# peaceminusones/Group-GAN-GCN-GAT

Hardware: AMD Instinct MI355X
Metric: scenes/sec (obs8/pred12, 20 peds) at 1/2/4/8 GPUs; ADE/FDE vs ref (higher is better)
Workload: dtype fp32; 1 GPU; train iteration = D-step + G-step (best_k=20, Adam), GAT generator; BASELINE configs[1] shape (batch 64); scenes_per_gpu=64, global_batch=64, obs_len=8, pred_len=12, generator=gat, hip_graph=True, parallelism=dp1

## Files before the change

### group-gan-gcn-gat_amd/csrc/fold.hip

```cpp
#include "sgg_common.h"

namespace sgg {

__global__ void __launch_bounds__(512) fold_fwd_kernel(const float* __restrict__ W, int ldw, int R, int E,
                                                       const float* __restrict__ We, const float* __restrict__ be,
                                                       const float* __restrict__ b1, const float* __restrict__ b2,
                                                       float* __restrict__ A, float* __restrict__ bias) {
  for (int r = threadIdx.x; r < R; r += blockDim.x) {
    float a0 = 0.f, a1 = 0.f, bb = 0.f;
    const float* w = W + (size_t)r * ldw;
#pragma unroll 8
    for (int e = 0; e < E; ++e) {
      const float we = w[e];
      a0 = fmaf(we, We[2 * e], a0);
      a1 = fmaf(we, We[2 * e + 1], a1);
      bb = fmaf(we, be[e], bb);
    }
    A[2 * r] = a0;
    A[2 * r + 1] = a1;
    bias[r] = bb + b1[r] + (b2 ? b2[r] : 0.f);
  }
}

struct FoldList {
  SggFold f[SGG_FOLD_MAX];
};

__global__ void __launch_bounds__(512) fold_fwd_multi_kernel(FoldList L) {
  const SggFold& d = L.f[blockIdx.x];
  for (int r = threadIdx.x; r < d.R; r += blockDim.x) {
    float a0 = 0.f, a1 = 0.f, bb = 0.f;
    const float* w = d.W + (size_t)r * d.ldw;
#pragma unroll 8
    for (int e = 0; e < d.E; ++e) {
      const float we = w[e];
      a0 = fmaf(we, d.We[2 * e], a0);
      a1 = fmaf(we, d.We[2 * e + 1], a1);
      bb = fmaf(we, d.be[e], bb);
    }
    d.A[2 * r] = a0;
    d.A[2 * r + 1] = a1;
    d.bias[r] = bb + d.b1[r] + (d.b2 ? d.b2[r] : 0.f);
  }
}

__device__ __forceinline__ void fold_bwd_body(const float* __restrict__ W, int ldw, int R, int E,
                                              const float* __restrict__ We, const float* __restrict__ be,
                                              const float* __restrict__ dA, const float* __restrict__ dbias,
                                              float* __restrict__ dW, int lddw, float* __restrict__ dWe,
                                              float* __restrict__ dbe, float* __restrict__ dbias_copy) {
  __shared__ float g3[3 * 512];
  __shared__ float part[3 * 512];
  for (int r = threadIdx.x; r < R; r += blockDim.x) {
    const float2 a = reinterpret_cast<const float2*>(dA)[r];
    const float b = dbias[r];
    g3[3 * r] = a.x;
    g3[3 * r + 1] = a.y;
    g3[3 * r + 2] = b;
    if (dbias_copy) dbias_copy[r] = b;
  }
  __syncthreads();
  const int ng = blockDim.x / E;
  const int t = threadIdx.x;
  if (t < ng * E) {
    const int e = t % E, g = t / E;
    const float we0 = We[2 * e], we1 = We[2 * e + 1], bee = be[e];
    float s0 = 0.f, s1 = 0.f, s2 = 0.f;
#pragma unroll 8
    for (int r = g; r < R; r += ng) {
      const float a0 = g3[3 * r], a1 = g3[3 * r + 1], b = g3[3 * r + 2];
      dW[(size_t)r * lddw + e] = fmaf(a0, we0, fmaf(a1, we1, b * bee));
      const float w = W[(size_t)r * ldw + e];
      s0 = fmaf(w, a0, s0);
      s1 = fmaf(w, a1, s1);
      s2 = fmaf(w, b, s2);
    }
    part[3 * t] = s0;
    part[3 * t + 1] = s1;
    part[3 * t + 2] = s2;
  }
  __syncthreads();
  if (t < 3 * E) {
    const int e = t / 3, j = t - 3 * e;
    float s = 0.f;
    for (int g = 0; g < ng; ++g) s += part[3 * (g * E + e) + j];
    if (j < 2) dWe[2 * e + j] = s;
    else dbe[e] = s;
  }
}

__global__ void __launch_bounds__(512) fold_bwd_kernel(const float* __restrict__ W, int ldw, int R, int E,
                                                       const float* __restrict__ We, const float* __restrict__ be,
                                                       const float* __restrict__ dA, const float* __restrict__ dbias,
                                                       float* __restrict__ dW, int lddw, float* __restrict__ dWe,
                                                       float* __restrict__ dbe, float* __restrict__ dbias_copy) {
  fold_bwd_body(W, ldw, R, E, We, be, dA, dbias, dW, lddw, dWe, dbe, dbias_copy);
// ... 53 lines not shown
```

### group-gan-gcn-gat_amd/csrc/lstm.hip

```cpp
#include <stdlib.h>
#include <string.h>

#include "sgg_common.h"

namespace sgg {

constexpr int kLstmPeds = 4;
constexpr int kLstmMaxT = 32;

__device__ __forceinline__ float sigm(float x) { return __builtin_amdgcn_rcpf(1.f + __expf(-x)); }
__device__ __forceinline__ float tanh_f(float x) {
  return fmaf(2.f, __builtin_amdgcn_rcpf(1.f + __builtin_amdgcn_exp2f(x * -2.8853900817779268f)), -1.f);
}

template <int H>
__global__ void __launch_bounds__(16 * H) lstm_fwd_kernel(
    const float* __restrict__ rel, const float* __restrict__ A, const float* __restrict__ Whh,
    const float* __restrict__ bias, const float* __restrict__ h0, const float* __restrict__ c0,
    const float* __restrict__ Wp, const float* __restrict__ bp, int T, int B, int decoder,
    float* __restrict__ h_all, float* __restrict__ c_all, float* __restrict__ act_all, float* __restrict__ rel_out) {
  const bool save_states = act_all != nullptr;
  constexpr int G4 = 4 * H;
  __shared__ __attribute__((aligned(16))) float hbuf[kLstmPeds][H];
  __shared__ float gbuf[kLstmPeds][G4];
// ... 236 lines not shown
    const bool x3 = H == 32 && !(x3e && strcmp(x3e, "0") == 0);
    snprintf(buf, sizeof buf, "sgg::lstm_fwd_mfma_kernel<%d, %s, %s>", H, tf[x3], tf[decoder != 0]);
  }
  else if (mw) snprintf(buf, sizeof buf, "sgg::lstm_mw_fwd_kernel<%d, %s, %s>", H, tf[decoder != 0], tf[save != 0]);
  else if (H <= 32) snprintf(buf, sizeof buf, "sgg::lstm_unit_fwd_kernel<%d>", H);
  else snprintf(buf, sizeof buf, "sgg::lstm_fwd_kernel<%d>", H);
  return buf;
}

static bool fwd_picks_mw(int H, int B, bool save) {
  const bool mw = lstm_mw_ok(H, B);
  if (save) return mw;
  return mw && !(lstm_fwd_mfma_ok(H, B) && !getenv("SGG_LSTM_NO_MFMA"));
}

extern "C" int sgg_lstm_u_ok(int T, int B, int H, int decoder, int save, int NU) {
  return !decoder && B > 0 && T >= 1 && NU >= 16 && NU % 16 == 0 && fwd_picks_mw(H, B, save != 0);
}

extern "C" int sgg_lstm_fwd_u(const float* rel, const float* A, const float* Whh, const float* bias, const float* h0,
                              const float* c0, int T, int B, int H, float* h_all, float* c_all, float* act_all,
                              const float* Wu, int ldwu, const float* cu, int NU, float* U, void* stream) {
  SGG_CHECK_ARG(rel && A && Whh && bias && h_all && c_all && Wu && cu && U, "sgg_lstm_fwd_u: null pointer");
  SGG_CHECK_ARG(sgg_lstm_u_ok(T, B, H, 0, act_all != nullptr, NU) && ldwu >= H,
                "sgg_lstm_fwd_u: no projection epilogue for T=%d B=%d H=%d NU=%d ldwu=%d (sgg_lstm_u_ok)", T, B, H, NU,
                ldwu);
  return lstm_mw_fwd(rel, A, Whh, bias, h0, c0, nullptr, nullptr, T, B, H, 0, h_all, c_all, act_all, nullptr,
                     (hipStream_t)stream, Wu, ldwu, cu, NU, U);
}

extern "C" int sgg_lstm_bwd_split(const float* A, const float* Whh, const float* Wp, const float* h_all,
                                  const float* c_all, const float* act_all, const float* rel, const float* rel_out,
                                  const float* dout, const float* dout2, int bsplit, int T, int B, int H, float* dh0,
                                  float* drel_in, float* drel_tot, float* wpart, void* stream) {
  SGG_CHECK_ARG(A && Whh && Wp && h_all && c_all && act_all && rel && rel_out && dout && dout2 && drel_in && drel_tot,
                "sgg_lstm_bwd_split: null pointer");
  SGG_CHECK_ARG(T >= 1 && B >= 1 && bsplit >= 0 && bsplit <= B && lstm_mw_ok(H, B),
                "sgg_lstm_bwd_split: bad sizes or no four-wave kernel (T=%d B=%d H=%d bsplit=%d)", T, B, H, bsplit);
  return lstm_mw_bwd(A, Whh, Wp, h_all, c_all, act_all, rel, rel_out, nullptr, dout, T, B, H, 1, dh0, drel_in,
                     drel_tot, wpart, (hipStream_t)stream, dout2, bsplit);
}

extern "C" int sgg_lstm_bwd_tail(const float* A, const float* Whh, const float* h_all, const float* c_all,
                                 const float* act_all, const float* rel, const float* dh_last, int T, int B, int H,
                                 int t_stop, float* drel_in, void* stream) {
  SGG_CHECK_ARG(A && Whh && h_all && c_all && act_all && rel && drel_in, "sgg_lstm_bwd_tail: null pointer");
  SGG_CHECK_ARG(T >= 1 && B >= 1 && t_stop >= 0 && t_stop < T && lstm_mw_ok(H, B),
                "sgg_lstm_bwd_tail: bad sizes or no four-wave kernel (T=%d B=%d H=%d t_stop=%d)", T, B, H, t_stop);
  return lstm_mw_bwd(A, Whh, nullptr, h_all, c_all, act_all, rel, nullptr, dh_last, nullptr, T, B, H, 0, nullptr,
                     drel_in, nullptr, nullptr, (hipStream_t)stream, nullptr, 0, t_stop);
}

static MwSeg to_mw(const SggLstmSeg& s) {
  return MwSeg{s.rel, s.A, s.Whh, s.bias, s.h0, s.c0, nullptr, nullptr, s.T, s.B, s.Bl, s.t0, s.Tl, s.Bsrc,
               s.h_all, s.c_all, s.act_all, nullptr, s.Wu, s.ldwu, s.cu, s.NU, s.U};
}

extern "C" int sgg_lstm_fwd_seg(const SggLstmSeg* seg, int H, void* stream) {
  SGG_CHECK_ARG(seg, "sgg_lstm_fwd_seg: null segment");
  SGG_CHECK_ARG(lstm_mw_ok(H, seg->B), "sgg_lstm_fwd_seg: no four-wave kernel for H=%d", H);
  return lstm_mw_fwd_seg(to_mw(*seg), H, (hipStream_t)stream);
}

static int device_cus() {
  static int ncu = 0;
  if (ncu == 0) {
    int d = 0, v = 0;
    const bool ok = hipGetDevice(&d) == hipSuccess &&
                    hipDeviceGetAttribute(&v, hipDeviceAttributeMultiprocessorCount, d) == hipSuccess;
    ncu = ok && v > 0 ? v : 256;
  }
  return ncu;
}

extern "C" int sgg_lstm_fwd_seg_glue(const SggLstmSeg* seg, int H, const SggGlueSeg* glue, void* stream) {
  SGG_CHECK_ARG(seg && glue, "sgg_lstm_fwd_seg_glue: null segment");
  SGG_CHECK_ARG(lstm_mw_ok(H, seg->B), "sgg_lstm_fwd_seg_glue: no four-wave kernel for H=%d", H);
  const SggGlueSeg& g = *glue;
  SGG_CHECK_ARG(g.kind == SGG_GLUE_NONE || g.kind == SGG_GLUE_SELECT || g.kind == SGG_GLUE_L2BWD,
                "sgg_lstm_fwd_seg_glue: glue kind %d", g.kind);
  if (g.kind == SGG_GLUE_SELECT) {
    SGG_CHECK_ARG(g.pred && g.gt && g.mask && g.scene_off && g.best, "sgg_lstm_fwd_seg_glue (select): null pointer");
    SGG_CHECK_ARG(g.S >= 0 && g.T >= 1 && g.B >= 0 && g.k >= 1 && g.k <= 256 && g.ldm >= g.T,
                  "sgg_lstm_fwd_seg_glue (select): bad sizes");
  } else if (g.kind == SGG_GLUE_L2BWD) {
    SGG_CHECK_ARG(g.pred && g.gt && g.mask && g.scene_off && g.gout && g.dpred,
                  "sgg_lstm_fwd_seg_glue (l2 backward): null pointer");
    SGG_CHECK_ARG(g.S >= 0 && g.T >= 1 && g.B >= 0 && g.ldm >= g.T && g.ldp >= 2 * g.B && g.ldd >= 2 * g.B,
                  "sgg_lstm_fwd_seg_glue (l2 backward): bad sizes");
  }
  if (g.kind != SGG_GLUE_NONE && g.S > 0) {
    const int cus = device_cus(), nblk = (seg->B + 15) / 16, last = nblk % cus;
    if ((nblk >= cus && last == 0) || last + g.S > cus) {
      const int rc = g.kind == SGG_GLUE_SELECT
                         ? sgg_l2_select(g.pred, g.gt, g.mask, g.ldm, g.scene_off, g.S, g.T, g.B, g.k, g.best, stream)
                         : sgg_l2_loss_bwd_scenes(g.pred, g.ldp, g.gt, g.mask, g.ldm, g.scene_off, g.S, g.T, g.B, g.w,
                                                  g.gout, g.dpred, g.ldd, g.term, stream);
      if (rc) return rc;
      return lstm_mw_fwd_seg(to_mw(*seg), H, (hipStream_t)stream);
    }
  }
  return lstm_mw_fwd_seg(to_mw(*seg), H, (hipStream_t)stream, glue);
}

extern "C" int sgg_lstm_fwd_seg2(const SggLstmSeg* a, int Ha, const SggLstmSeg* b, int Hb, void* stream) {
  SGG_CHECK_ARG(a && b, "sgg_lstm_fwd_seg2: null segment");
  SGG_CHECK_ARG(lstm_mw_ok(Ha, a->B) && lstm_mw_ok(Hb, b->B), "sgg_lstm_fwd_seg2: no four-wave kernel (Ha=%d Hb=%d)",
                Ha, Hb);
  return lstm_mw_fwd_seg2(to_mw(*a), Ha, to_mw(*b), Hb, (hipStream_t)stream);
}

extern "C" int sgg_lstm_fwd_seg3(const SggLstmSeg* a, int Ha, const SggLstmSeg* b, int Hb, const SggLstmSeg* c, int Hc,
                                 void* stream) {
  SGG_CHECK_ARG(a && b && c, "sgg_lstm_fwd_seg3: null segment");
  SGG_CHECK_ARG(lstm_mw_ok(Ha, a->B) && lstm_mw_ok(Hb, b->B) && lstm_mw_ok(Hc, c->B),
                "sgg_lstm_fwd_seg3: no four-wave kernel (Ha=%d Hb=%d Hc=%d)", Ha, Hb, Hc);
  return lstm_mw_fwd_seg3(to_mw(*a), Ha, to_mw(*b), Hb, to_mw(*c), Hc, (hipStream_t)stream);
}

extern "C" int sgg_lstm_bwd_shared(const float* A, const float* Whh, const float* h_all, const float* c_all,
                                   const float* act_all, const float* rel, const float* dh_last, int T, int B, int H,
                                   int t_sh, int Bsrc, float* drel_in, float* wpart, void* stream) {
  SGG_CHECK_ARG(A && Whh && h_all && c_all && act_all && rel, "sgg_lstm_bwd_shared: null pointer");
  SGG_CHECK_ARG(T >= 1 && B >= 1 && t_sh >= 1 && lstm_mw_ok(H, B),
                "sgg_lstm_bwd_shared: bad sizes or no four-wave kernel (T=%d B=%d H=%d t_sh=%d)", T, B, H, t_sh);
  SGG_CHECK_ARG(drel_in || (wpart && lstm_mw_bwd_nodx_ok(H)),
                "sgg_lstm_bwd_shared: drel_in may be NULL only with weight gradients (wpart) and H = 16 / 32 / 48 "
                "(wpart=%d H=%d)", wpart != nullptr, H);
  return lstm_mw_bwd(A, Whh, nullptr, h_all, c_all, act_all, rel, nullptr, dh_last, nullptr, T, B, H, 0, nullptr,
                     drel_in, nullptr, wpart, (hipStream_t)stream, nullptr, 0, 0, t_sh, Bsrc);
}

extern "C" int sgg_lstm_wpart_rows(int H, int B) {
  if (B < 0) return -1;
  return lstm_mw_ok(H, B) ? lstm_mw_wpart_rows(H, B) : 0;
}

extern "C" int sgg_lstm_fwd(const float* rel, const float* A, const float* Whh, const float* bias, const float* h0,
                            const float* c0, const float* Wp, const float* bp, int T, int B, int H, int decoder, float* h_all,
                            float* c_all, float* act_all, float* rel_out, void* stream) {
  SGG_CHECK_ARG(rel && A && Whh && bias && h_all && c_all, "sgg_lstm_fwd: null pointer");
  SGG_CHECK_ARG(!decoder || (Wp && bp && rel_out), "sgg_lstm_fwd: decoder needs Wp, bp, rel_out");
  SGG_CHECK_ARG(T >= 1 && B >= 0, "sgg_lstm_fwd: bad sizes T=%d B=%d", T, B);
  if (B == 0) return 0;
  hipStream_t st = (hipStream_t)stream;
  const bool mw = lstm_mw_ok(H, B);
  if (act_all && mw)
    return lstm_mw_fwd(rel, A, Whh, bias, h0, c0, Wp, bp, T, B, H, decoder, h_all, c_all, act_all, rel_out, st);
  if (!act_all && lstm_fwd_mfma_ok(H, B) && !getenv("SGG_LSTM_NO_MFMA"))
    return lstm_fwd_mfma(rel, A, Whh, bias, h0, c0, Wp, bp, T, B, H, decoder, h_all, c_all, nullptr, rel_out, st);
  if (mw)
    return lstm_mw_fwd(rel, A, Whh, bias, h0, c0, Wp, bp, T, B, H, decoder, h_all, c_all, act_all, rel_out, st);
  if (lstm_unit_ok(H, decoder) && !getenv("SGG_LSTM_ROWS"))
    return lstm_unit_fwd(rel, A, Whh, bias, h0, c0, Wp, bp, T, B, H, decoder, h_all, c_all, act_all, rel_out, st);
  switch (H) {
    case 16: return launch_lstm_fwd<16>(rel, A, Whh, bias, h0, c0, Wp, bp, T, B, decoder, h_all, c_all, act_all, rel_out, st);
    case 32: return launch_lstm_fwd<32>(rel, A, Whh, bias, h0, c0, Wp, bp, T, B, decoder, h_all, c_all, act_all, rel_out, st);
    case 48: return launch_lstm_fwd<48>(rel, A, Whh, bias, h0, c0, Wp, bp, T, B, decoder, h_all, c_all, act_all, rel_out, st);
    case 64: return launch_lstm_fwd<64>(rel, A, Whh, bias, h0, c0, Wp, bp, T, B, decoder, h_all, c_all, act_all, rel_out, st);
    default: SGG_CHECK_ARG(false, "sgg_lstm_fwd: hidden size %d not built (16/32/48/64)", H);
  }
}

static int dec_check(const SggDecInit* di, const float* A, const float* Whh, const float* bias, const float* Wp,
                     const float* bp, int T, int B, int H, float* h_all, float* c_all, float* act_all, float* rel_out,
                     const SggTrajOut* to) {
  SGG_CHECK_ARG(di && di->ctx && di->ped_scene && di->last_rel && (di->nz == 0 || di->z) && A && Whh && bias &&
                    ((h_all && c_all) || (!h_all && !c_all && !act_all)) && Wp && bp && rel_out,
                "sgg_lstm_fwd_dec: null pointer");
  SGG_CHECK_ARG(T >= 1 && B >= 0 && di->Bper >= 1 && B % di->Bper == 0 && di->Dc >= 1 && di->nz >= 0 &&
                    di->Dc + di->nz == H && di->ldc >= di->Dc && di->S >= 1,
                "sgg_lstm_fwd_dec: bad sizes (T=%d B=%d Bper=%d Dc=%d nz=%d H=%d)", T, B, di->Bper, di->Dc, di->nz, H);
  if (to) {
    SGG_CHECK_ARG(to->out && to->head && (!to->start || to->pos0), "sgg_lstm_fwd_dec: null pointer in SggTrajOut");
    SGG_CHECK_ARG(to->T0 >= 0 && to->ncol >= 1 && to->col0 >= 0 && to->col0 + to->ncol <= B &&
                      to->NB == (to->b ? 2 : 1) * to->ncol && to->ldh >= 2 * to->ncol &&
                      (!to->b || to->ldb >= 2 * to->ncol),
                  "sgg_lstm_fwd_dec: bad SggTrajOut sizes (NB=%d T0=%d col0=%d ncol=%d B=%d)", to->NB, to->T0,
                  to->col0, to->ncol, B);
  }
  return 0;
}

extern "C" int sgg_lstm_fwd_dec_seg(const SggDecInit* di, const float* A, const float* Whh, const float* bias,
                                    const float* Wp, const float* bp, int T, int B, int H, float* h_all, float* c_all,
                                    float* act_all, float* rel_out, float* rel0_out, const SggTrajOut* to,
                                    const SggLstmSeg* pre, int Hp, void* stream) {
  if (int rc = dec_check(di, A, Whh, bias, Wp, bp, T, B, H, h_all, c_all, act_all, rel_out, to)) return rc;
  SGG_CHECK_ARG(pre && B >= 1 && act_all && lstm_mw_ok(H, B) && lstm_mw_ok(Hp, pre->B),
                "sgg_lstm_fwd_dec_seg: needs a saving four-wave decoder and a prefix segment (H=%d B=%d Hp=%d)", H, B,
                Hp);
  return lstm_mw_fwd_dec_seg(A, Whh, bias, Wp, bp, T, B, H, h_all, c_all, act_all, rel_out, di, rel0_out, to,
                             to_mw(*pre), Hp, (hipStream_t)stream);
}

extern "C" int sgg_lstm_fwd_dec2(const SggDecInit* di, const SggDecInit* di2, const float* A, const float* Whh,
                                 const float* bias, const float* Wp, const float* bp, int T, int B, int B2, int H,
                                 float* rel_out, float* rel_out2, const SggTrajOut* to2, void* stream) {
  if (int rc = dec_check(di, A, Whh, bias, Wp, bp, T, B, H, nullptr, nullptr, nullptr, rel_out, nullptr)) return rc;
  if (int rc = dec_check(di2, A, Whh, bias, Wp, bp, T, B2, H, nullptr, nullptr, nullptr, rel_out2, to2)) return rc;
  SGG_CHECK_ARG(B >= 1 && B2 >= 1 && lstm_fwd_mfma_ok(H, B) && !getenv("SGG_LSTM_NO_MFMA"),
                "sgg_lstm_fwd_dec2: the batch-MFMA rollout family only (H=%d B=%d)", H, B);
  return lstm_fwd_mfma_dec2(di, di2, A, Whh, bias, Wp, bp, T, B, B2, H, rel_out, rel_out2, to2, (hipStream_t)stream);
}

extern "C" int sgg_lstm_fwd_dec(const SggDecInit* di, const float* A, const float* Whh, const float* bias,
                                const float* Wp, const float* bp, int T, int B, int H, float* h_all, float* c_all,
                                float* act_all, float* rel_out, float* rel0_out, const SggTrajOut* to,
                                void* stream) {
  if (int rc = dec_check(di, A, Whh, bias, Wp, bp, T, B, H, h_all, c_all, act_all, rel_out, to)) return rc;
  if (B == 0) return 0;
  hipStream_t st = (hipStream_t)stream;
  const bool mw = lstm_mw_ok(H, B);
  if (act_all && mw)
    return lstm_mw_fwd(nullptr, A, Whh, bias, nullptr, nullptr, Wp, bp, T, B, H, 1, h_all, c_all, act_all, rel_out,
                       st, nullptr, 0, nullptr, 0, nullptr, di, rel0_out, to);
  if (!act_all && lstm_fwd_mfma_ok(H, B) && !getenv("SGG_LSTM_NO_MFMA")) {
    if (to) {
      SGG_CHECK_ARG(!h_all, "sgg_lstm_fwd_dec: the batch-MFMA family writes the discriminator input without a "
                            "final state (h_all NULL)");
      return lstm_fwd_mfma_dec2(di, di, A, Whh, bias, Wp, bp, T, 0, B, H, nullptr, rel_out, to, st);
    }
    return lstm_fwd_mfma(nullptr, A, Whh, bias, nullptr, nullptr, Wp, bp, T, B, H, 1, h_all, c_all, nullptr, rel_out,
                         st, di);
  }
  SGG_CHECK_ARG(!to || mw, "sgg_lstm_fwd_dec: no family writes the discriminator input for H=%d B=%d", H, B);
  if (!act_all && mw)
    return lstm_mw_fwd(nullptr, A, Whh, bias, nullptr, nullptr, Wp, bp, T, B, H, 1, h_all, c_all, nullptr, rel_out, st,
                       nullptr, 0, nullptr, 0, nullptr, di, nullptr, to);
  SGG_CHECK_ARG(false, "sgg_lstm_fwd_dec: no fused decoder start for H=%d B=%d (use sgg_decoder_init)", H, B);
}

extern "C" int sgg_lstm_bwd(const float* A, const float* Whh, const float* Wp, const float* h_all, const float* c_all,
                            const float* act_all, const float* rel, const float* rel_out, const float* dh_last,
                            const float* dout, int T, int B, int H, int decoder, float* dG, float* dh0,
                            float* drel_in, float* drel_tot, float* wpart, void* stream) {
  SGG_CHECK_ARG(A && Whh && c_all && act_all, "sgg_lstm_bwd: null pointer");
  SGG_CHECK_ARG(drel_in || (!decoder && wpart && lstm_mw_ok(H, B) && lstm_mw_bwd_nodx_ok(H)),
                "sgg_lstm_bwd: drel_in may be NULL only for an encoder of the four-wave family with weight gradients "
                "(wpart) and H = 16 / 32 / 48 (decoder=%d wpart=%d H=%d)", decoder, wpart != nullptr, H);
  SGG_CHECK_ARG(!decoder || (Wp && dout && drel_tot), "sgg_lstm_bwd: decoder needs Wp, dout, drel_tot");
// ... 22 lines not shown
```

### group-gan-gcn-gat_amd/csrc/lstm_mw.hip

```cpp
#include <stdlib.h>
#include <string.h>

#include <type_traits>

#include "sgg_common.h"
#include "l2_body.h"

namespace sgg {

namespace {

constexpr int kMwThreads = 256;
constexpr int kMwPeds = 16;
constexpr int kMwMaxT = 64;
constexpr int kDgPitch = 68;

constexpr float kNegLog2e = -1.4426950408889634f;
__device__ __forceinline__ float gate_act(float x, float s, float nsl) {
  return fmaf(s, __builtin_amdgcn_rcpf(1.f + __builtin_amdgcn_exp2f(x * nsl)), 1.f - s);
}
__device__ __forceinline__ float tanh_m(float x) {
  return fmaf(2.f, __builtin_amdgcn_rcpf(1.f + __builtin_amdgcn_exp2f(x * (2.f * kNegLog2e))), -1.f);
}

template <int MU>
__device__ __forceinline__ void store_vec(float* p, const float (&v)[MU]) {
  if constexpr (MU == 4) {
    *reinterpret_cast<float4*>(p) = make_float4(v[0], v[1], v[2], v[3]);
  } else if constexpr (MU == 2) {
    *reinterpret_cast<float2*>(p) = make_float2(v[0], v[1]);
  } else if constexpr (MU == 3) {
    typedef float f3 __attribute__((ext_vector_type(3)));
    f3 x = {v[0], v[1], v[2]};
    __builtin_memcpy(p, &x, 12);
  } else {
#pragma unroll
    for (int i = 0; i < MU; ++i) p[i] = v[i];
  }
}
template <int MU>
__device__ __forceinline__ void load_vec(const float* p, float (&v)[MU]) {
  if constexpr (MU == 4) {
    const float4 x = *reinterpret_cast<const float4*>(p);
    v[0] = x.x; v[1] = x.y; v[2] = x.z; v[3] = x.w;
  } else if constexpr (MU == 2) {
    const float2 x = *reinterpret_cast<const float2*>(p);
    v[0] = x.x; v[1] = x.y;
  } else if constexpr (MU == 3) {
    typedef float f3 __attribute__((ext_vector_type(3)));
    f3 x;
    __builtin_memcpy(&x, p, 12);
    v[0] = x.x; v[1] = x.y; v[2] = x.z;
  } else {
#pragma unroll
    for (int i = 0; i < MU; ++i) v[i] = p[i];
  }
}

__device__ __forceinline__ int slot_unit(int j, int q) { return 16 * (j >> 2) + 4 * q + (j & 3); }

__device__ __forceinline__ floatx4 mfma_x3x2(const bf16x8 (&a)[2][3], const bf16x8 (&b)[2][3], floatx4 c) {
  constexpr int pa[6] = {2, 1, 0, 1, 0, 0}, pb[6] = {0, 1, 2, 0, 1, 0};
#pragma unroll
  for (int k = 0; k < 6; ++k) {
    c = __builtin_amdgcn_mfma_f32_16x16x32_bf16(a[0][pa[k]], b[0][pb[k]], c, 0, 0, 0);
    c = __builtin_amdgcn_mfma_f32_16x16x32_bf16(a[1][pa[k]], b[1][pb[k]], c, 0, 0, 0);
  }
  return c;
}

template <int H>
struct MwCfg {
  static constexpr int MU = H / 16, KS = H / 4, G4 = 4 * H;
  static constexpr int HP = H <= 16 ? 16 : 80;
  static constexpr int NHS = (kMwPeds * H + kMwThreads - 1) / kMwThreads;
  static constexpr int P = G4 * H + G4 + 2 * G4;
};

}


#ifdef SGG_LSTM_PROF
__device__ long long g_lstm_prof[256];
#define LMARK(i) \
  if (threadIdx.x == 0 && blk == 0) g_lstm_prof[i] = wall_clock64();
#define LSUB(k) \
  if ((threadIdx.x & 63) == 0 && blk == 0 && t == 4) g_lstm_prof[64 + 8 * (threadIdx.x >> 6) + (k)] = wall_clock64();
#define LUSE(x) __asm__ volatile("" ::"v"(x));
#define LSUBB(k) \
  if ((threadIdx.x & 63) == 0 && blk == 0 && t == T - 5) g_lstm_prof[96 + 8 * (threadIdx.x >> 6) + (k)] = wall_clock64();
#else
#define LSUBB(k)
#define LMARK(i)
#define LSUB(k)
#define LUSE(x)
#endif

#ifndef SGG_MW_UPRE
#define SGG_MW_UPRE 1
#endif
#ifndef SGG_MW_FWD_X3
#define SGG_MW_FWD_X3 1
#endif

namespace {

template <int H, bool DEC, bool SAVE>
__device__ __forceinline__ void mw_fwd_body(const MwSeg& sg, int blk, const SggGlueSeg* glue = nullptr) {
  constexpr int MU = MwCfg<H>::MU, KS = MwCfg<H>::KS;
  constexpr bool decoder = DEC, save = SAVE;
  const float* __restrict__ rel = sg.rel;
  const float* __restrict__ A = sg.A;
  const float* __restrict__ Whh = sg.Whh;
  const float* __restrict__ bias = sg.bias;
  const float* __restrict__ Wp = sg.Wp;
  const float* __restrict__ bp = sg.bp;
  float* __restrict__ h_all = sg.h_all;
  float* __restrict__ c_tile = sg.c_tile;
  float* __restrict__ act_tile = sg.act_tile;
  float* __restrict__ rel_out = sg.rel_out;
  const int T = sg.T, B = sg.B, Bl = sg.Bl, t0 = sg.t0, Tl = sg.Tl;
  constexpr bool X3 = !DEC && SGG_MW_FWD_X3 && H == 48;
  __shared__ float hb[X3 ? 1 : 2][KS][64];
  __shared__ sgg_uint4v hx[X3 ? 2 : 1][3][2][64];
  constexpr int kHsP = H + 4;
  __shared__ float hst[X3 && SAVE ? 2 : 1][kMwPeds][X3 && SAVE ? kHsP : 1];
  __shared__ float2 rpart[2][4][kMwPeds];
  __shared__ float relseq[kMwMaxT][kMwPeds][2];
  if constexpr (!DEC) {
    if (glue) {
      static_assert(sizeof(relseq) >= kL2MaxElems * sizeof(float) && sizeof(hx) >= kL2MaxK * sizeof(float),
                    "the glue bodies' LDS is lent by relseq / hx");
      float* msk = &relseq[0][0][0];
      if (glue->kind == SGG_GLUE_SELECT) {
        l2_select_body<kMwThreads / 64>(glue->pred, glue->gt, glue->mask, glue->ldm, glue->scene_off, glue->T,
                                        glue->B, glue->k, glue->best, blk, reinterpret_cast<float*>(&hx[0][0][0][0]),
                                        msk);
      } else if (threadIdx.x < 64) {
        l2_bwd_scene_body(glue->pred, glue->ldp, glue->gt, glue->mask, glue->ldm, glue->scene_off, glue->T, glue->B,
                          glue->w, glue->gout, glue->dpred, glue->ldd, glue->term, blk, threadIdx.x, msk);
      }
      return;
    }
  }
  const int g = __builtin_amdgcn_readfirstlane(threadIdx.x >> 6);
  const int lane = threadIdx.x & 63;
  const int q = lane >> 4, c16 = lane & 15;
  const int ped = blk * kMwPeds + c16;
  const int pc = ped < B ? ped : B - 1;
  LMARK(0);

  float w[MU][KS + 1], ak0[MU], ak1[MU];
  bf16x8 wx[X3 ? MU : 1][2][3];
  if constexpr (X3) {
#pragma unroll
    for (int mu = 0; mu < MU; ++mu) {
      const int row = (c16 & 3) * H + slot_unit(g * MU + mu, c16 >> 2);
      const float a0 = A[2 * row], a1 = A[2 * row + 1], bi = bias[row];
#pragma unroll
      for (int c = 0; c < 2; ++c) {
        float v[8];
#pragma unroll
        for (int i = 0; i < 8; ++i) {
          const int w2 = (8 * c + i) >> 2, m2 = (8 * c + i) & 3;
          if (m2 < MU)
            v[i] = Whh[row * H + slot_unit(w2 * MU + m2, q)];
          else if (m2 == 3)
            v[i] = q != 0 ? 0.f : w2 == 0 ? a0 : w2 == 1 ? a1 : w2 == 2 ? bi : 0.f;
          else
            v[i] = 0.f;
        }
        split8(v, wx[mu][c]);
      }
    }
  }
#pragma unroll
  for (int mu = 0; mu < (X3 ? 0 : MU); ++mu) {
    const int row = (c16 & 3) * H + slot_unit(g * MU + mu, c16 >> 2);
#pragma unroll
    for (int m = 0; m < KS / 4; ++m) {
      const float4 v = *reinterpret_cast<const float4*>(Whh + row * H + 16 * m + 4 * q);
      w[mu][4 * m] = v.x;
      w[mu][4 * m + 1] = v.y;
      w[mu][4 * m + 2] = v.z;
      w[mu][4 * m + 3] = v.w;
    }
    ak0[mu] = A[2 * row];
    ak1[mu] = A[2 * row + 1];
    w[mu][KS] = q == 0 ? ak0[mu] : q == 1 ? ak1[mu] : q == 2 ? bias[row] : 0.f;
  }
  float c[MU], wp0[MU], wp1[MU], hv0[MU];
  const int nsrc = (sg.Bsrc + kMwPeds - 1) / kMwPeds;
  const int sblk = t0 > 0 ? blk % nsrc : blk;
  const int spc = t0 > 0 ? pc % sg.Bsrc : pc;
#pragma unroll
  for (int i = 0; i < MU; ++i) {
    const int j = g * MU + i, u = slot_unit(j, q);
    float hv, cv;
    if (t0 > 0) {
      hv = h_all[((size_t)t0 * Bl + spc) * H + u];
      cv = c_tile[((((size_t)sblk * (Tl + 1) + t0) * 4 + g) * 64 + lane) * MU + i];
    } else {
      hv = sg.di.ctx ? dec_h0(sg.di, pc, u) : sg.h0 ? sg.h0[(size_t)pc * H + u] : 0.f;
      cv = sg.c0 ? sg.c0[(size_t)pc * H + u] : 0.f;
      if (save) {
        h_all[(size_t)pc * H + u] = hv;
        c_tile[(((size_t)blk * (Tl + 1) * 4 + g) * 64 + lane) * MU + i] = cv;
      }
    }
    c[i] = cv;
    hv0[i] = hv;
    if constexpr (!X3) hb[0][j][lane] = hv;
    wp0[i] = decoder ? Wp[u] : 0.f;
    wp1[i] = decoder ? Wp[H + u] : 0.f;
  }
  const float bp0 = decoder ? bp[0] : 0.f, bp1 = decoder ? bp[1] : 0.f;
  constexpr int kTo = 4;
  float2 tov[kTo];
  float2* tod[kTo];
  int nto = 0;
  if (DEC && sg.to.out != nullptr) {
    const SggTrajOut& to = sg.to;
    const int dup = to.b ? 2 : 1;
    const int nh = to.T0 * dup, nb = to.b ? T : 0, ns = to.start ? dup : 0;
    nto = kMwPeds * (nh + nb + ns);
    auto entry = [&](int e, float2*& d) -> float2 {
      const int i = e % kMwPeds, w = e / kMwPeds;
      const int col = min(blk * kMwPeds + i, B - 1) - to.col0;
      d = nullptr;
      if (col < 0 || col >= to.ncol) return make_float2(0.f, 0.f);
      float2* o2 = reinterpret_cast<float2*>(to.out);
      if (w < nh) {
        const int t = w / dup, half = w - t * dup;
        d = o2 + (size_t)t * to.NB + col + half * to.ncol;
        return reinterpret_cast<const float2*>(to.head + (size_t)t * to.ldh)[col];
      }
      if (w < nh + nb) {
        const int t = w - nh;
        d = o2 + (size_t)(to.T0 + t) * to.NB + to.ncol + col;
        return reinterpret_cast<const float2*>(to.b + (size_t)t * to.ldb)[col];
      }
      d = reinterpret_cast<float2*>(to.start) + col + (w - nh - nb) * to.ncol;
      return reinterpret_cast<const float2*>(to.pos0)[col];
    };
#pragma unroll
    for (int m = 0; m < kTo; ++m) {
      const int e = threadIdx.x + m * kMwThreads;
      tod[m] = nullptr;
      if (e < nto) tov[m] = entry(e, tod[m]);
    }
    for (int e = threadIdx.x + kTo * kMwThreads; e < nto; e += kMwThreads) {
      float2* d;
      const float2 v = entry(e, d);
      if (d) *d = v;
    }
  }

  constexpr int kRelPer = 2 * kMwPeds * kMwMaxT / kMwThreads;
  float rv[kRelPer];
  if (!decoder) {
#pragma unroll
    for (int m = 0; m < kRelPer; ++m) {
      const int e = threadIdx.x + m * kMwThreads;
      if (e < 2 * kMwPeds * T) {
        const int t = e / (2 * kMwPeds), p = (e >> 1) & (kMwPeds - 1), k = e & 1;
        const int pp = min(blk * kMwPeds + p, B - 1);
        rv[m] = rel[((size_t)(t0 + t) * B + pp) * 2 + k];
      }
    }
  }

  constexpr bool kUPre = SGG_MW_UPRE && !DEC && H <= 48;
  constexpr int kUT = 8;
  const float* __restrict__ Wu = sg.Wu;
  const int ldwu = sg.ldwu, NU = sg.NU;
  const bool upre = kUPre && sg.U && NU <= 16 * 4 * kUT &&
                    ((reinterpret_cast<uintptr_t>(Wu) | ((uintptr_t)ldwu * 4)) & 15) == 0;
  float wu[kUPre ? kUT : 1][KS];
  float cuv[kUPre ? kUT : 1][4];
  auto load_wu = [&](int i) {
    const int ntile = NU >> 4;
    const float4 v = *reinterpret_cast<const float4*>(sg.cu + 16 * min(g + 4 * i, ntile - 1) + 4 * q);
    cuv[i][0] = v.x;
    cuv[i][1] = v.y;
    cuv[i][2] = v.z;
    cuv[i][3] = v.w;
    const float* wr = Wu + (size_t)(min(g + 4 * i, ntile - 1) * 16 + c16) * ldwu;
#pragma unroll
    for (int m = 0; m < KS / 4; ++m) {
      const float4 w4 = *reinterpret_cast<const float4*>(wr + 16 * m + 4 * q);
      wu[i][4 * m] = w4.x;
      wu[i][4 * m + 1] = w4.y;
      wu[i][4 * m + 2] = w4.z;
      wu[i][4 * m + 3] = w4.w;
    }
  };

  if (!decoder) {
#pragma unroll
    for (int m = 0; m < kRelPer; ++m) {
      const int e = threadIdx.x + m * kMwThreads;
      if (e < 2 * kMwPeds * T) relseq[e / (2 * kMwPeds)][(e >> 1) & (kMwPeds - 1)][e & 1] = rv[m];
    }
  }
  if (DEC && nto > 0) {
#pragma unroll
    for (int m = 0; m < kTo; ++m)
      if (tod[m]) *tod[m] = tov[m];
  }
  auto put_x3 = [&](int buf, const float (&hv)[MU], float inv) {
    float v[4] = {0.f, 0.f, 0.f, inv};
#pragma unroll
    for (int i = 0; i < MU; ++i) v[i] = hv[i];
    unsigned wd[3][2];
#pragma unroll
    for (int k = 0; k < 2; ++k) {
      float h0, m0, l0, h1, m1, l1;
      split3(v[2 * k], h0, m0, l0);
      split3(v[2 * k + 1], h1, m1, l1);
      wd[0][k] = bf16_pack_top(h0, h1);
      wd[1][k] = bf16_pack_top(m0, m1);
      wd[2][k] = bf16_pack_top(l0, l1);
    }
#pragma unroll
    for (int p = 0; p < 3; ++p)
      reinterpret_cast<uint2*>(&hx[buf][p][g >> 1][lane])[g & 1] = make_uint2(wd[p][0], wd[p][1]);
  };
  auto in_x3 = [&](int t) -> float {
    return g < 2 ? rel[((size_t)(t0 + t) * B + pc) * 2 + g] : (g == 2 ? 1.f : 0.f);
  };
  if constexpr (X3) put_x3(0, hv0, in_x3(0));
  lds_barrier();
  LMARK(1);

  auto input = [&](int t) -> float {
// ... 178 lines not shown
    for (int ks = 0; ks < KS; ++ks) hk[ks] = hb[X3 ? 0 : T & 1][ks][lane];
    const int ntile = NU >> 4;
    floatx4 acc[kUT];
#pragma unroll
    for (int i = 0; i < kUT; ++i) acc[i] = floatx4{0.f, 0.f, 0.f, 0.f};
#pragma unroll
    for (int ks = 0; ks < KS; ++ks)
#pragma unroll
      for (int i = 0; i < kUT; ++i) acc[i] = __builtin_amdgcn_mfma_f32_16x16x4f32(wu[i][ks], hk[ks], acc[i], 0, 0, 0);
#pragma unroll
    for (int i = 0; i < kUT; ++i) {
      const int nt = g + 4 * i;
      if (nt < ntile)
        *reinterpret_cast<float4*>(U + (size_t)pc * NU + 16 * nt + 4 * q) =
            make_float4(acc[i][0] + cuv[i][0], acc[i][1] + cuv[i][1], acc[i][2] + cuv[i][2], acc[i][3] + cuv[i][3]);
    }
  } else if (!decoder && U) {
    float hk[KS];
#pragma unroll
    for (int ks = 0; ks < KS; ++ks) hk[ks] = hb[X3 ? 0 : T & 1][ks][lane];
    const int ntile = NU >> 4;
    float wa[2][KS], wn[2][KS];
    const bool vec = ((reinterpret_cast<uintptr_t>(Wu) | ((uintptr_t)ldwu * 4)) & 15) == 0;
    auto load_w = [&](int nt, float (&w)[KS]) {
      const float* wr = Wu + (size_t)(min(nt, ntile - 1) * 16 + c16) * ldwu;
      if (vec) {
#pragma unroll
        for (int m = 0; m < KS / 4; ++m) {
          const float4 v = *reinterpret_cast<const float4*>(wr + 16 * m + 4 * q);
          w[4 * m] = v.x;
          w[4 * m + 1] = v.y;
          w[4 * m + 2] = v.z;
          w[4 * m + 3] = v.w;
        }
      } else {
#pragma unroll
        for (int ks = 0; ks < KS; ++ks) w[ks] = wr[slot_unit(ks, q)];
      }
    };
    load_w(g, wa[0]);
    load_w(g + 4, wa[1]);
    for (int nt = g; nt < ntile; nt += 8) {
      const bool more = nt + 8 < ntile;
      if (more) {
        load_w(nt + 8, wn[0]);
        load_w(nt + 12, wn[1]);
      }
      floatx4 acc0 = floatx4{0.f, 0.f, 0.f, 0.f}, acc1 = acc0;
#pragma unroll
      for (int ks = 0; ks < KS; ++ks) {
        acc0 = __builtin_amdgcn_mfma_f32_16x16x4f32(wa[0][ks], hk[ks], acc0, 0, 0, 0);
        acc1 = __builtin_amdgcn_mfma_f32_16x16x4f32(wa[1][ks], hk[ks], acc1, 0, 0, 0);
      }
      const float4 cb0 = *reinterpret_cast<const float4*>(cu + 16 * nt + 4 * q);
      *reinterpret_cast<float4*>(U + (size_t)pc * NU + 16 * nt + 4 * q) =
          make_float4(acc0[0] + cb0.x, acc0[1] + cb0.y, acc0[2] + cb0.z, acc0[3] + cb0.w);
      if (nt + 4 < ntile) {
        const float4 cb1 = *reinterpret_cast<const float4*>(cu + 16 * (nt + 4) + 4 * q);
        *reinterpret_cast<float4*>(U + (size_t)pc * NU + 16 * (nt + 4) + 4 * q) =
            make_float4(acc1[0] + cb1.x, acc1[1] + cb1.y, acc1[2] + cb1.z, acc1[3] + cb1.w);
      }
      if (more) {
#pragma unroll
        for (int ks = 0; ks < KS; ++ks) {
          wa[0][ks] = wn[0][ks];
          wa[1][ks] = wn[1][ks];
        }
      }
    }
  }
  LMARK(63);
}

template <int H, bool DEC, bool SAVE>
__global__ void __launch_bounds__(kMwThreads) lstm_mw_fwd_kernel(MwSeg sg, SggGlueSeg gl, int nblk) {
  if constexpr (!DEC) {
    if ((int)blockIdx.x >= nblk) {
      mw_fwd_body<H, DEC, SAVE>(sg, blockIdx.x - nblk, &gl);
      return;
    }
  }
  mw_fwd_body<H, DEC, SAVE>(sg, blockIdx.x);
}

template <int HA, bool SA, int HB, bool SB>
__global__ void __launch_bounds__(kMwThreads) lstm_mw_fwd2_kernel(MwSeg a, MwSeg b, int nblk_a) {
  if ((int)blockIdx.x < nblk_a)
    mw_fwd_body<HA, false, SA>(a, blockIdx.x);
  else
    mw_fwd_body<HB, false, SB>(b, blockIdx.x - nblk_a);
}

template <int HA, bool SA, int HB, bool SB>
__global__ void __launch_bounds__(kMwThreads) lstm_mw_fwd2d_kernel(MwSeg a, MwSeg b, int nblk_a) {
  if ((int)blockIdx.x < nblk_a)
    mw_fwd_body<HA, true, SA>(a, blockIdx.x);
  else
    mw_fwd_body<HB, false, SB>(b, blockIdx.x - nblk_a);
}

template <int HA, bool SA, int HB, bool SB, int HC, bool SC>
__global__ void __launch_bounds__(kMwThreads) lstm_mw_fwd3_kernel(MwSeg a, MwSeg b, MwSeg c, int nblk_a, int nblk_b) {
  const int blk = blockIdx.x;
  if (blk < nblk_a)
    mw_fwd_body<HA, false, SA>(a, blk);
  else if (blk < nblk_a + nblk_b)
    mw_fwd_body<HB, false, SB>(b, blk - nblk_a);
  else
    mw_fwd_body<HC, false, SC>(c, blk - nblk_a - nblk_b);
}

#ifndef SGG_MW_BWD_DB
#define SGG_MW_BWD_DB 1
#endif
#ifndef SGG_MW_BWD_X3
#define SGG_MW_BWD_X3 1
#endif
#ifndef SGG_MW_BWD_DB_NODX
#define SGG_MW_BWD_DB_NODX 1
#endif

template <int H, bool DEC, bool WGRAD, bool NODX>
__device__ __forceinline__ void mw_bwd_body(
    const float* __restrict__ A, const float* __restrict__ Whh, const float* __restrict__ Wp,
    const float* __restrict__ h_all, const float* __restrict__ c_tile, const float* __restrict__ act_tile,
    const float* __restrict__ rel, const float* __restrict__ rel_out, const float* __restrict__ dh_last,
    const float* __restrict__ dout, int T, int B, float* __restrict__ dh0, float* __restrict__ drel_in,
    float* __restrict__ drel_tot, float* __restrict__ wpart, const float* __restrict__ dout2, int bsplit,
    int t_stop, int t_sh, int Bsrc) {
  static_assert(!NODX || (WGRAD && !DEC), "NODX: the encoder's weight-gradient form only");
  constexpr int MU = MwCfg<H>::MU, KS = MwCfg<H>::KS, G4 = MwCfg<H>::G4, HP = MwCfg<H>::HP;
  constexpr bool decoder = DEC, wgrad = WGRAD;
  constexpr bool BX3 = SGG_MW_BWD_X3 != 0;
  constexpr bool hacc = wgrad && !decoder && !NODX;
  constexpr bool oacc = !(wgrad && !decoder);
  constexpr bool hdb = wgrad;
  constexpr int NHS = MwCfg<H>::NHS, P0 = MwCfg<H>::P, P = P0 + (DEC ? 2 * H + 2 : 0);
  __shared__ float dgb[2][4][KS][kDgPitch];
  __shared__ float part[2][4][KS][64];
  __shared__ float2 fbp[NODX ? 1 : 2][4][kMwPeds];
  __shared__ float hs[2][kMwPeds][HP];
  const int g = __builtin_amdgcn_readfirstlane(threadIdx.x >> 6);
  const int lane = threadIdx.x & 63;
  const int q = lane >> 4, c16 = lane & 15;
  const int blk = blockIdx.x;
  LMARK(0);
  const int ped = blk * kMwPeds + c16;
  const bool valid = ped < B;
  const int pc = valid ? ped : B - 1;
  const int nsrc = t_sh > 0 ? Bsrc / kMwPeds : 1;
  auto sblk = [&](bool shared_at) { return (shared_at && t_sh > 0) ? blk % nsrc : blk; };

  float hv[NHS];
  const int ht = threadIdx.x & (kMwThreads - 1);
  auto stage_load = [&](int t) {
#pragma unroll
    for (int m = 0; m < NHS; ++m) {
      const int e = ht + m * kMwThreads;
      int r = min(blk * kMwPeds + e / H, B - 1);
      if (t <= t_sh && t_sh > 0) r %= Bsrc;
      hv[m] = h_all[((size_t)t * B + r) * H + e % H];
    }
// ... 428 lines not shown
          x += __shfl_xor(x, o);
          y += __shfl_xor(y, o);
        }
        const int u = slot_unit(g * MU + i, q);
        if (c16 == 0) {
          row[P0 + u] = x;
          row[P0 + H + u] = y;
        }
      }
      if (g == 0 && q == 0) {
        float x = dbp0, y = dbp1;
#pragma unroll
        for (int o = 1; o < 16; o <<= 1) {
          x += __shfl_xor(x, o);
          y += __shfl_xor(y, o);
        }
        if (c16 == 0) {
          row[P0 + 2 * H] = x;
          row[P0 + 2 * H + 1] = y;
        }
      }
    }
  }
  LMARK(62);
}

#define SGG_MW_BWD_PARAMS                                                                                         \
  const float *__restrict__ A, const float *__restrict__ Whh, const float *__restrict__ Wp,                      \
      const float *__restrict__ h_all, const float *__restrict__ c_tile, const float *__restrict__ act_tile,     \
      const float *__restrict__ rel, const float *__restrict__ rel_out, const float *__restrict__ dh_last,       \
      const float *__restrict__ dout, int T, int B, float *__restrict__ dh0, float *__restrict__ drel_in,        \
      float *__restrict__ drel_tot, float *__restrict__ wpart, const float *__restrict__ dout2, int bsplit,      \
      int t_stop, int t_sh, int Bsrc
#define SGG_MW_BWD_ARGS                                                                                           \
  A, Whh, Wp, h_all, c_tile, act_tile, rel, rel_out, dh_last, dout, T, B, dh0, drel_in, drel_tot, wpart, dout2,  \
      bsplit, t_stop, t_sh, Bsrc

template <int H, bool DEC, bool WGRAD>
__global__ void __launch_bounds__(WGRAD ? 2 * kMwThreads : kMwThreads) lstm_mw_bwd_kernel(SGG_MW_BWD_PARAMS) {
  mw_bwd_body<H, DEC, WGRAD, false>(SGG_MW_BWD_ARGS);
}

template <int H>
__global__ void __launch_bounds__(2 * kMwThreads) lstm_mw_bwd_nodx_kernel(SGG_MW_BWD_PARAMS) {
  mw_bwd_body<H, false, true, true>(SGG_MW_BWD_ARGS);
}
constexpr bool mw_bwd_nodx_built(int H) { return H == 16 || H == 32 || H == 48; }

template <int H>
int launch_seg(const MwSeg& sg, bool decoder, hipStream_t st, const SggGlueSeg* glue = nullptr) {
  const int nblk = (sg.B + kMwPeds - 1) / kMwPeds;
  auto k = decoder ? (sg.act_tile ? lstm_mw_fwd_kernel<H, true, true> : lstm_mw_fwd_kernel<H, true, false>)
                   : (sg.act_tile ? lstm_mw_fwd_kernel<H, false, true> : lstm_mw_fwd_kernel<H, false, false>);
  const bool ride = glue && !decoder && glue->kind != SGG_GLUE_NONE && glue->S > 0;
  SggGlueSeg gl{};
  if (ride) gl = *glue;
  hipLaunchKernelGGL(k, dim3(nblk + (ride ? gl.S : 0)), dim3(kMwThreads), 0, st, sg, gl, nblk);
  SGG_RETURN_LAUNCH("sgg_lstm_fwd");
}

int launch_seg_h(const MwSeg& sg, int H, bool decoder, hipStream_t st, const SggGlueSeg* glue = nullptr) {
  switch (H) {
    case 16: return launch_seg<16>(sg, decoder, st, glue);
    case 32: return launch_seg<32>(sg, decoder, st, glue);
    case 48: return launch_seg<48>(sg, decoder, st, glue);
    default: return launch_seg<64>(sg, decoder, st, glue);
  }
}

template <int H>
int launch_bwd(const float* A, const float* Whh, const float* Wp, const float* h_all, const float* c_all,
               const float* act_all, const float* rel, const float* rel_out, const float* dh_last, const float* dout,
               int T, int B, int decoder, float* dh0, float* drel_in, float* drel_tot, float* wpart, hipStream_t st,
               const float* dout2, int bsplit, int t_stop, int t_sh, int Bsrc) {
  const int grid = (B + kMwPeds - 1) / kMwPeds;
  auto k = decoder ? (wpart ? lstm_mw_bwd_kernel<H, true, true> : lstm_mw_bwd_kernel<H, true, false>)
                   : (wpart ? lstm_mw_bwd_kernel<H, false, true> : lstm_mw_bwd_kernel<H, false, false>);
  if constexpr (mw_bwd_nodx_built(H)) {
    if (!drel_in) k = lstm_mw_bwd_nodx_kernel<H>;
  }
  hipLaunchKernelGGL(k, dim3(grid), dim3(wpart ? 2 * kMwThreads : kMwThreads), 0, st, A, Whh, Wp, h_all, c_all, act_all, rel, rel_out,
                     dh_last, dout, T, B, dh0, drel_in, drel_tot, wpart, dout2, bsplit, t_stop, t_sh, Bsrc);
  SGG_RETURN_LAUNCH("sgg_lstm_bwd");
}

}

bool lstm_mw_ok(int H, int B) {
  (void)B;
  const char* e = getenv("SGG_LSTM_MW");
  if (e && strcmp(e, "0") == 0) return false;
  if (e && strcmp(e, "big") == 0) return H == 48 || H == 64;
  return H == 16 || H == 32 || H == 48 || H == 64;
}

bool lstm_mw_bwd_nodx_ok(int H) { return mw_bwd_nodx_built(H); }

long long lstm_mw_state_floats(int T, int B, int H, int which) {
  const long long padded = (long long)(B + kMwPeds - 1) / kMwPeds * kMwPeds;
  return which == 0 ? (long long)T * padded * 4 * H : (long long)(T + 1) * padded * H;
}

int lstm_mw_wpart_rows(int H, int B) {
  (void)H;
  return (B + kMwPeds - 1) / kMwPeds;
}

int lstm_mw_fwd(const float* rel, const float* A, const float* Whh, const float* bias, const float* h0,
                const float* c0, const float* Wp, const float* bp, int T, int B, int H, int decoder, float* h_all,
                float* c_all, float* act_all, float* rel_out, hipStream_t st, const float* Wu, int ldwu,
                const float* cu, int NU, float* U, const SggDecInit* di, float* rel0_out, const SggTrajOut* to) {
  SGG_CHECK_ARG(decoder || T <= kMwMaxT, "sgg_lstm_fwd: encoder sequences of the H=%d kernels hold <= %d steps (T=%d)",
                H, kMwMaxT, T);
  MwSeg sg{rel, A, Whh, bias, h0, c0, Wp, bp, T, B, B, 0, T, B, h_all, c_all, act_all, rel_out, Wu, ldwu, cu, NU, U};
  if (di) {
    sg.di = *di;
    sg.rel0_out = rel0_out;
  }
  if (to) sg.to = *to;
  return launch_seg_h(sg, H, decoder != 0, st);
}

static int seg_check(const MwSeg& s, int H, const char* fn) {
  SGG_CHECK_ARG(s.rel && s.A && s.Whh && s.bias && s.h_all && (s.c_tile || !s.act_tile), "%s: null pointer", fn);
  SGG_CHECK_ARG(H == 16 || H == 32 || H == 48 || H == 64, "%s: hidden size %d (16/32/48/64)", fn, H);
  SGG_CHECK_ARG(s.T >= 1 && s.T <= kMwMaxT && s.B >= 1 && s.Bl >= s.B && s.t0 >= 0 && s.t0 + s.T <= s.Tl,
                "%s: bad sizes T=%d B=%d Bl=%d t0=%d Tl=%d", fn, s.T, s.B, s.Bl, s.t0, s.Tl);
  SGG_CHECK_ARG(s.t0 == 0 || (s.c_tile && s.Bsrc >= 1 && s.Bsrc <= s.Bl &&
                              (s.Bsrc == s.B || (s.Bsrc % kMwPeds == 0 && s.B % s.Bsrc == 0))),
                "%s: a segment from step t0=%d needs the saved cells and Bsrc = B or a multiple of 16 dividing B "
                "(B=%d Bsrc=%d)", fn, s.t0, s.B, s.Bsrc);
  SGG_CHECK_ARG(s.t0 == 0 || (!s.h0 && !s.c0), "%s: t0 > 0 takes its state from h_all / c_all, not h0 / c0", fn);
  SGG_CHECK_ARG(!s.U || (s.Wu && s.cu && s.NU >= 16 && s.NU % 16 == 0 && s.ldwu >= H), "%s: bad projection", fn);
  return 0;
}

int lstm_mw_fwd_seg(const MwSeg& s, int H, hipStream_t st, const SggGlueSeg* glue) {
  if (int rc = seg_check(s, H, glue ? "sgg_lstm_fwd_seg_glue" : "sgg_lstm_fwd_seg")) return rc;
  return launch_seg_h(s, H, false, st, glue);
}

int lstm_mw_fwd_seg2(const MwSeg& a, int Ha, const MwSeg& b, int Hb, hipStream_t st) {
  if (int rc = seg_check(a, Ha, "sgg_lstm_fwd_seg2 (a)")) return rc;
  if (int rc = seg_check(b, Hb, "sgg_lstm_fwd_seg2 (b)")) return rc;
  const int na = (a.B + kMwPeds - 1) / kMwPeds, nb = (b.B + kMwPeds - 1) / kMwPeds;
  if (Ha == 32 && Hb == 48 && b.act_tile) {
    auto k = a.act_tile ? lstm_mw_fwd2_kernel<32, true, 48, true> : lstm_mw_fwd2_kernel<32, false, 48, true>;
    hipLaunchKernelGGL(k, dim3(na + nb), dim3(kMwThreads), 0, st, a, b, na);
    SGG_RETURN_LAUNCH("sgg_lstm_fwd_seg2");
  }
  if (int rc = launch_seg_h(a, Ha, false, st)) return rc;
  return launch_seg_h(b, Hb, false, st);
}

int lstm_mw_fwd_dec_seg(const float* A, const float* Whh, const float* bias, const float* Wp, const float* bp, int T,
                        int B, int H, float* h_all, float* c_all, float* act_all, float* rel_out, const SggDecInit* di,
                        float* rel0_out, const SggTrajOut* to, const MwSeg& b, int Hb, hipStream_t st) {
  if (int rc = seg_check(b, Hb, "sgg_lstm_fwd_dec_seg (prefix)")) return rc;
  MwSeg a{nullptr, A, Whh, bias, nullptr, nullptr, Wp, bp, T, B, B, 0, T, B, h_all, c_all, act_all, rel_out};
  a.di = *di;
  a.rel0_out = rel0_out;
  if (to) a.to = *to;
  const int na = (B + kMwPeds - 1) / kMwPeds, nb = (b.B + kMwPeds - 1) / kMwPeds;
  if (H == 32 && Hb == 48 && act_all && b.act_tile) {
    hipLaunchKernelGGL((lstm_mw_fwd2d_kernel<32, true, 48, true>), dim3(na + nb), dim3(kMwThreads), 0, st, a, b, na);
    SGG_RETURN_LAUNCH("sgg_lstm_fwd_dec_seg");
  }
  if (int rc = launch_seg_h(a, H, true, st)) return rc;
  return launch_seg_h(b, Hb, false, st);
}

int lstm_mw_fwd_seg3(const MwSeg& a, int Ha, const MwSeg& b, int Hb, const MwSeg& c, int Hc, hipStream_t st) {
  if (int rc = seg_check(a, Ha, "sgg_lstm_fwd_seg3 (a)")) return rc;
  if (int rc = seg_check(b, Hb, "sgg_lstm_fwd_seg3 (b)")) return rc;
  if (int rc = seg_check(c, Hc, "sgg_lstm_fwd_seg3 (c)")) return rc;
  const int na = (a.B + kMwPeds - 1) / kMwPeds, nb = (b.B + kMwPeds - 1) / kMwPeds, nc = (c.B + kMwPeds - 1) / kMwPeds;
  if (Ha == 32 && Hb == 48 && Hc == 32 && !a.act_tile && b.act_tile && c.act_tile) {
    hipLaunchKernelGGL((lstm_mw_fwd3_kernel<32, false, 48, true, 32, true>), dim3(na + nb + nc), dim3(kMwThreads), 0, st,
                       a, b, c, na, nb);
    SGG_RETURN_LAUNCH("sgg_lstm_fwd_seg3");
  }
  if (int rc = lstm_mw_fwd_seg2(a, Ha, b, Hb, st)) return rc;
  return launch_seg_h(c, Hc, false, st);
}

int lstm_mw_bwd(const float* A, const float* Whh, const float* Wp, const float* h_all, const float* c_all,
                const float* act_all, const float* rel, const float* rel_out, const float* dh_last, const float* dout,
// ... 19 lines not shown
```

### group-gan-gcn-gat_amd/csrc/sgg_common.h

```cpp
#pragma once
#include <hip/hip_runtime.h>
#include <stdint.h>
#include <stdio.h>
#include <stdarg.h>
#include "../../include/sgg.h"

typedef float floatx4 __attribute__((ext_vector_type(4)));

namespace sgg {

constexpr int kWave = 64;
constexpr int kGatEncMaxHeads = SGG_GATENC_MAX_HEADS;
using GatEncArgs = SggGatEncArgs;
constexpr int kHidden = 512;

void set_error(const char* fmt, ...);

#define SGG_CHECK_ARG(cond, ...)            \
  do {                                      \
    if (!(cond)) {                          \
      ::sgg::set_error(__VA_ARGS__);        \
      return SGG_E_ARG;                     \
    }                                       \
  } while (0)
// ... 29 lines not shown
                                                        const float* Wp, const float* bp, int T, int B, int H,
                                                        int decoder, float* h_all, float* c_all, float* act_all,
                                                        float* rel_out, hipStream_t st,
                                                        const SggDecInit* di = nullptr);

__attribute__((visibility("hidden"))) int lstm_fwd_mfma_dec2(const SggDecInit* di, const SggDecInit* di2,
                                                             const float* A, const float* Whh, const float* bias,
                                                             const float* Wp, const float* bp, int T, int B, int B2,
                                                             int H, float* rel_out, float* rel_out2,
                                                             const SggTrajOut* to2, hipStream_t st);

__attribute__((visibility("hidden"))) bool lstm_unit_ok(int H, int decoder);
__attribute__((visibility("hidden"))) int lstm_unit_fwd(const float* rel, const float* A, const float* Whh,
                                                        const float* bias, const float* h0, const float* c0,
                                                        const float* Wp, const float* bp, int T, int B, int H,
                                                        int decoder, float* h_all, float* c_all, float* act_all,
                                                        float* rel_out, hipStream_t st);
__attribute__((visibility("hidden"))) int lstm_unit_bwd(const float* A, const float* Whh, const float* Wp,
                                                        const float* c_all, const float* act_all, const float* dh_last,
                                                        const float* dout, int T, int B, int H, int decoder, float* dG,
                                                        float* dh0, float* drel_in, float* drel_tot, hipStream_t st);

__attribute__((visibility("hidden"))) bool lstm_mw_ok(int H, int B);
__attribute__((visibility("hidden"))) long long lstm_mw_state_floats(int T, int B, int H, int which);
__attribute__((visibility("hidden"))) int lstm_mw_wpart_rows(int H, int B);
__attribute__((visibility("hidden"))) int lstm_mw_fwd(const float* rel, const float* A, const float* Whh,
                                                      const float* bias, const float* h0, const float* c0,
                                                      const float* Wp, const float* bp, int T, int B, int H,
                                                      int decoder, float* h_all, float* c_all, float* act_all,
                                                      float* rel_out, hipStream_t st, const float* Wu = nullptr,
                                                      int ldwu = 0, const float* cu = nullptr, int NU = 0,
                                                      float* U = nullptr, const SggDecInit* di = nullptr,
                                                      float* rel0_out = nullptr, const SggTrajOut* to = nullptr);
__attribute__((visibility("hidden"))) int lstm_mw_bwd(const float* A, const float* Whh, const float* Wp,
                                                      const float* h_all, const float* c_all, const float* act_all,
                                                      const float* rel, const float* rel_out, const float* dh_last,
                                                      const float* dout, int T, int B, int H, int decoder,
                                                      float* dh0, float* drel_in, float* drel_tot, float* wpart,
                                                      hipStream_t st, const float* dout2 = nullptr,
                                                      int bsplit = 0, int t_stop = 0, int t_sh = 0, int Bsrc = 0);
__attribute__((visibility("hidden"))) bool lstm_mw_bwd_nodx_ok(int H);
struct MwSeg {
  const float *rel, *A, *Whh, *bias, *h0, *c0, *Wp, *bp;
  int T, B, Bl, t0, Tl, Bsrc;
  float *h_all, *c_tile, *act_tile, *rel_out;
  const float* Wu;
  int ldwu;
  const float* cu;
  int NU;
  float* U;
  SggDecInit di;
  float* rel0_out;
  SggTrajOut to;
};
__device__ __forceinline__ float dec_h0(const SggDecInit& d, int p, int u) {
  const int r = p / d.Bper, i = p - r * d.Bper;
  if (u < d.Dc) return d.ctx[(size_t)i * d.ldc + u];
  const int s = d.ped_scene[i];
  const int k = (d.best && r == 0) ? (int)d.best[s] : d.first_k + r - (d.best ? 1 : 0);
  return d.z[((size_t)k * d.S + s) * d.nz + (u - d.Dc)];
}
__device__ __forceinline__ float dec_rel0(const SggDecInit& d, int p, int k) {
  return d.last_rel[(size_t)(p % d.Bper) * 2 + k];
}
__attribute__((visibility("hidden"))) int lstm_mw_fwd_seg(const MwSeg& s, int H, hipStream_t st,
                                                          const SggGlueSeg* glue = nullptr);
__attribute__((visibility("hidden"))) int lstm_mw_fwd_seg2(const MwSeg& a, int Ha, const MwSeg& b, int Hb,
                                                           hipStream_t st);
__attribute__((visibility("hidden"))) int lstm_mw_fwd_dec_seg(const float* A, const float* Whh, const float* bias,
                                                              const float* Wp, const float* bp, int T, int B, int H,
                                                              float* h_all, float* c_all, float* act_all,
                                                              float* rel_out, const SggDecInit* di, float* rel0_out,
                                                              const SggTrajOut* to, const MwSeg& b, int Hb,
                                                              hipStream_t st);
__attribute__((visibility("hidden"))) int lstm_mw_fwd_seg3(const MwSeg& a, int Ha, const MwSeg& b, int Hb,
                                                           const MwSeg& c, int Hc, hipStream_t st);

__attribute__((visibility("hidden"))) void fold_bwd_multi(const SggFoldBwd* folds, int n, hipStream_t st);

__device__ __forceinline__ float keep_if(float v, bool keep) {
  return __int_as_float(__float_as_int(v) & (keep ? -1 : 0));
}

typedef __bf16 bf16x8 __attribute__((ext_vector_type(8)));
typedef unsigned sgg_uint4v __attribute__((ext_vector_type(4)));

__device__ __forceinline__ float bf16_trunc(float x) { return __uint_as_float(__float_as_uint(x) & 0xffff0000u); }
__device__ __forceinline__ unsigned bf16_pack_top(float a, float b) {
  return __builtin_amdgcn_perm(__float_as_uint(b), __float_as_uint(a), 0x07060302u);
}
__device__ __forceinline__ void split3(float x, float& h, float& m, float& l) {
#pragma clang fp contract(off)
  h = bf16_trunc(x);
  const float r = x - h;
  m = bf16_trunc(r);
  l = r - m;
}
__device__ __forceinline__ void split8(const float (&v)[8], bf16x8 (&o)[3]) {
  sgg_uint4v u[3];
#pragma unroll
  for (int i = 0; i < 4; ++i) {
    float h0, m0, l0, h1, m1, l1;
    split3(v[2 * i], h0, m0, l0);
    split3(v[2 * i + 1], h1, m1, l1);
    u[0][i] = bf16_pack_top(h0, h1);
    u[1][i] = bf16_pack_top(m0, m1);
    u[2][i] = bf16_pack_top(l0, l1);
  }
#pragma unroll
  for (int p = 0; p < 3; ++p) o[p] = __builtin_bit_cast(bf16x8, u[p]);
}
__device__ __forceinline__ floatx4 mfma_x3(const bf16x8 (&a)[3], const bf16x8 (&b)[3], floatx4 c) {
  c = __builtin_amdgcn_mfma_f32_16x16x32_bf16(a[2], b[0], c, 0, 0, 0);
  c = __builtin_amdgcn_mfma_f32_16x16x32_bf16(a[1], b[1], c, 0, 0, 0);
  c = __builtin_amdgcn_mfma_f32_16x16x32_bf16(a[0], b[2], c, 0, 0, 0);
  c = __builtin_amdgcn_mfma_f32_16x16x32_bf16(a[1], b[0], c, 0, 0, 0);
  c = __builtin_amdgcn_mfma_f32_16x16x32_bf16(a[0], b[1], c, 0, 0, 0);
  return __builtin_amdgcn_mfma_f32_16x16x32_bf16(a[0], b[0], c, 0, 0, 0);
}

__device__ __forceinline__ float elu(float x) { return x > 0.f ? x : expm1f(x); }
__device__ __forceinline__ float elu_grad(float x) { return x > 0.f ? 1.f : expf(x); }

}
```

### group-gan-gcn-gat_amd/sgan/_native.py

```python
import ctypes
import os

import torch

from ._srchash import source_hash

_LIB_EXPLICIT = bool(os.environ.get("SGG_LIB"))
_LIB_PATH = os.environ.get("SGG_LIB") or os.path.join(os.path.dirname(os.path.abspath(__file__)), "_lib", "libsgg.so")

_i = ctypes.c_int
_f = ctypes.c_float
_p = ctypes.c_void_p
_sz = ctypes.c_size_t

MAX_HEADS = 4


class GatEncWeights(ctypes.Structure):
    _fields_ = [("Wi", _p * MAX_HEADS), ("ai", _p * MAX_HEADS), ("Wio", _p), ("aio", _p),
                ("Wg", _p * MAX_HEADS), ("ag", _p * MAX_HEADS), ("Wgo", _p), ("ago", _p), ("Woe", _p), ("boe", _p)]


class GatEncArgs(ctypes.Structure):
    _fields_ = [("X", _p), ("ldx", _i), ("labels", _p), ("scene_off", _p), ("S", _i), ("np", _i), ("nh", _i),
                ("alpha", _f), ("w", GatEncWeights), ("y", _p), ("ldy", _i), ("dy", _p), ("lddy", _i), ("dX", _p),
                ("lddx", _i), ("slab", _p), ("saved", _p), ("X2", _p), ("ldx2", _i), ("kx1", _i),
                ("dX2", _p), ("lddx2", _i), ("dy_copies", _i), ("dy_cstride", _i)]


_pargs = ctypes.POINTER(GatEncArgs)


class GcnModArgs(ctypes.Structure):
    _fields_ = [("X", _p), ("ldx", _i), ("X2", _p), ("ldx2", _i), ("kx1", _i), ("labels", _p), ("scene_off", _p),
                ("S", _i), ("np", _i), ("fin", _i), ("fe", _i), ("bf16", _i), ("W0i", _p), ("W1i", _p), ("W0g", _p),
                ("W1g", _p), ("Woe", _p), ("boe", _p), ("y", _p), ("ldy", _i), ("dy", _p), ("lddy", _i),
                ("dy_copies", _i), ("dy_cstride", _i), ("dX", _p), ("lddx", _i), ("dX2", _p), ("lddx2", _i),
                ("slab", _p)]


_gargs = ctypes.POINTER(GcnModArgs)


class LstmSeg(ctypes.Structure):
    _fields_ = [("rel", _p), ("A", _p), ("Whh", _p), ("bias", _p), ("h0", _p), ("c0", _p), ("T", _i), ("B", _i),
                ("Bl", _i), ("t0", _i), ("Tl", _i), ("Bsrc", _i), ("h_all", _p), ("c_all", _p), ("act_all", _p),
                ("Wu", _p), ("ldwu", _i), ("cu", _p), ("NU", _i), ("U", _p)]


_sargs = ctypes.POINTER(LstmSeg)


GLUE_NONE, GLUE_SELECT, GLUE_L2BWD = 0, 1, 2


class GlueSeg(ctypes.Structure):
    _fields_ = [("kind", _i), ("pred", _p), ("ldp", _i), ("gt", _p), ("mask", _p), ("ldm", _i), ("scene_off", _p),
                ("S", _i), ("T", _i), ("B", _i), ("k", _i), ("best", _p), ("w", _f), ("gout", _p), ("dpred", _p),
                ("ldd", _i), ("term", _p)]

FOLD_MAX = 8


class Fold(ctypes.Structure):
    _fields_ = [("W", _p), ("ldw", _i), ("R", _i), ("E", _i), ("We", _p), ("be", _p), ("b1", _p), ("b2", _p),
                ("A", _p), ("bias", _p)]

RED_MAX = 24
FOLDB_MAX = 6


class Red(ctypes.Structure):
    _fields_ = [("src", _p), ("rows", _i), ("ld", _i), ("col0", _i), ("cols", _i), ("out", _p), ("map", _i),
                ("N", _i), ("ldo", _i), ("trans", _i)]


class FoldBwd(ctypes.Structure):
    _fields_ = [("W", _p), ("ldw", _i), ("R", _i), ("E", _i), ("We", _p), ("be", _p),
                ("dA_src", _p), ("dA_rows", _i), ("dA_ld", _i), ("dA_col0", _i),
                ("db_src", _p), ("db_rows", _i), ("db_ld", _i), ("db_col0", _i),
                ("dW", _p), ("lddw", _i), ("dWe", _p), ("dbe", _p), ("dbias_copy", _p)]


class DecInit(ctypes.Structure):
    _fields_ = [("ctx", _p), ("ldc", _i), ("Dc", _i), ("z", _p), ("nz", _i), ("best", _p), ("first_k", _i),
                ("ped_scene", _p), ("S", _i), ("Bper", _i), ("last_rel", _p)]


LOSSJOB_MAX = 2


class TrajOut(ctypes.Structure):
    _fields_ = [("out", _p), ("NB", _i), ("T0", _i), ("col0", _i), ("ncol", _i), ("head", _p), ("ldh", _i),
                ("b", _p), ("ldb", _i), ("pos0", _p), ("start", _p)]


class PoolBatch(ctypes.Structure):
    _fields_ = [("U", _p), ("pos", _p), ("scene_off", _p), ("chunks", _p), ("nchunks", _i), ("max_rows", _i),
                ("gpw", _i), ("B", _i), ("max_n", _i), ("out", _p), ("argmax", _p), ("nchunks_dev", _p)]


class GatLayerSet(ctypes.Structure):
    _fields_ = [("x1", _p), ("ld1", _i), ("K1", _i), ("x2", _p), ("ld2", _i), ("K2", _i), ("seg_off", _p),
                ("nseg", _i), ("n", _i), ("max_seg", _i), ("xn", _p), ("rstd", _p), ("wh", _p), ("hp", _p), ("y", _p),
                ("ldy", _i)]


class L2Job(ctypes.Structure):
    _fields_ = [("term", _p), ("S", _i), ("loss", _p)]


class BceJob(ctypes.Structure):
    _fields_ = [("x", _p), ("n", _i), ("split", _i), ("ya", _p), ("yb", _p), ("w", _f), ("loss", _p),
                ("addend", _p), ("total", _p), ("nvalid", _p)]


SIGNATURES = {
    "sgg_version": (_i, []),
    "sgg_last_error": (ctypes.c_char_p, []),
    "sgg_source_hash": (ctypes.c_char_p, []),
    "sgg_xw": (_i, [_p, _i, _p, _i, _p, _i, _i, _p, _p, _i, _i, _i, _i, _i, _p]),
    "sgg_xw_bf16": (_i, [_p, _i, _p, _i, _p, _i, _i, _p, _p, _i, _i, _i, _i, _i, _p]),
    "sgg_pool_plan": (_i, [_p, _i, _i, _i, _i, _p, _i, _p, _p]),
    "sgg_pool_fwd": (_i, [_p, _p, _p, _p, _p, _p, _p, _i, _i, _i, _i, _i, _i, _p, _p, _p, _p]),
    "sgg_pool_plan_bf16": (_i, [_p, _i, _i, _i, _p, _i, _p, _p]),
    "sgg_pool_fwd_bf16": (_i, [_p, _p, _p, _p, _p, _p, _p, _i, _i, _i, _i, _i, _i, _p, _p, _p, _p]),
    "sgg_pool_fwd2": (_i, [ctypes.POINTER(PoolBatch), ctypes.POINTER(PoolBatch), _p, _p, _p, _i, _i, _p]),
    "sgg_pool_bwd_grid": (_i, [_i]),
    "sgg_pool_dh_dw": (_i, [_p, _i, _p, _i, _p, _i, _i, _p, _i, _i, _i, _p, _sz, _p]),
    "sgg_pool_bwd": (_i, [_p, _p, _p, _p, _p, _p, _p, _p, _i, _i, _i, _i, _p, _p, _p]),
    "sgg_gat_fwd": (_i, [_p, _i, _p, _p, _p, _p, _i, _i, _i, _f, _i, _i, _i, _p, _p, _i, _p]),
    "sgg_gat_bwd": (_i, [_p, _i, _p, _p, _p, _i, _i, _i, _f, _i, _i, _i, _p, _p, _p, _i, _p, _p, _p, _p]),
    "sgg_gat_fwd_ex": (_i, [_p, _i, _p, _p, _p, _p, _p, _i, _i, _i, _f, _i, _i, _i, _p, _p, _i, _p]),
    "sgg_gat_bwd_ex": (_i, [_p, _i, _p, _p, _p, _p, _i, _i, _i, _f, _i, _i, _i, _p, _p, _p, _i, _p, _p, _p, _p, _p,
                            _p]),
    "sgg_gat_bwd_ex_work_bytes": (_sz, [_i, _i, _i]),
    "sgg_gat_layer_lds_bytes": (_sz, [_i, _i, _i]),
    "sgg_gat_layer_fwd": (_i, [_p, _i, _i, _p, _i, _i, _p, _p, _p, _p, _p, _i, _i, _i, _i, _f, _f, _i, _i, _i, _p, _p,
                               _p, _p, _p, _i, _p]),
    "sgg_gat_layer_fwd2": (_i, [ctypes.POINTER(GatLayerSet), ctypes.POINTER(GatLayerSet), _p, _p, _p, _p, _i, _i, _f,
                                _f, _i, _i, _p]),
    "sgg_seg_norm_fwd": (_i, [_p, _i, _i, _p, _i, _f, _p, _i, _p, _p]),
    "sgg_seg_norm_bwd": (_i, [_p, _i, _p, _i, _i, _p, _i, _p, _p, _i, _p]),
    "sgg_group_index_ws": (_sz, [_i, _i]),
    "sgg_group_index": (_i, [_p, _p, _i, _i, _i, _p, _p, _p, _p, _p, _p, _p]),
    "sgg_seg_reduce": (_i, [_p, _i, _i, _p, _p, _p, _p, _p, _i, _i, _p, _i, _p]),
    "sgg_seg_gather": (_i, [_p, _i, _i, _p, _p, _p, _i, _p, _i, _p]),
    "sgg_xtw_splits": (_i, [_i, _i, _i]),
    "sgg_lstm_bwd_split": (_i, [_p, _p, _p, _p, _p, _p, _p, _p, _p, _p, _i, _i, _i, _i, _p, _p, _p, _p, _p]),
    "sgg_lstm_bwd_tail": (_i, [_p, _p, _p, _p, _p, _p, _p, _i, _i, _i, _i, _p, _p]),
    "sgg_lstm_fwd_seg": (_i, [_sargs, _i, _p]),
    "sgg_lstm_fwd_seg_glue": (_i, [_sargs, _i, ctypes.POINTER(GlueSeg), _p]),
    "sgg_lstm_fwd_seg2": (_i, [_sargs, _i, _sargs, _i, _p]),
    "sgg_lstm_fwd_seg3": (_i, [_sargs, _i, _sargs, _i, _sargs, _i, _p]),
    "sgg_lstm_bwd_shared": (_i, [_p, _p, _p, _p, _p, _p, _p, _i, _i, _i, _i, _i, _p, _p, _p]),
    "sgg_lstm_u_ok": (_i, [_i, _i, _i, _i, _i, _i]),
    "sgg_lstm_fwd_u": (_i, [_p, _p, _p, _p, _p, _p, _i, _i, _i, _p, _p, _p, _p, _i, _p, _i, _p, _p]),
    "sgg_head_ok": (_i, [_i, _i]),
    "sgg_head_slab_cols": (_i, [_i, _i]),
    "sgg_head_fwd": (_i, [_p, _i, _i, _i, _i, _p, _p, _p, _p, _i, _p, _p, _p]),
    "sgg_head_bwd": (_i, [_p, _i, _i, _i, _i, _p, _p, _p, _p, _p, _i, _p, _i, _p, _p, _p, _p, _i, _f, _p, _p]),
    "sgg_head_fwdbwd": (_i, [_p, _i, _i, _i, _i, _p, _p, _p, _p, _i, _p, _p, _i, _p, _p, _p, _p, _i, _f, _p, _p]),
    "sgg_xtw_partial": (_i, [_p, _i, _p, _i, _p, _i, _i, _i, _i, _i, _p, _sz, _p]),
    "sgg_grad_finish": (_i, [ctypes.POINTER(Red), _i, ctypes.POINTER(FoldBwd), _i, _p, _sz, _p]),
    "sgg_lstm_fwd_dec": (_i, [ctypes.POINTER(DecInit), _p, _p, _p, _p, _p, _i, _i, _i, _p, _p, _p, _p, _p,
                              ctypes.POINTER(TrajOut), _p]),
    "sgg_lstm_fwd_dec2": (_i, [ctypes.POINTER(DecInit), ctypes.POINTER(DecInit), _p, _p, _p, _p, _p, _i, _i, _i, _i,
                               _p, _p, ctypes.POINTER(TrajOut), _p]),
    "sgg_lstm_fwd_dec_seg": (_i, [ctypes.POINTER(DecInit), _p, _p, _p, _p, _p, _i, _i, _i, _p, _p, _p, _p, _p,
                                  ctypes.POINTER(TrajOut), _sargs, _i, _p]),
    "sgg_grad_finish_losses": (_i, [ctypes.POINTER(Red), _i, ctypes.POINTER(FoldBwd), _i, _p, _sz,
                                    ctypes.POINTER(L2Job), _i, ctypes.POINTER(BceJob), _i, _p]),
    "sgg_adam_parts": (_i, [ctypes.c_longlong]),
    "sgg_adam_step": (_i, [_p, _p, _p, _p, _p, _i, ctypes.c_double, ctypes.c_double, ctypes.c_double, _f, _f, _p, _p,
                          _sz, _p]),
    "sgg_xtw": (_i, [_p, _i, _p, _i, _p, _i, _i, _i, _i, _p, _i, _i, _p, _p, _sz, _p]),
    "sgg_fold_fwd": (_i, [_p, _i, _i, _i, _p, _p, _p, _p, _p, _p, _p]),
    "sgg_fold_fwd_multi": (_i, [ctypes.POINTER(Fold), _i, _p]),
    "sgg_fold_bwd": (_i, [_p, _i, _i, _i, _p, _p, _p, _p, _p, _i, _p, _p, _p, _p]),
    "sgg_lstm_fwd": (_i, [_p, _p, _p, _p, _p, _p, _p, _p, _i, _i, _i, _i, _p, _p, _p, _p, _p]),
    "sgg_lstm_state_floats": (ctypes.c_longlong, [_i, _i, _i, _i]),
    "sgg_lstm_wpart_rows": (_i, [_i, _i]),
    "sgg_lstm_kernel_name": (ctypes.c_char_p, [_i, _i, _i, _i, _i]),
    "sgg_lstm_bwd": (_i, [_p, _p, _p, _p, _p, _p, _p, _p, _p, _p, _i, _i, _i, _i, _p, _p, _p, _p, _p, _p]),
    "sgg_bce_fwd": (_i, [_p, _i, _i, _p, _p, _f, _p, _p, _p, _p, _p]),
    "sgg_bce_bwd": (_i, [_p, _i, _i, _p, _p, _f, _p, _p, _p, _p]),
    "sgg_gatenc_param_size": (_i, [_i]),
    "sgg_gatenc_lds_bytes": (ctypes.c_longlong, [_i, _i, _i]),
    "sgg_gatenc_saved_floats": (ctypes.c_longlong, [_i, _i, _i]),
    "sgg_gatenc_fwd": (_i, [_pargs, _p]),
    "sgg_gatenc_fwd2": (_i, [_pargs, _pargs, _p]),
    "sgg_gatenc_bwd": (_i, [_pargs, _p]),
    "sgg_gcnmod_param_size": (_i, [_i, _i]),
    "sgg_gcnmod_slab_rows": (_i, [_i]),
    "sgg_gcnmod_lds_bytes": (ctypes.c_longlong, [_i, _i, _i, _i]),
    "sgg_gcnmod_fwd": (_i, [_gargs, _p]),
    "sgg_gcnmod_fwd2": (_i, [_gargs, _gargs, _p]),
    "sgg_gcnmod_bwd": (_i, [_gargs, _p]),
    "sgg_slab_reduce": (_i, [_p, _i, _i, _p, _p]),
    "sgg_gather_batch_floats": (ctypes.c_longlong, [_i, _i, _i]),
    "sgg_gather_batch": (_i, [_p, _i, _p, _i, _i, _i, _p, _p]),
    "sgg_traj_cat": (_i, [_p, _i, _i, _p, _i, _p, _i, _i, _i, _p, _p, _p, _p]),
    "sgg_decoder_init": (_i, [_p, _i, _i, _p, _i, _p, _i, _i, _p, _i, _i, _p, _p, _p, _p]),
    "sgg_l2_select": (_i, [_p, _p, _p, _i, _p, _i, _i, _i, _i, _p, _p]),
    "sgg_l2_loss_fwd": (_i, [_p, _i, _p, _p, _i, _p, _i, _i, _i, _f, _p, _p, _p, _p]),
    "sgg_l2_loss_bwd": (_i, [_p, _i, _p, _p, _i, _p, _p, _i, _i, _f, _p, _p, _i, _p]),
    "sgg_l2_loss_bwd_scenes": (_i, [_p, _i, _p, _p, _i, _p, _i, _i, _i, _f, _p, _p, _i, _p, _p]),
}

_lib = None


class NativeError(RuntimeError):
    pass


def lib_path():
    return _LIB_PATH


def built_hash():
    return load(require_gpu=False).sgg_source_hash().decode()

# ... 39 lines not shown
```

### group-gan-gcn-gat_amd/sgan/kernels.py

```python
import contextlib
import functools
import os
import weakref

import torch

from . import _native as N

GATENC_FUSED = os.environ.get("SGG_GATENC_FUSED", "1") != "0"
GATENC_SAVE = os.environ.get("SGG_GATENC_SAVE", "1") != "0"
DUAL_POOL_BWD = os.environ.get("SGG_DUAL_POOL_BWD", "1") != "0"
SIDE_STREAM = os.environ.get("SGG_SIDE_STREAM", "0") == "1"


DEBUG = os.environ.get("SGG_DEBUG", "0") == "1"


def _lib():
    return N.load()


def _req(t, name, dtype=torch.float32):
    if not t.is_cuda:
        raise N.NativeError("%s must be a device tensor (no CPU path)" % name)
# ... 103 lines not shown

    bf16 = (prec or _PRECISION) == "bf16"
    fn = _lib().sgg_xw_bf16 if bf16 else _lib().sgg_xw

    def launch():
        N.check(fn(N.ptr(x), x.stride(0), N.ptr(mask), mask.stride(0) if mask is not None else 0,
                   N.ptr(w), w.stride(0), int(bool(trans_w)), N.ptr(bias), N.ptr(y), y.stride(0), M, K, Nn,
                   int(act), N.stream_ptr()), "sgg_xw")
    launch()
    if timer.active and M > 0:
        tw = "true" if trans_w else "false"
        name = ("sgg::xw_bf16_kernel<%s>" % tw if bf16 else
                "sgg::xw_splitk_kernel<%s>" % tw if K >= 256 else
                "sgg::xw_kernel<true, true>" if trans_w and K <= 256 else
                "sgg::xw_kernel<%s, false>" % tw)
        timer.add(name, (M, K, Nn, mask is not None), 2.0 * M * K * Nn,
                  4.0 * (M * K * (2 if mask is not None else 1) + K * Nn + M * Nn), launch)
    return y


def xtw(X, Y, colsum=False, trans_c=False, out=None, mask=None):
    lib = _lib()
    X = _rows(X, "X")
    Y = _rows(Y, "Y")
    if mask is not None:
        mask = _rows(mask, "mask")
        assert mask.shape == Y.shape
    R, M = X.shape
    Nn = Y.shape[1]
    assert Y.shape[0] == R
    shape = (Nn, M) if trans_c else (M, Nn)
    if out is None:
        C = torch.empty(shape, device=X.device, dtype=torch.float32)
    else:
        assert tuple(out.shape) == shape and out.stride(1) == 1, (out.shape, shape)
        C = out
    if R == 0:
        C.zero_()
        return (C, torch.zeros(Nn, device=X.device)) if colsum else C
    splits = lib.sgg_xtw_splits(R, M, Nn)
    ws = torch.empty(splits * (M * Nn + Nn), device=X.device, dtype=torch.float32)
    cs = torch.empty(Nn, device=X.device, dtype=torch.float32) if colsum else None
    def launch():
        N.check(lib.sgg_xtw(N.ptr(X), X.stride(0), N.ptr(Y), Y.stride(0), N.ptr(mask),
                            mask.stride(0) if mask is not None else 0, R, M, Nn, N.ptr(C), C.stride(0), int(trans_c),
                            N.ptr(cs), N.ptr(ws), ws.numel() * 4, N.stream_ptr()), "sgg_xtw")
    launch()
    if timer.active:
        timer.add("sgg::xtw_partial_kernel+xtw_reduce_kernel", (R, M, Nn, mask is not None), 2.0 * R * M * Nn,
                  4.0 * (R * M + R * Nn * (2 if mask is not None else 1) + M * Nn) + 8.0 * ws.numel(), launch)
    return (C, cs) if colsum else C


def fold_fwd(W, We, be, b1, b2=None):
    key, ver = _fold_key(W, We, be, b1, b2)
    ent = _FOLD_CACHE.get(key)
    if _fold_hit(ent, ver, (W, We, be, b1, b2)):
        return ent[1], ent[2]
    prefold([(W, We, be, b1, b2)])
    ent = _FOLD_CACHE[key]
    return ent[1], ent[2]


_EPOCH = {}
_FOLD_CACHE = {}


def _fold_key(W, We, be, b1, b2):
    ts = (W, We, be, b1, b2)
    key = tuple((t.data_ptr(), tuple(t.shape), t.stride(0)) if t is not None else None for t in ts)
    ver = tuple((t._version, _EPOCH.get(t.data_ptr(), 0)) if t is not None else None for t in ts)
    return key, ver


def _owner(t):
    return t._base if t._base is not None else t


def _fold_hit(ent, ver, ts):
    return (ent is not None and ent[0] == ver
            and all((r is None) if t is None else (r is not None and r() is _owner(t)) for r, t in zip(ent[4], ts)))


def _fold_purge():
    dead = [k for k, e in _FOLD_CACHE.items() if any(r is not None and r() is None for r in e[4])]
    for k in dead:
        del _FOLD_CACHE[k]


def clear_fold_cache():
    _FOLD_CACHE.clear()


def prefold(specs):
    todo = []
    for W, We, be, b1, b2 in specs:
        key, ver = _fold_key(W, We, be, b1, b2)
        if not _fold_hit(_FOLD_CACHE.get(key), ver, (W, We, be, b1, b2)):
            todo.append((key, ver, (W, We, be, b1, b2)))
    if not todo:
        return
    _fold_purge()
    arr = (N.Fold * len(todo))()
    outs = []
    for k, (key, ver, (W, We, be, b1, b2)) in enumerate(todo):
        W = _rows(W, "W")
        R, E = W.shape
        A = torch.empty(R, 2, device=W.device, dtype=torch.float32)
        bias = torch.empty(R, device=W.device, dtype=torch.float32)
        parts = (W, We.contiguous(), be.contiguous(), b1.contiguous(), b2.contiguous() if b2 is not None else None)
        arr[k] = N.Fold(N.ptr(parts[0]), W.stride(0), R, E, N.ptr(parts[1]), N.ptr(parts[2]), N.ptr(parts[3]),
                        N.ptr(parts[4]), N.ptr(A), N.ptr(bias))
        outs.append((key, ver, A, bias, parts))
    for i in range(0, len(todo), N.FOLD_MAX):
        chunk = (N.Fold * min(N.FOLD_MAX, len(todo) - i))(*arr[i:i + N.FOLD_MAX])
        N.check(_lib().sgg_fold_fwd_multi(chunk, len(chunk), N.stream_ptr()), "sgg_fold_fwd_multi")
    for (key, ver, A, bias, parts), (_, _, ts) in zip(outs, todo):
        refs = tuple(weakref.ref(_owner(t)) if t is not None else None for t in ts)
        copies = tuple(p for p, t in zip(parts, ts) if p is not None and p.data_ptr() != t.data_ptr())
        _FOLD_CACHE[key] = (ver, A, bias, copies, refs)


def lstm_fold_spec(lstm, emb):
    return (lstm.weight_ih_l0, emb.weight, emb.bias, lstm.bias_ih_l0, lstm.bias_hh_l0)


def pool_fold_spec(pool):
    l1, E = pool.mlp_pre_pool[0], pool.embedding_dim
    return (l1.weight[:, :E], pool.spatial_embedding.weight, pool.spatial_embedding.bias, l1.bias, None)


def fold_bwd(W, We, be, dA, dbias, dW=None, dbias_copy=None):
    W = _rows(W, "W")
    R, E = W.shape
    dW = dW if dW is not None else torch.empty(R, E, device=W.device, dtype=torch.float32)
    dWe = torch.empty(E, 2, device=W.device, dtype=torch.float32)
    dbe = torch.empty(E, device=W.device, dtype=torch.float32)
    N.check(_lib().sgg_fold_bwd(N.ptr(W), W.stride(0), R, E, N.ptr(We.contiguous()), N.ptr(be.contiguous()),
                                N.ptr(dA.contiguous()), N.ptr(dbias.contiguous()), N.ptr(dW), dW.stride(0), N.ptr(dWe),
                                N.ptr(dbe), N.ptr(dbias_copy), N.stream_ptr()), "sgg_fold_bwd")
    return dW, dWe, dbe


def xtw_partial(X, Y, colsum=False):
    lib = _lib()
    X = _rows(X, "X")
    Y = _rows(Y, "Y")
    R, M = X.shape
    Nn = Y.shape[1]
    assert Y.shape[0] == R and R > 0
    splits = lib.sgg_xtw_splits(R, M, Nn)
    ws = torch.empty(splits * (M * Nn + (Nn if colsum else 0)), device=X.device, dtype=torch.float32)

    def launch():
        N.check(lib.sgg_xtw_partial(N.ptr(X), X.stride(0), N.ptr(Y), Y.stride(0), None, 0, R, M, Nn, int(colsum),
                                    N.ptr(ws), ws.numel() * 4, N.stream_ptr()), "sgg_xtw_partial")
    launch()
    if timer.active:
        mt = 4 if M >= 64 else (M + 15) // 16
        timer.add("sgg::xtw_partial_kernel<%d>" % mt, (R, M, Nn), 2.0 * R * M * Nn,
                  4.0 * (R * M + R * Nn) + 4.0 * ws.numel(), launch)
    return ws, splits


class GradFinish:

    def __init__(self):
        self.reds, self.folds, self.keep = [], [], []

    def _hold(self, *ts):
        self.keep += [t.untyped_storage() for t in ts if t is not None]

    def rowsum(self, src, rows, ld, col0, cols, out):
# ... 825 lines not shown
            _, dWe, dbe = gf.fold(W1[:, :E], We, be, part, rows, P, bn * 512, ws[splits * H * 512:], splits, 512, 0,
                                  dW=dW1[:, :E])
            gf.run()
        return dh, None, dW1, dWe, dbe, dc, dW2, db2, None, None, None


class Handoff:

    def __init__(self):
        self.pending = None

    def put(self, *args):
        self.pending = args

    def take(self):
        p, self.pending = self.pending, None
        return p


class CopiesLink:

    def __init__(self):
        self.pending = None

    def put(self, base, copies, cstride, ld):
        self.pending = (base, copies, cstride, ld)

    def take(self):
        p, self.pending = self.pending, None
        return p


class GradLink:

    def __init__(self):
        self.grad = None

    def put(self, g):
        assert self.grad is None, "GradLink: gradient already pending"
        self.grad = g.contiguous()

    def take(self):
        g, self.grad = self.grad, None
        return g


def social_pool(h, pos, W1, We, be, b1, W2, b2, scenes, link=None, U=None):
    out, _ = _Pool.apply(h, pos, W1, We, be, b1, W2, b2, scenes, link, U)
    return out


def pool_u_spec(pool):
    l1, E = pool.mlp_pre_pool[0], pool.embedding_dim
    _, c = fold_fwd(l1.weight[:, :E], pool.spatial_embedding.weight, pool.spatial_embedding.bias, l1.bias)
    return l1.weight[:, E:], c


class _GatAttn(torch.autograd.Function):
    @staticmethod
    def forward(ctx, wh, a, bias, labels, seg_off, nseg, max_seg, alpha, mode, epi, heads):
        lib = _lib()
        wh = _req(wh, "wh").contiguous()
        n, HF = wh.shape
        F = HF // heads
        ctx.a_shape = a.shape
        a = a.contiguous().view(-1)
        if bias is not None:
            bias = bias.contiguous()
        y = torch.empty(n, HF, device=wh.device, dtype=torch.float32)
        hp = torch.empty(n, HF, device=wh.device, dtype=torch.float32) if epi else None
        N.check(lib.sgg_gat_fwd(N.ptr(wh), heads, N.ptr(a), N.ptr(bias), N.ptr(labels), N.ptr(seg_off), nseg, n, F,
                                float(alpha), mode, epi, max_seg, N.ptr(hp), N.ptr(y), HF, N.stream_ptr()),
                "sgg_gat_fwd")
        ctx.meta = (labels, seg_off, nseg, max_seg, float(alpha), mode, epi, heads, bias is not None)
        ctx.save_for_backward(wh, a, hp, y)
        return y

    @staticmethod
    def backward(ctx, dy):
        lib = _lib()
        wh, a, hp, y = ctx.saved_tensors
        labels, seg_off, nseg, max_seg, alpha, mode, epi, heads, has_bias = ctx.meta
        n, HF = wh.shape
        F = HF // heads
        dy = dy.contiguous()
        dWh = torch.empty(n, HF, device=wh.device, dtype=torch.float32)
        ds = torch.empty(n, heads, device=wh.device, dtype=torch.float32)
        dt = torch.empty(n, heads, device=wh.device, dtype=torch.float32)
        N.check(lib.sgg_gat_bwd(N.ptr(wh), heads, N.ptr(a), N.ptr(labels), N.ptr(seg_off), nseg, n, F, alpha, mode,
                                epi, max_seg, N.ptr(hp), N.ptr(y), N.ptr(dy), HF, N.ptr(dWh), N.ptr(ds), N.ptr(dt),
                                N.stream_ptr()), "sgg_gat_bwd")
        if not ctx.needs_input_grad[1] and not has_bias:
            return dWh, None, None, None, None, None, None, None, None, None, None
        dsdt = torch.cat([ds, dt], 1)
        if heads == 1:
            da = xtw(wh, dsdt).t().reshape(ctx.a_shape)
        else:
            C = xtw(wh, dsdt).view(heads, F, 2, heads)
            hh = torch.arange(heads, device=wh.device)
            da = C[hh, :, :, hh].permute(0, 2, 1).reshape(heads, 2 * F)
        dbias = None
        if has_bias:
            dpre = dy if epi == 0 else dy * torch.where(hp > 0, torch.ones_like(hp), torch.exp(hp))
            dbias = dpre.view(n, heads, F).double().sum((0, 1)).float()
        return dWh, da, dbias, None, None, None, None, None, None, None, None


# ... 653 lines not shown
    sc = groups.scenes
    rs = groups.ped_inv_size if scale else None
    return _SegGather.apply(gx, groups.ped_gid, rs, None, sc.B, sc.scene_off, groups.group_scene,
                            groups.n_groups_dev)


def scene_mean_over_groups(gx, groups):
    sc = groups.scenes
    if not hasattr(groups, "_group_inv_ng"):
        ng = (groups.group_off[1:] - groups.group_off[:-1]).float().clamp(min=1)
        groups._group_inv_ng = ng.index_select(0, groups.group_scene.long()).reciprocal()
    sm = _SegReduce.apply(gx, groups.group_scene, None, groups.group_off, None, None, sc.S, True,
                          groups._group_inv_ng, groups.n_groups_dev)
    return _SegGather.apply(sm, groups.group_scene, None, groups.n_groups_dev, groups.cap, groups.group_off, None,
                            None)


def _tkey(t):
    return (t.data_ptr(), tuple(t.shape), tuple(t.stride()))


class SharedPrefix:

    def __init__(self, lstm, emb, obs_rel, T, copies, fold_specs=None):
        self.lstm, self.emb, self.fold_specs = lstm, emb, fold_specs
        self.obs_rel = obs_rel
        self.key = _tkey(obs_rel)
        self.T_pre, self.Bsrc = int(obs_rel.shape[0]), int(obs_rel.shape[1])
        self.T, self.B = int(T), copies * self.Bsrc
        self.H = int(lstm.weight_hh_l0.shape[1])
        self.ran = self.used = False
        lib = _lib()
        self.ok = (lstm.num_layers == 1 and 0 < self.T_pre < self.T and self.Bsrc > 0
                   and (copies == 1 or self.Bsrc % 16 == 0)
                   and bool(lib.sgg_lstm_u_ok(self.T, self.B, self.H, 0, 1, 16))
                   and bool(lib.sgg_lstm_u_ok(self.T_pre, self.Bsrc, self.H, 0, 1, 16)))

    def arm(self, rel, H_g):
        return self.ok and not self.ran and H_g == 32 and self.H == 48 and _tkey(rel) == self.key

    def arm_dec(self, H_dec):
        return self.ok and not self.ran and H_dec == 32 and self.H == 48

    def segment(self, rel):
        lib = _lib()
        dev = rel.device
        T, B, H = self.T, self.B, self.H
        self.h_all = torch.empty(T + 1, B, H, device=dev, dtype=torch.float32)
        self.c_all = torch.empty(int(lib.sgg_lstm_state_floats(T, B, H, 1)), device=dev, dtype=torch.float32)
        self.act = torch.empty(int(lib.sgg_lstm_state_floats(T, B, H, 0)), device=dev, dtype=torch.float32)
        l = self.lstm
        if self.fold_specs is not None:
            prefold(self.fold_specs())
        self.A, self.bias = fold_fwd(l.weight_ih_l0, self.emb.weight, self.emb.bias, l.bias_ih_l0, l.bias_hh_l0)
        self.Whh = l.weight_hh_l0.contiguous()
        self.fold_ver = _fold_key(*lstm_fold_spec(l, self.emb))[1]
        self.whh_ver = (l.weight_hh_l0._version, _EPOCH.get(l.weight_hh_l0.data_ptr(), 0))
        s = N.LstmSeg(N.ptr(rel), N.ptr(self.A), N.ptr(self.Whh), N.ptr(self.bias), None, None, self.T_pre,
                      self.Bsrc, B, 0, T, self.Bsrc, N.ptr(self.h_all), N.ptr(self.c_all), N.ptr(self.act),
                      None, 0, None, 0, None)
        s._keep = (rel, self.A, self.Whh, self.bias, self.h_all, self.c_all, self.act)
        return s

    def matches(self, rel, W_hh, T, save):
        if not (self.ran and not self.used and save and T == self.T and W_hh is self.lstm.weight_hh_l0):
            return False
        if tuple(rel.shape) != (self.T, self.B, 2) or getattr(rel, "_sgg_head_key", None) != self.key:
            return False
        l = self.lstm
        return (_fold_key(*lstm_fold_spec(l, self.emb))[1] == self.fold_ver
                and (l.weight_hh_l0._version, _EPOCH.get(l.weight_hh_l0.data_ptr(), 0)) == self.whh_ver)


_PREFIX = [None]


@contextlib.contextmanager
def shared_prefix(D, obs_rel, T, copies):
    prev = _PREFIX[0]
    enc = D.encoder
    _PREFIX[0] = SharedPrefix(enc.encoder, enc.spatial_embedding, obs_rel, T, copies,
                              getattr(D, "fold_specs", None))
    try:
        yield _PREFIX[0]
    finally:
        _PREFIX[0] = prev


class EncoderRider:

    def __init__(self):
        self.held = None
        self.timing = None
        self.done = False

    def hold(self, segs, launch, timing):
        self.held = (segs, launch)
        self.timing = timing

    def carry(self, own, H):
        (a, Ha), (b, Hb) = self.held[0]
        self.held = None
        self.done = True
        lib = _lib()
        return lambda: N.check(lib.sgg_lstm_fwd_seg3(N.ctypes.byref(a), Ha, N.ctypes.byref(b), Hb,
                                                     N.ctypes.byref(own), H, N.stream_ptr()), "sgg_lstm_fwd_seg3")

    def flush(self):
        if self.held is not None:
            segs, launch = self.held
            self.held = None
            launch()
            if timer.active:
                name, key, fl, nb = self.timing
                timer.add(name, key, fl, nb, launch)
        self.done = True


_RIDER = [None]


class DecoderRider:

    def __init__(self):
        self.held = None
        self.timing = None
        self.done = False

    def hold(self, di, rel_out, to, B, H, T, weights, keep, launch):
        self.held = (di, rel_out, to, B, H, T, weights, keep, launch)

    def fits(self, H, T, *weights):
        if self.held is None:
            return False
        _, _, _, _, Hh, Th, wh, _, _ = self.held
        return Hh == H and Th == T and all(a is b for a, b in zip(wh, weights))

    def carry(self, di, A, Whh, bias, Wp, bp, T, B, H, rel_out, keep):
        di2, rel2, to2, B2, _, _, _, keep2, _ = self.held
        self.held = None
        self.done = True
        lib = _lib()
        return lambda k=(keep, keep2): lib.sgg_lstm_fwd_dec2(
            N.ctypes.byref(di), N.ctypes.byref(di2), N.ptr(A), N.ptr(Whh), N.ptr(bias), N.ptr(Wp), N.ptr(bp), T, B,
            B2, H, N.ptr(rel_out), N.ptr(rel2), N.ctypes.byref(to2) if to2 is not None else None, N.stream_ptr())

    def flush(self):
        if self.held is not None:
            launch = self.held[-1]
            self.held = None
            launch()
            if timer.active:
                timer.add(*self.timing, launch)
        self.done = True


_DRIDER = [None]


@contextlib.contextmanager
def decoder_pair():
    prev = _DRIDER[0]
    r = _DRIDER[0] = DecoderRider()
    try:
        yield r
    finally:
        _DRIDER[0] = prev
        r.flush()


@contextlib.contextmanager
def encoder_pair():
# ... 15 lines not shown
        self.held = None

    def hold(self, seg, alone, outs, nbytes):
        self.flush()
        self.held = (seg, alone, outs, nbytes)

    def take(self):
        seg, _, _, nb = self.held
        self.held = None
        return seg, nb

    def writes(self, t):
        return self.held is not None and t is not None and any(o.data_ptr() == t.data_ptr() for o in self.held[2])

    def flush(self):
        if self.held is not None:
            alone = self.held[1]
            self.held = None
            alone()


_GRIDE = [None]


@contextlib.contextmanager
def glue_ride():
    prev = _GRIDE[0]
    r = _GRIDE[0] = GlueRider()
    try:
        yield r
    finally:
        _GRIDE[0] = prev
        r.flush()


def glue_flush(reader=None):
    r = _GRIDE[0]
    if r is not None and (reader is None or r.writes(reader)):
        r.flush()


class _LSTMSeq(torch.autograd.Function):

    @staticmethod
    def forward(ctx, rel, W_ih, W_hh, b_ih, b_hh, We, be, h0, c0, Wp, bp, decoder, T, save, u=None, slink=None):
        lib = _lib()
        ctx.t_stop = int(getattr(rel, "_sgg_grad_from", 0))
        pfx = _PREFIX[0]
        rel_in = rel
        rel = _req(rel, "rel").contiguous()
        H = W_hh.shape[1]
        B = rel.shape[-2]
        dev = rel.device
        A, bias = fold_fwd(W_ih, We, be, b_ih, b_hh)
        carry = pfx is not None and not decoder and h0 is None and c0 is None and pfx.arm(rel_in, H)
        cont = (pfx is not None and not decoder and h0 is None and c0 is None and not carry
                and pfx.matches(rel_in, W_hh, T, save))
        ctx.t_sh, ctx.bsrc = (pfx.T_pre, pfx.Bsrc) if cont and pfx.Bsrc < B else (0, 0)
        glue, glue_nb = None, 0.0
        if _GRIDE[0] is not None and _GRIDE[0].held is not None:
            if cont or (not decoder and not carry and save and T <= 64
                        and bool(lib.sgg_lstm_u_ok(T, B, H, 0, 1, u[0].shape[0] if u is not None else 16))
                        and (u is None or _RIDER[0] is None or _RIDER[0].held is None)):
                glue, glue_nb = _GRIDE[0].take()
            else:
                glue_flush()
        if cont:
            h_all, c_all, act = pfx.h_all, pfx.c_all, pfx.act
            pfx.used = True
        else:
            h_all = torch.empty(T + 1, B, H, device=dev, dtype=torch.float32)
            c_all = torch.empty(int(lib.sgg_lstm_state_floats(T, B, H, 1)), device=dev, dtype=torch.float32)
            act = torch.empty(int(lib.sgg_lstm_state_floats(T, B, H, 0)), device=dev, dtype=torch.float32) \
                if save else None
        rel_out = torch.empty(T, B, 2, device=dev, dtype=torch.float32) if decoder else None
        no_final = (_NO_FINAL[0] and decoder and not save and not cont and h0 is not None and c0 is None
                    and getattr(h0, "_sgg_dinit", None) is not None)
        if no_final:
            h_all = c_all = None
        Whh = W_hh.contiguous()
        h0c = h0.contiguous() if h0 is not None else None
        c0c = c0.contiguous() if c0 is not None else None
        Wpc = Wp.contiguous() if Wp is not None else None
        U = None
        Wu = cu = None
        if u is not None:
            Wu, cu = u
            Wu = _rows(Wu, "Wu")
            cu = cu.contiguous()
            U = torch.empty(B, Wu.shape[0], device=dev, dtype=torch.float32)

        def seg(t0, Tn, Bsrc):
            s = N.LstmSeg(N.ptr(rel), N.ptr(A), N.ptr(Whh), N.ptr(bias), N.ptr(h0c), N.ptr(c0c), Tn, B, B, t0, T,
                          Bsrc, N.ptr(h_all), N.ptr(c_all), N.ptr(act), N.ptr(Wu),
                          Wu.stride(0) if Wu is not None else 0, N.ptr(cu), Wu.shape[0] if Wu is not None else 0,
                          N.ptr(U))
            s._keep = (rel, A, Whh, bias, h0c, c0c, h_all, c_all, act, Wu, cu, U)
            return s
        pfx_seg = pfx.segment(rel) if carry else None
        if carry:
            pfx.ran = True
        kname = None
        launch_done = False
        dheld = dcarried = False
        if carry:
            ga, gb = seg(0, T, B), pfx_seg
            kname = "sgg::lstm_mw_fwd2_kernel<32, %s, 48, true>" % ("true" if save else "false")

            def launch():
                N.check(lib.sgg_lstm_fwd_seg2(N.ctypes.byref(ga), H, N.ctypes.byref(gb), pfx.H, N.stream_ptr()),
                        "sgg_lstm_fwd_seg2")
        elif cont:
            gs = seg(pfx.T_pre, T - pfx.T_pre, pfx.Bsrc)

            if glue is not None:
                def launch():
                    N.check(lib.sgg_lstm_fwd_seg_glue(N.ctypes.byref(gs), H, N.ctypes.byref(glue), N.stream_ptr()),
                            "sgg_lstm_fwd_seg_glue")
            else:
                def launch():
                    N.check(lib.sgg_lstm_fwd_seg(N.ctypes.byref(gs), H, N.stream_ptr()), "sgg_lstm_fwd_seg")
        elif u is not None and glue is not None:
            gs = seg(0, T, B)

            def launch():
                N.check(lib.sgg_lstm_fwd_seg_glue(N.ctypes.byref(gs), H, N.ctypes.byref(glue), N.stream_ptr()),
                        "sgg_lstm_fwd_seg_glue")
        elif u is not None:
            def launch():
                N.check(lib.sgg_lstm_fwd_u(N.ptr(rel), N.ptr(A), N.ptr(Whh), N.ptr(bias), N.ptr(h0c), N.ptr(c0c), T,
                                           B, H, N.ptr(h_all), N.ptr(c_all), N.ptr(act), N.ptr(Wu), Wu.stride(0),
                                           N.ptr(cu), Wu.shape[0], N.ptr(U), N.stream_ptr()), "sgg_lstm_fwd_u")
        else:
            def launch():
                N.check(lib.sgg_lstm_fwd(N.ptr(rel), N.ptr(A), N.ptr(Whh), N.ptr(bias), N.ptr(h0c), N.ptr(c0c),
                                         N.ptr(Wpc), N.ptr(bp), T, B, H, int(decoder), N.ptr(h_all), N.ptr(c_all),
                                         N.ptr(act), N.ptr(rel_out), N.stream_ptr()), "sgg_lstm_fwd")
            if glue is not None:
                gs = seg(0, T, B)

                def launch():
                    N.check(lib.sgg_lstm_fwd_seg_glue(N.ctypes.byref(gs), H, N.ctypes.byref(glue), N.stream_ptr()),
                            "sgg_lstm_fwd_seg_glue")
            dinit =getattr(h0, "_sgg_dinit", None) if (decoder and h0 is not None and c0 is None) else None
            if dinit is not None:
                di, dkeep, materialize = dinit
                ta = _TRAJ[0]
                to = ta.desc(T, B) if ta is not None else None
                fkeep = (dkeep, A, Whh, bias, Wpc, bp, h_all, c_all, act, rel_out, rel,
                         (ta.out, ta.start, ta.head, ta.b, ta.pos0) if to is not None else None)
                dcarry = pfx is not None and save and pfx.arm_dec(H)
                if dcarry:
                    pseg = pfx.segment(pfx.obs_rel)
                    pfx.ran = True
                    kname = "sgg::lstm_mw_fwd2d_kernel<32, true, 48, true>"
                    fused = lambda k=fkeep, to=to, pseg=pseg, Hp=pfx.H: lib.sgg_lstm_fwd_dec_seg(
                        N.ctypes.byref(di), N.ptr(A), N.ptr(Whh), N.ptr(bias), N.ptr(Wpc), N.ptr(bp), T, B, H,
                        N.ptr(h_all), N.ptr(c_all), N.ptr(act), N.ptr(rel_out), N.ptr(rel),
                        N.ctypes.byref(to) if to is not None else None, N.ctypes.byref(pseg), Hp, N.stream_ptr())
                else:
                    fused = lambda k=fkeep, to=to: lib.sgg_lstm_fwd_dec(
                        N.ctypes.byref(di), N.ptr(A), N.ptr(Whh), N.ptr(bias), N.ptr(Wpc), N.ptr(bp), T, B, H,
                        N.ptr(h_all), N.ptr(c_all), N.ptr(act), N.ptr(rel_out), N.ptr(rel) if save else None,
                        N.ctypes.byref(to) if to is not None else None, N.stream_ptr())
                drider = _DRIDER[0]
                if drider is not None and not save and not dcarry and h_all is None and Wpc is not None:
                    mfma = "mfma" in lib.sgg_lstm_kernel_name(H, B, 1, 0, 0).decode()
                    if to is not None and drider.held is None and not drider.done:
                        dheld = True
                    elif mfma and drider.fits(H, T, A, Whh, bias, Wpc, bp):
                        fused = drider.carry(di, A, Whh, bias, Wpc, bp, T, B, H, rel_out, fkeep)
                        dcarried = True
                if dheld:
                    rc = 0
                else:
                    rc = fused()
                if rc != 0 and (dcarry or dcarried):
                    N.check(rc, "sgg_lstm_fwd_dec_seg" if dcarry else "sgg_lstm_fwd_dec2")
                if rc != 0 and to is not None:
                    to = None
                    fused = functools.partial(fused, to=None)
                    rc = fused()
                if rc == 0:
                    if to is not None:
                        ta.filled = (rel_out.data_ptr() + 8 * ta.col0, rel_out.stride(0))
                    launch = lambda: N.check(fused(), "sgg_lstm_fwd_dec")
                    if dheld:
                        drider.hold(di, rel_out, to, B, H, T, (A, Whh, bias, Wpc, bp), fkeep, launch)
                else:
                    if h_all is None:
                        h_all = torch.empty(T + 1, B, H, device=dev, dtype=torch.float32)
                        c_all = torch.empty(int(lib.sgg_lstm_state_floats(T, B, H, 1)), device=dev,
                                            dtype=torch.float32)
                    h0d, r0d = h0.detach(), rel
                    materialize(h0d, r0d)
                    plain = launch
                    launch = lambda: (materialize(h0d, r0d), plain())
                    plain()
                launch_done = True
            else:
                launch_done = False
        rider = _RIDER[0]
        held = carried = False
        if rider is not None and not launch_done and not decoder:
            if carry and rider.held is None and not rider.done:
                held = True
            elif (u is not None and save and not carry and not cont and rider.held is not None
                  and len(rider.held[0]) == 2):
                own = seg(0, T, B)
                launch = rider.carry(own, H)
                carried = True
        if not launch_done and not held:
            launch()
        if timer.active or held or dheld:
            Ts = T - pfx.T_pre if cont else T
            fl = Ts * B * (8.0 * H * (H + 3) + 12.0 * H) + (2.0 * B * H * U.shape[1] if U is not None else 0.0)
            nb = 4.0 * (Ts * B * 2 + ((act.numel() + c_all.numel()) * Ts / T + (Ts + 1) * B * H if save else
                                      (0 if no_final else 2 * B * H))
                        + 4 * H * (H + 3) + (T * B * 2 if decoder else 0) + (U.numel() if U is not None else 0))
            nb += glue_nb
            if carry or (decoder and kname is not None):
                Hp, Tp, Bp = pfx.H, pfx.T_pre, pfx.Bsrc
                fl += Tp * Bp * (8.0 * Hp * (Hp + 3) + 12.0 * Hp)
                nb += 4.0 * (Tp * Bp * 2 + Tp * Bp * 5 * Hp + (Tp + 1) * Bp * Hp + 4 * Hp * (Hp + 3))
            name = kname or lib.sgg_lstm_kernel_name(H, B, int(decoder), int(save), 0).decode()
            key = (Ts, B, int(decoder), int(save)) + ((pfx.T_pre,) if (carry or cont) else ())
            if dheld:
                drider.timing = (name, key, fl, nb)
            elif dcarried:
                hname, hkey, hfl, hnb = drider.timing
                timer.add(name, key + hkey, fl + hfl, nb + hnb, launch)
            elif held:
                rider.hold([(ga, H), (gb, pfx.H)], launch, (name, key, fl, nb))
            elif carried:
                hname, hkey, hfl, hnb = rider.timing
                timer.add("sgg::lstm_mw_fwd3_kernel<32, false, 48, true, 32, true>", hkey + key, hfl + fl, hnb + nb,
                          launch)
            else:
                timer.add(name, key, fl, nb, launch)
        ctx.meta = (decoder, T, B, H, h0 is not None)
        ctx.slink = slink
        ctx.set_materialize_grads(False)
        if save:
            ctx.save_for_backward(rel, W_ih, We, be, A, Whh, Wpc, h_all, c_all, act, rel_out)
        h_last = h_all[T] if h_all is not None else rel.new_empty(0, H)
        if U is not None:
            ctx.mark_non_differentiable(U)
            return h_last, U
        if decoder:
            return h_last, rel_out
        return h_last, h_last.new_empty(0)

    @staticmethod
    def backward(ctx, dh_last, drel_out):
        lib = _lib()
        decoder, T, B, H, has_h0 = ctx.meta
        rel, W_ih, We, be, A, Whh, Wp, h_all, c_all, act, rel_out = ctx.saved_tensors
        dev = rel.device
        need = ctx.needs_input_grad
        wgrad = any(need[1:7])
        rows = int(lib.sgg_lstm_wpart_rows(H, B))
        G4 = 4 * H
        P = G4 * H + G4 + 2 * G4
        PW = P + (2 * H + 2 if decoder else 0)
        wpart = torch.empty(rows, PW, device=dev, dtype=torch.float32) if (wgrad and rows > 0) else None
        dG = torch.empty(T, B, G4, device=dev, dtype=torch.float32) if rows == 0 else None
        nodx_name = (lib.sgg_lstm_kernel_name(H, B, 0, 1, 2).decode()
                     if (not decoder and not need[0] and wpart is not None) else "")
        nodx = nodx_name != ""
        drel_in = None if nodx else torch.empty(T, B, 2, device=dev, dtype=torch.float32)
        dh0 = torch.empty(B, H, device=dev, dtype=torch.float32) if has_h0 else None
        drel_tot = torch.empty(T, B, 2, device=dev, dtype=torch.float32) if decoder else None
        split = None
        if decoder and ctx.slink is not None:
            pend = ctx.slink.take()
            if pend is not None:
                ga, gb, bsplit, ph = pend
                if drel_out is None or drel_out.data_ptr() != ph.data_ptr():
                    raise N.NativeError("decoder backward: the split rollout output has another consumer")
                if rows > 0 and wgrad:
                    split = (ga, gb, bsplit)
                else:
                    drel_out = torch.cat([ga, gb], 1)
        if decoder:
            if split is not None:
                dout = split[0]
            else:
                dout = drel_out.contiguous() if drel_out is not None else torch.zeros(T, B, 2, device=dev)
            dhl = None
        else:
# ... 517 lines not shown
```

### group-gan-gcn-gat_amd/sgan/train_step.py

```python
import contextlib
import collections
import functools
import os
import random
import time

import numpy as np
import torch
import torch.distributed as dist

from . import kernels as K
from .models import get_noise
from .scene import SceneIndex


PAIR = os.environ.get("SGG_PAIR", "1") != "0"
DEC_PAIR = os.environ.get("SGG_DEC_PAIR", "1") != "0"


class TrainArgs:

    def __init__(self, **kw):
        self.obs_len = 8
        self.pred_len = 12
# ... 50 lines not shown
    def collective(self):
        return self.on and (self.world > 1 or self.exercise)

    @property
    def segmented(self):
        return self.collective and not self.capture

    def shard(self, S_global):
        if S_global < self.world:
            raise ValueError("scene-sharded DP needs >= %d scenes (one per rank), got %d: the reference loader "
                             "keeps a short last batch (loader.py:22-27); drop it or run it on fewer ranks"
                             % (self.world, S_global))
        per, rem = divmod(S_global, self.world)
        s0 = self.rank * per + min(self.rank, rem)
        return s0, s0 + per + (1 if self.rank < rem else 0)

    def allreduce_(self, tensors):
        if not self.collective or not tensors:
            return
        if self.cut is not None:
            self.cut(tensors)
            return
        flat = torch.cat([t.reshape(-1) for t in tensors])
        if self.transport == "rccl":
            self.rccl.allreduce_sum_(flat)
        else:
            dist.all_reduce(flat, op=dist.ReduceOp.SUM, group=self.group)
        views = flat.split([t.numel() for t in tensors])
        torch._foreach_copy_(tensors, [v.view_as(t) for v, t in zip(views, tensors)])


class StepInputs:

    def __init__(self, z_d, z_g, y):
        self.z_d, self.z_g, self.y = z_d, z_g, y


class KernelOps:
    traj_cat = staticmethod(K.traj_cat)
    l2_select = staticmethod(K.l2_select)
    l2_loss = staticmethod(K.l2_loss)
    bce_pair = staticmethod(K.bce_pair)
    bce_pair_total = staticmethod(K.bce_pair_total)
    split2 = staticmethod(K.split2)
    prefold = staticmethod(K.prefold)
    one = staticmethod(lambda device: K.const(1.0, device))
    optimizer = staticmethod(lambda params, lr: K.ClipAdam(params, lr=lr))
    handoff = staticmethod(K.bce_handoff)
    defer_finish = staticmethod(K.defer_grad_finish)
    shared_prefix = staticmethod(K.shared_prefix)
    traj_ahead = staticmethod(K.traj_ahead)
    decoder_pair = staticmethod(K.decoder_pair)
    glue_ride = staticmethod(K.glue_ride)
    eager_losses = staticmethod(K.eager_losses)


class GanTrainer:
    def __init__(self, G, D, args=None, dp=None, selective_backward=True, capturable=False, bce_pair=None, ops=None):
        self.G, self.D = G, D
        self.ops = ops or KernelOps()
        self._bce_override = bce_pair
        self.bce_pair = bce_pair or self.ops.bce_pair
        self.args = args or TrainArgs()
        self.dp = dp or DataParallel()
        self.selective_backward = selective_backward
        bn = [n for n, m in list(G.named_modules()) + list(D.named_modules()) if isinstance(m, torch.nn.BatchNorm1d)]
        if bn:
            raise NotImplementedError("GanTrainer: BatchNorm layers (%s) are not supported (train.py's batch_norm=0 "
                                      "default); drive the modules with the reference's own step functions" % bn[:3])
        self.g_params = list(G.parameters())
        self.d_params = list(D.parameters())
        self.opt_g = self.ops.optimizer(self.g_params, self.args.g_learning_rate)
        self.opt_d = self.ops.optimizer(self.d_params, self.args.d_learning_rate)

    def _noise(self, S_global, s0, s1):
        G = self.G
        if not G.noise_dim:
            return None
        if G.noise_mix_type != "global":
            raise NotImplementedError("GanTrainer shards scenes; per-ped noise ('ped' mix) is not sharded yet")
        z = get_noise((S_global,) + tuple(G.noise_dim), G.noise_type)
        return z[s0:s1]

    def _finish(self, params, opt, loss_terms, clip):
        K.side_join()
        K.grad_flush()
        grads = [p.grad for p in params if p.grad is not None]
        if self.dp.collective:
            vals = torch.stack([t.detach().reshape(()) for t in loss_terms])
            self.dp.allreduce_(grads + [vals])
        else:
            vals = [t.detach().reshape(()) for t in loss_terms]
        opt.step(max_norm=clip)
        return vals

    def _prefix(self, obs_rel, copies):
        sp = getattr(self.ops, "shared_prefix", None)
        if sp is None or getattr(self.D, "encoder", None) is None or os.environ.get("SGG_NO_SHARED_PREFIX"):
            return contextlib.nullcontext()
        return sp(self.D, obs_rel, self.args.obs_len + self.args.pred_len, copies)

    def _traj_ahead(self, head, T1, ncol, col0=0, b=None, pos0=None):
        ta = getattr(self.ops, "traj_ahead", None)
        if ta is None:
            return contextlib.nullcontext()
        return ta(head, T1, ncol, col0, b, pos0)

    def _scope(self):
        st = contextlib.ExitStack()
        st.enter_context(getattr(self.ops, "handoff", contextlib.nullcontext)())
        if not self._grad_observed():
            st.enter_context(getattr(self.ops, "defer_finish", contextlib.nullcontext)())
        st.enter_context(getattr(self.ops, "glue_ride", contextlib.nullcontext)())
        return st

    def _grad_observed(self):
        for p in self.g_params + self.d_params:
            if getattr(p, "_backward_hooks", None) or getattr(p, "_post_accumulate_grad_hooks", None) \
                    or p.retains_grad:
                return True
        return False

    def d_step(self, batch, sc, S_global=None, B_global=None, shard=(0, None), inputs=None, pair=None):
        with self._scope():
            return self._d_step(batch, sc, S_global, B_global, shard, inputs, pair)

    def _pairs(self, sc, sc_g):
        G = self.G
        return (PAIR and self.selective_backward and self.args.best_k > 1 and self.args.l2_loss_weight > 0
                and hasattr(G, "context_pair") and G.pair_ok(sc, sc_g))

    def _d_step(self, batch, sc, S_global, B_global, shard, inputs, pair=None):
        a = self.args
        G = self.G
        (obs, pred_gt, obs_rel, pred_gt_rel, _ov, _pv, obs_g, _pg, _nl, _lm, sse) = batch
        g_kw = (S_global, B_global)
        S_global = S_global or sc.S
        B_global = B_global or sc.B
        s0 = shard[0]
        z = inputs.z_d if inputs is not None else self._noise(S_global, s0, s0 + sc.S)
        prefold = getattr(self.ops, "prefold", None)
        if prefold is not None and hasattr(G, "fold_specs") and hasattr(self.D, "fold_specs") \
                and G.num_layers == 1 and self.D.encoder.num_layers == 1:
            prefold(G.fold_specs() + self.D.fold_specs())
        pre = None
        dpair = getattr(self.ops, "decoder_pair", None)
        dpair = dpair() if (pair is not None and DEC_PAIR and dpair is not None) else contextlib.nullcontext()
        with self._prefix(obs_rel, 2):
            with dpair:
                with self._traj_ahead(obs_rel, pred_gt_rel.shape[0], sc.B, 0, pred_gt_rel, obs[0]):
                    if pair is not None:
                        bg, scg = pair
                        ctx_d, ctx_g = G.context_pair((obs, obs_rel, sse, obs_g, sc),
                                                      (bg[0], bg[2], bg[10], bg[6], scg))
                        with torch.no_grad():
                            fake_rel = G.decode(ctx_d, obs, obs_rel, sse, user_noise=z, scenes=sc)
                    else:
                        with torch.no_grad():
                            fake_rel = G(obs, obs_rel, sse, obs_g, user_noise=z, scenes=sc)
                    traj_rel, start = self.ops.traj_cat(obs_rel, fake_rel, pred_gt_rel, obs[0])
                if pair is not None:
                    self._no_shared = True
                    try:
                        pre = self._g_prefix(bg, scg, g_kw[0], g_kw[1], shard, inputs, ctx=ctx_g)
                    finally:
                        self._no_shared = False
# ... 597 lines not shown
```

### include/sgg.h

```cpp
#ifndef SGG_H
#define SGG_H

#include <stdint.h>
#include <stddef.h>

#ifdef __cplusplus
extern "C" {
#endif

#define SGG_E_ARG (-1)

int sgg_version(void);
const char* sgg_last_error(void);
const char* sgg_source_hash(void);

#define SGG_POOL_MAX_PEDS 64
#define SGG_GAT_MAX_NODES 128

int sgg_xw(const float* X, int ldx, const float* Xmask, int ldm, const float* W, int ldw, int trans_w,
           const float* bias, float* Y, int ldy, int M, int K, int N, int act, void* stream);

int sgg_xw_bf16(const float* X, int ldx, const float* Xmask, int ldm, const float* W, int ldw, int trans_w,
                const float* bias, float* Y, int ldy, int M, int K, int N, int act, void* stream);

// ... 217 lines not shown
  int NB;
  int T0;
  int col0;
  int ncol;
  const float* head;
  int ldh;
  const float* b;
  int ldb;
  const float* pos0;
  float* start;
} SggTrajOut;
int sgg_lstm_fwd_dec(const SggDecInit* di, const float* A, const float* Whh, const float* bias, const float* Wp,
                     const float* bp, int T, int B, int H, float* h_all, float* c_all, float* act_all,
                     float* rel_out, float* rel0_out, const SggTrajOut* to, void* stream);
int sgg_lstm_fwd_dec2(const SggDecInit* di, const SggDecInit* di2, const float* A, const float* Whh,
                      const float* bias, const float* Wp, const float* bp, int T, int B, int B2, int H,
                      float* rel_out, float* rel_out2, const SggTrajOut* to2, void* stream);

int sgg_lstm_u_ok(int T, int B, int H, int decoder, int save, int NU);
int sgg_lstm_fwd_u(const float* rel, const float* A, const float* Whh, const float* bias, const float* h0,
                   const float* c0, int T, int B, int H, float* h_all, float* c_all, float* act_all,
                   const float* Wu, int ldwu, const float* cu, int NU, float* U, void* stream);

int sgg_lstm_wpart_rows(int H, int B);
const char* sgg_lstm_kernel_name(int H, int B, int decoder, int save, int bwd);
int sgg_lstm_bwd_split(const float* A, const float* Whh, const float* Wp, const float* h_all, const float* c_all,
                       const float* act_all, const float* rel, const float* rel_out, const float* dout,
                       const float* dout2, int bsplit, int T, int B, int H, float* dh0, float* drel_in,
                       float* drel_tot, float* wpart, void* stream);
int sgg_lstm_bwd_tail(const float* A, const float* Whh, const float* h_all, const float* c_all,
                      const float* act_all, const float* rel, const float* dh_last, int T, int B, int H,
                      int t_stop, float* drel_in, void* stream);
int sgg_lstm_bwd(const float* A, const float* Whh, const float* Wp, const float* h_all, const float* c_all,
                 const float* act_all, const float* rel, const float* rel_out, const float* dh_last,
                 const float* dout, int T, int B, int H, int decoder, float* dG, float* dh0,
                 float* drel_in, float* drel_tot, float* wpart, void* stream);

typedef struct {
  const float* rel;
  const float* A;
  const float* Whh;
  const float* bias;
  const float* h0;
  const float* c0;
  int T, B, Bl, t0, Tl, Bsrc;
  float* h_all;
  float* c_all;
  float* act_all;
  const float* Wu;
  int ldwu;
  const float* cu;
  int NU;
  float* U;
} SggLstmSeg;
int sgg_lstm_fwd_seg(const SggLstmSeg* seg, int H, void* stream);
int sgg_lstm_fwd_seg2(const SggLstmSeg* a, int Ha, const SggLstmSeg* b, int Hb, void* stream);
int sgg_lstm_fwd_seg3(const SggLstmSeg* a, int Ha, const SggLstmSeg* b, int Hb, const SggLstmSeg* c, int Hc,
                      void* stream);
int sgg_lstm_fwd_dec_seg(const SggDecInit* di, const float* A, const float* Whh, const float* bias, const float* Wp,
                         const float* bp, int T, int B, int H, float* h_all, float* c_all, float* act_all,
                         float* rel_out, float* rel0_out, const SggTrajOut* to, const SggLstmSeg* pre, int Hp,
                         void* stream);
int sgg_lstm_bwd_shared(const float* A, const float* Whh, const float* h_all, const float* c_all,
                        const float* act_all, const float* rel, const float* dh_last, int T, int B, int H,
                        int t_sh, int Bsrc, float* drel_in, float* wpart, void* stream);

int sgg_bce_fwd(const float* x, int n, int split, const float* ya, const float* yb, float w, float* loss,
                const float* addend, float* total, const int32_t* nvalid, void* stream);

int sgg_bce_bwd(const float* x, int n, int split, const float* ya, const float* yb, float w,
                const float* gout, float* dx, const int32_t* nvalid, void* stream);

int sgg_adam_parts(long long total);
int sgg_adam_step(float* const* params, float* const* grads, float* const* exp_avg, float* const* exp_avg_sq,
                  const long long* numel, int n, double lr, double beta1, double beta2, float eps, float max_norm,
                  float* const* step, float* ws, size_t ws_bytes, void* stream);

#define SGG_GATENC_MAX_HEADS 4
typedef struct {
  const float* Wi[SGG_GATENC_MAX_HEADS];
  const float* ai[SGG_GATENC_MAX_HEADS];
  const float* Wio;
  const float* aio;
  const float* Wg[SGG_GATENC_MAX_HEADS];
  const float* ag[SGG_GATENC_MAX_HEADS];
  const float* Wgo;
  const float* ago;
  const float* Woe;
  const float* boe;
} SggGatEncWeights;

typedef struct {
  const float* X;
  int ldx;
  const float* labels;
  const int32_t* scene_off;
  int S;
  int np;
  int nh;
  float alpha;
  SggGatEncWeights w;
  float* y;
  int ldy;
  const float* dy;
  int lddy;
  float* dX;
  int lddx;
  float* slab;
  float* saved;
  const float* X2;
  int ldx2;
  int kx1;
  float* dX2;
  int lddx2;
  int dy_copies;
// ... 99 lines not shown
```

Before: 142,900 scenes/s.

## Fold input-embedding weights inside fused LSTM kernels via rider fold jobs

Fold jobs (W_ih·W_emb products and combined biases) are deferred and run as extra blocks in the fused multi-segment LSTM forward kernels, so they no longer need a separate fold launch. Encoder segments that carry raw fold weights compute their own folded input weights in-kernel. The goal is to drop standalone fold_fwd_multi launches from the graph. The cost is more complex kernels, with a fallback to separate launches when the riders do not fit the CU count or a dependency is detected.

```diff
diff --git a/group-gan-gcn-gat_amd/csrc/fold.hip b/group-gan-gcn-gat_amd/csrc/fold.hip
--- a/group-gan-gcn-gat_amd/csrc/fold.hip
+++ b/group-gan-gcn-gat_amd/csrc/fold.hip
@@ -1,4 +1,5 @@
 #include "sgg_common.h"
+#include "fold_body.h"
 
 namespace sgg {
 
@@ -6,20 +7,7 @@
                                                        const float* __restrict__ We, const float* __restrict__ be,
                                                        const float* __restrict__ b1, const float* __restrict__ b2,
                                                        float* __restrict__ A, float* __restrict__ bias) {
-  for (int r = threadIdx.x; r < R; r += blockDim.x) {
-    float a0 = 0.f, a1 = 0.f, bb = 0.f;
-    const float* w = W + (size_t)r * ldw;
-#pragma unroll 8
-    for (int e = 0; e < E; ++e) {
-      const float we = w[e];
-      a0 = fmaf(we, We[2 * e], a0);
-      a1 = fmaf(we, We[2 * e + 1], a1);
-      bb = fmaf(we, be[e], bb);
-    }
-    A[2 * r] = a0;
-    A[2 * r + 1] = a1;
-    bias[r] = bb + b1[r] + (b2 ? b2[r] : 0.f);
-  }
+  fold_fwd_body(W, ldw, R, E, We, be, b1, b2, A, bias);
 }
 
 struct FoldList {
@@ -28,20 +16,7 @@
 
 __global__ void __launch_bounds__(512) fold_fwd_multi_kernel(FoldList L) {
   const SggFold& d = L.f[blockIdx.x];
-  for (int r = threadIdx.x; r < d.R; r += blockDim.x) {
-    float a0 = 0.f, a1 = 0.f, bb = 0.f;
-    const float* w = d.W + (size_t)r * d.ldw;
-#pragma unroll 8
-    for (int e = 0; e < d.E; ++e) {
-      const float we = w[e];
-      a0 = fmaf(we, d.We[2 * e], a0);
-      a1 = fmaf(we, d.We[2 * e + 1], a1);
-      bb = fmaf(we, d.be[e], bb);
-    }
-    d.A[2 * r] = a0;
-    d.A[2 * r + 1] = a1;
-    d.bias[r] = bb + d.b1[r] + (d.b2 ? d.b2[r] : 0.f);
-  }
+  fold_fwd_body(d.W, d.ldw, d.R, d.E, d.We, d.be, d.b1, d.b2, d.A, d.bias);
 }
 
 __device__ __forceinline__ void fold_bwd_body(const float* __restrict__ W, int ldw, int R, int E,
diff --git a/group-gan-gcn-gat_amd/csrc/fold_body.h b/group-gan-gcn-gat_amd/csrc/fold_body.h
--- /dev/null
+++ b/group-gan-gcn-gat_amd/csrc/fold_body.h
@@ -0,0 +1,87 @@
+#pragma once
+#include "sgg_common.h"
+
+namespace sgg {
+
+__device__ __forceinline__ void fold_step(float we, float we0, float we1, float bee, float& a0, float& a1,
+                                          float& bb) {
+  a0 = fmaf(we, we0, a0);
+  a1 = fmaf(we, we1, a1);
+  bb = fmaf(we, bee, bb);
+}
+
+__device__ __forceinline__ float fold_bias(float bb, float b1v, float b2v) { return bb + b1v + b2v; }
+
+__device__ __forceinline__ void fold_fwd_body(const float* __restrict__ W, int ldw, int R, int E,
+                                              const float* __restrict__ We, const float* __restrict__ be,
+                                              const float* __restrict__ b1, const float* __restrict__ b2,
+                                              float* __restrict__ A, float* __restrict__ bias) {
+  for (int r = threadIdx.x; r < R; r += blockDim.x) {
+    float a0 = 0.f, a1 = 0.f, bb = 0.f;
+    const float* w = W + (size_t)r * ldw;
+#pragma unroll 8
+    for (int e = 0; e < E; ++e) fold_step(w[e], We[2 * e], We[2 * e + 1], be[e], a0, a1, bb);
+    A[2 * r] = a0;
+    A[2 * r + 1] = a1;
+    bias[r] = fold_bias(bb, b1[r], b2 ? b2[r] : 0.f);
+  }
+}
+
+constexpr int kFoldChunk = 16;
+constexpr int kFoldMaxE = 64;
+
+template <int NR>
+struct FoldChunk {
+  float4 w[NR][kFoldChunk / 4];
+  float emb;
+};
+
+template <int NR>
+__device__ __forceinline__ void fold_load(const float* __restrict__ W, int ldw, int E, const int (&row)[NR], int e0,
+                                          const float* __restrict__ We, const float* __restrict__ be, int lane,
+                                          FoldChunk<NR>& ch) {
+#pragma unroll
+  for (int i = 0; i < NR; ++i)
+#pragma unroll
+    for (int k = 0; k < kFoldChunk / 4; ++k)
+      ch.w[i][k] = *reinterpret_cast<const float4*>(W + (size_t)row[i] * ldw + min(e0 + 4 * k, E - 4));
+  const float* p = lane < 2 * kFoldChunk ? We + min(2 * e0 + lane, 2 * E - 1)
+                                         : be + min(e0 + ((lane - 2 * kFoldChunk) & (kFoldChunk - 1)), E - 1);
+  ch.emb = *p;
+}
+
+template <int NR>
+__device__ __forceinline__ void fold_acc(const FoldChunk<NR>& ch, int E, int e0, float (&a0)[NR], float (&a1)[NR],
+                                         float (&bb)[NR]) {
+  auto emb = [&](int l) -> float {
+    return __int_as_float(__builtin_amdgcn_readlane(__float_as_int(ch.emb), l));
+  };
+#pragma unroll
+  for (int k = 0; k < kFoldChunk / 4; ++k) {
+    if (e0 + 4 * k < E) {
+#pragma unroll
+      for (int u = 0; u < 4; ++u) {
+        const int j = 4 * k + u;
+        const float we0 = emb(2 * j), we1 = emb(2 * j + 1), bee = emb(2 * kFoldChunk + j);
+#pragma unroll
+        for (int i = 0; i < NR; ++i) {
+          const float w = u == 0 ? ch.w[i][k].x : u == 1 ? ch.w[i][k].y : u == 2 ? ch.w[i][k].z : ch.w[i][k].w;
+          fold_step(w, we0, we1, bee, a0[i], a1[i], bb[i]);
+        }
+      }
+    }
+  }
+}
+
+template <int NR>
+__device__ __forceinline__ void fold_rest(const float* __restrict__ W, int ldw, int E, const int (&row)[NR],
+                                          const float* __restrict__ We, const float* __restrict__ be, int lane,
+                                          float (&a0)[NR], float (&a1)[NR], float (&bb)[NR]) {
+  for (int e0 = kFoldChunk; e0 < E; e0 += kFoldChunk) {
+    FoldChunk<NR> ch;
+    fold_load<NR>(W, ldw, E, row, e0, We, be, lane, ch);
+    fold_acc<NR>(ch, E, e0, a0, a1, bb);
+  }
+}
+
+}
diff --git a/group-gan-gcn-gat_amd/csrc/lstm.hip b/group-gan-gcn-gat_amd/csrc/lstm.hip
--- a/group-gan-gcn-gat_amd/csrc/lstm.hip
+++ b/group-gan-gcn-gat_amd/csrc/lstm.hip
@@ -312,9 +312,13 @@
 }
 
 static MwSeg to_mw(const SggLstmSeg& s) {
-  return MwSeg{s.rel, s.A, s.Whh, s.bias, s.h0, s.c0, nullptr, nullptr, s.T, s.B, s.Bl, s.t0, s.Tl, s.Bsrc,
-               s.h_all, s.c_all, s.act_all, nullptr, s.Wu, s.ldwu, s.cu, s.NU, s.U};
-}
+  MwSeg m{s.rel, s.A, s.Whh, s.bias, s.h0, s.c0, nullptr, nullptr, s.T, s.B, s.Bl, s.t0, s.Tl, s.Bsrc,
+          s.h_all, s.c_all, s.act_all, nullptr, s.Wu, s.ldwu, s.cu, s.NU, s.U};
+  m.fW = s.fW; m.fldw = s.fldw; m.fE = s.fE; m.fWe = s.fWe; m.fbe = s.fbe; m.fb1 = s.fb1; m.fb2 = s.fb2;
+  m.uW = s.uW; m.uldw = s.uldw; m.uE = s.uE; m.uWe = s.uWe; m.ube = s.ube; m.ub1 = s.ub1;
+  return m;
+}
+static bool has_raw(const SggLstmSeg& s) { return s.fW != nullptr || s.uW != nullptr; }
 
 extern "C" int sgg_lstm_fwd_seg(const SggLstmSeg* seg, int H, void* stream) {
   SGG_CHECK_ARG(seg, "sgg_lstm_fwd_seg: null segment");
@@ -333,8 +337,16 @@
   return ncu;
 }
 
+static bool riders_fit(int nblk, int n) {
+  const int cus = device_cus(), last = nblk % cus;
+  return !((nblk >= cus && last == 0) || last + n > cus);
+}
+
+extern "C" int sgg_lstm_riders_fit(int nblk, int n) { return nblk >= 1 && n >= 0 && riders_fit(nblk, n) ? 1 : 0; }
+
 extern "C" int sgg_lstm_fwd_seg_glue(const SggLstmSeg* seg, int H, const SggGlueSeg* glue, void* stream) {
   SGG_CHECK_ARG(seg && glue, "sgg_lstm_fwd_seg_glue: null segment");
+  SGG_CHECK_ARG(!has_raw(*seg), "sgg_lstm_fwd_seg_glue: a segment with raw fold weights (sgg_lstm_fwd_seg takes it)");
   SGG_CHECK_ARG(lstm_mw_ok(H, seg->B), "sgg_lstm_fwd_seg_glue: no four-wave kernel for H=%d", H);
   const SggGlueSeg& g = *glue;
   SGG_CHECK_ARG(g.kind == SGG_GLUE_NONE || g.kind == SGG_GLUE_SELECT || g.kind == SGG_GLUE_L2BWD,
@@ -350,8 +362,7 @@
                   "sgg_lstm_fwd_seg_glue (l2 backward): bad sizes");
   }
   if (g.kind != SGG_GLUE_NONE && g.S > 0) {
-    const int cus = device_cus(), nblk = (seg->B + 15) / 16, last = nblk % cus;
-    if ((nblk >= cus && last == 0) || last + g.S > cus) {
+    if (!riders_fit((seg->B + 15) / 16, g.S)) {
       const int rc = g.kind == SGG_GLUE_SELECT
                          ? sgg_l2_select(g.pred, g.gt, g.mask, g.ldm, g.scene_off, g.S, g.T, g.B, g.k, g.best, stream)
                          : sgg_l2_loss_bwd_scenes(g.pred, g.ldp, g.gt, g.mask, g.ldm, g.scene_off, g.S, g.T, g.B, g.w,
@@ -365,6 +376,7 @@
 
 extern "C" int sgg_lstm_fwd_seg2(const SggLstmSeg* a, int Ha, const SggLstmSeg* b, int Hb, void* stream) {
   SGG_CHECK_ARG(a && b, "sgg_lstm_fwd_seg2: null segment");
+  SGG_CHECK_ARG(!has_raw(*a) && !has_raw(*b), "sgg_lstm_fwd_seg2: a segment with raw fold weights");
   SGG_CHECK_ARG(lstm_mw_ok(Ha, a->B) && lstm_mw_ok(Hb, b->B), "sgg_lstm_fwd_seg2: no four-wave kernel (Ha=%d Hb=%d)",
                 Ha, Hb);
   return lstm_mw_fwd_seg2(to_mw(*a), Ha, to_mw(*b), Hb, (hipStream_t)stream);
@@ -373,9 +385,79 @@
 extern "C" int sgg_lstm_fwd_seg3(const SggLstmSeg* a, int Ha, const SggLstmSeg* b, int Hb, const SggLstmSeg* c, int Hc,
                                  void* stream) {
   SGG_CHECK_ARG(a && b && c, "sgg_lstm_fwd_seg3: null segment");
+  SGG_CHECK_ARG(!has_raw(*a) && !has_raw(*b) && !has_raw(*c),
+                "sgg_lstm_fwd_seg3: a segment with raw fold weights (sgg_lstm_fwd_seg3_fold takes it)");
   SGG_CHECK_ARG(lstm_mw_ok(Ha, a->B) && lstm_mw_ok(Hb, b->B) && lstm_mw_ok(Hc, c->B),
                 "sgg_lstm_fwd_seg3: no four-wave kernel (Ha=%d Hb=%d Hc=%d)", Ha, Hb, Hc);
   return lstm_mw_fwd_seg3(to_mw(*a), Ha, to_mw(*b), Hb, to_mw(*c), Hc, (hipStream_t)stream);
+}
+
+static int dec_check(const SggDecInit* di, const float* A, const float* Whh, const float* bias, const float* Wp,
+                     const float* bp, int T, int B, int H, float* h_all, float* c_all, float* act_all, float* rel_out,
+                     const SggTrajOut* to);
+
+static int riders_check(const SggFoldRiders* folds, const SggLstmSeg* const* segs, int nseg, const float* dec_A,
+                        const float* dec_bias, const char* fn) {
+  SGG_CHECK_ARG(folds && folds->n >= 1 && folds->n <= SGG_FOLD_MAX, "%s: 1 <= n <= %d fold jobs (got %d)", fn,
+                SGG_FOLD_MAX, folds ? folds->n : 0);
+  for (int k = 0; k < folds->n; ++k) {
+    const SggFold& d = folds->f[k];
+    SGG_CHECK_ARG(d.W && d.We && d.be && d.b1 && d.A && d.bias, "%s: null pointer in fold %d", fn, k);
+    SGG_CHECK_ARG(d.R >= 1 && d.E >= 1 && d.ldw >= d.E, "%s: bad sizes in fold %d", fn, k);
+    auto writes = [&](const float* p) { return p != nullptr && (p == d.A || p == d.bias); };
+    SGG_CHECK_ARG(!writes(dec_A) && !writes(dec_bias), "%s: the decoder segment reads the output of fold %d", fn, k);
+    for (int i = 0; i < nseg; ++i) {
+      const SggLstmSeg& s = *segs[i];
+      SGG_CHECK_ARG(s.fW || (!writes(s.A) && !writes(s.bias)),
+                    "%s: segment %d reads the output of fold %d without the raw weights (fW)", fn, i, k);
+      SGG_CHECK_ARG(!s.U || s.uW || !writes(s.cu),
+                    "%s: segment %d reads the output of fold %d as its projection bias without the raw weights (uW)",
+                    fn, i, k);
+    }
+  }
+  return 0;
+}
+
+static MwFolds to_mw(const SggFoldRiders& f) {
+  MwFolds m{};
+  m.n = f.n;
+  for (int k = 0; k < f.n; ++k) m.f[k] = f.f[k];
+  return m;
+}
+
+extern "C" int sgg_lstm_fwd_seg3_fold(const SggLstmSeg* a, int Ha, const SggLstmSeg* b, int Hb, const SggLstmSeg* c,
+                                      int Hc, const SggFoldRiders* folds, void* stream) {
+  SGG_CHECK_ARG(a && b && c, "sgg_lstm_fwd_seg3_fold: null segment");
+  SGG_CHECK_ARG(lstm_mw_ok(Ha, a->B) && lstm_mw_ok(Hb, b->B) && lstm_mw_ok(Hc, c->B),
+                "sgg_lstm_fwd_seg3_fold: no four-wave kernel (Ha=%d Hb=%d Hc=%d)", Ha, Hb, Hc);
+  const SggLstmSeg* segs[3] = {a, b, c};
+  if (int rc = riders_check(folds, segs, 3, nullptr, nullptr, "sgg_lstm_fwd_seg3_fold")) return rc;
+  const MwSeg ma = to_mw(*a), mb = to_mw(*b), mc = to_mw(*c);
+  const int nblk = (a->B + 15) / 16 + (b->B + 15) / 16 + (c->B + 15) / 16;
+  if (lstm_mw_fold3_ok(ma, Ha, mb, Hb, mc, Hc) && riders_fit(nblk, folds->n))
+    return lstm_mw_fwd_seg3_fold(ma, mb, mc, to_mw(*folds), (hipStream_t)stream);
+  if (int rc = sgg_fold_fwd_multi(folds->f, folds->n, stream)) return rc;
+  return lstm_mw_fwd_seg3(ma, Ha, mb, Hb, mc, Hc, (hipStream_t)stream);
+}
+
+extern "C" int sgg_lstm_fwd_dec_seg_fold(const SggDecInit* di, const float* A, const float* Whh, const float* bias,
+                                         const float* Wp, const float* bp, int T, int B, int H, float* h_all,
+                                         float* c_all, float* act_all, float* rel_out, float* rel0_out,
+                                         const SggTrajOut* to, const SggLstmSeg* pre, int Hp,
+                                         const SggFoldRiders* folds, void* stream) {
+  if (int rc = dec_check(di, A, Whh, bias, Wp, bp, T, B, H, h_all, c_all, act_all, rel_out, to)) return rc;
+  SGG_CHECK_ARG(pre && B >= 1 && act_all && lstm_mw_ok(H, B) && lstm_mw_ok(Hp, pre->B),
+                "sgg_lstm_fwd_dec_seg_fold: needs a saving four-wave decoder and a prefix segment (H=%d B=%d Hp=%d)",
+                H, B, Hp);
+  if (int rc = riders_check(folds, &pre, 1, A, bias, "sgg_lstm_fwd_dec_seg_fold")) return rc;
+  const MwSeg mp = to_mw(*pre);
+  const int nblk = (B + 15) / 16 + (pre->B + 15) / 16;
+  if (lstm_mw_fold_dec_ok(H, Hp, act_all, mp) && riders_fit(nblk, folds->n))
+    return lstm_mw_fwd_dec_seg_fold(A, Whh, bias, Wp, bp, T, B, h_all, c_all, act_all, rel_out, di, rel0_out, to, mp,
+                                    to_mw(*folds), (hipStream_t)stream);
+  if (int rc = sgg_fold_fwd_multi(folds->f, folds->n, stream)) return rc;
+  return lstm_mw_fwd_dec_seg(A, Whh, bias, Wp, bp, T, B, H, h_all, c_all, act_all, rel_out, di, rel0_out, to, mp, Hp,
+                             (hipStream_t)stream);
 }
 
 extern "C" int sgg_lstm_bwd_shared(const float* A, const float* Whh, const float* h_all, const float* c_all,
@@ -447,6 +529,8 @@
                                     float* act_all, float* rel_out, float* rel0_out, const SggTrajOut* to,
                                     const SggLstmSeg* pre, int Hp, void* stream) {
   if (int rc = dec_check(di, A, Whh, bias, Wp, bp, T, B, H, h_all, c_all, act_all, rel_out, to)) return rc;
+  SGG_CHECK_ARG(!pre || !has_raw(*pre),
+                "sgg_lstm_fwd_dec_seg: a segment with raw fold weights (sgg_lstm_fwd_dec_seg_fold takes it)");
   SGG_CHECK_ARG(pre && B >= 1 && act_all && lstm_mw_ok(H, B) && lstm_mw_ok(Hp, pre->B),
                 "sgg_lstm_fwd_dec_seg: needs a saving four-wave decoder and a prefix segment (H=%d B=%d Hp=%d)", H, B,
                 Hp);
diff --git a/group-gan-gcn-gat_amd/csrc/lstm_mw.hip b/group-gan-gcn-gat_amd/csrc/lstm_mw.hip
--- a/group-gan-gcn-gat_amd/csrc/lstm_mw.hip
+++ b/group-gan-gcn-gat_amd/csrc/lstm_mw.hip
@@ -5,6 +5,7 @@
 
 #include "sgg_common.h"
 #include "l2_body.h"
+#include "fold_body.h"
 
 namespace sgg {
 
@@ -105,8 +106,9 @@
 
 namespace {
 
-template <int H, bool DEC, bool SAVE>
+template <int H, bool DEC, bool SAVE, bool FOLD = false>
 __device__ __forceinline__ void mw_fwd_body(const MwSeg& sg, int blk, const SggGlueSeg* glue = nullptr) {
+  static_assert(!(FOLD && DEC), "in-kernel folds: encoder segments only");
   constexpr int MU = MwCfg<H>::MU, KS = MwCfg<H>::KS;
   constexpr bool decoder = DEC, save = SAVE;
   const float* __restrict__ rel = sg.rel;
@@ -127,6 +129,8 @@
   __shared__ float hst[X3 && SAVE ? 2 : 1][kMwPeds][X3 && SAVE ? kHsP : 1];
   __shared__ float2 rpart[2][4][kMwPeds];
   __shared__ float relseq[kMwMaxT][kMwPeds][2];
+  constexpr int kClMax = 512;
+  __shared__ float cl[FOLD ? kClMax : 1];
   if constexpr (!DEC) {
     if (glue) {
       static_assert(sizeof(relseq) >= kL2MaxElems * sizeof(float) && sizeof(hx) >= kL2MaxK * sizeof(float),
@@ -152,25 +156,33 @@
 
   float w[MU][KS + 1], ak0[MU], ak1[MU];
   bf16x8 wx[X3 ? MU : 1][2][3];
+  auto x3_whh = [&](int row, int c, int i) -> float {
+    const int w2 = (8 * c + i) >> 2, m2 = (8 * c + i) & 3;
+    return m2 < MU ? Whh[row * H + slot_unit(w2 * MU + m2, q)] : 0.f;
+  };
+  auto x3_val = [&](int c, int i, float wh, float a0, float a1, float bi) -> float {
+    const int w2 = (8 * c + i) >> 2, m2 = (8 * c + i) & 3;
+    return m2 == 3 ? (q != 0 ? 0.f : w2 == 0 ? a0 : w2 == 1 ? a1 : w2 == 2 ? bi : 0.f) : wh;
+  };
+  float whv[X3 && FOLD ? MU : 1][2][8];
   if constexpr (X3) {
 #pragma unroll
     for (int mu = 0; mu < MU; ++mu) {
       const int row = (c16 & 3) * H + slot_unit(g * MU + mu, c16 >> 2);
-      const float a0 = A[2 * row], a1 = A[2 * row + 1], bi = bias[row];
-#pragma unroll
-      for (int c = 0; c < 2; ++c) {
-        float v[8];
-#pragma unroll
-        for (int i = 0; i < 8; ++i) {
-          const int w2 = (8 * c + i) >> 2, m2 = (8 * c + i) & 3;
-          if (m2 < MU)
-            v[i] = Whh[row * H + slot_unit(w2 * MU + m2, q)];
-          else if (m2 == 3)
-            v[i] = q != 0 ? 0.f : w2 == 0 ? a0 : w2 == 1 ? a1 : w2 == 2 ? bi : 0.f;
-          else
-            v[i] = 0.f;
-        }
-        split8(v, wx[mu][c]);
+      if constexpr (FOLD) {
+#pragma unroll
+        for (int c = 0; c < 2; ++c)
+#pragma unroll
+          for (int i = 0; i < 8; ++i) whv[mu][c][i] = x3_whh(row, c, i);
+      } else {
+        const float a0 = A[2 * row], a1 = A[2 * row + 1], bi = bias[row];
+#pragma unroll
+        for (int c = 0; c < 2; ++c) {
+          float v[8];
+#pragma unroll
+          for (int i = 0; i < 8; ++i) v[i] = x3_val(c, i, x3_whh(row, c, i), a0, a1, bi);
+          split8(v, wx[mu][c]);
+        }
       }
     }
   }
@@ -185,9 +197,11 @@
       w[mu][4 * m + 2] = v.z;
       w[mu][4 * m + 3] = v.w;
     }
-    ak0[mu] = A[2 * row];
-    ak1[mu] = A[2 * row + 1];
-    w[mu][KS] = q == 0 ? ak0[mu] : q == 1 ? ak1[mu] : q == 2 ? bias[row] : 0.f;
+    if constexpr (!FOLD) {
+      ak0[mu] = A[2 * row];
+      ak1[mu] = A[2 * row + 1];
+      w[mu][KS] = q == 0 ? ak0[mu] : q == 1 ? ak1[mu] : q == 2 ? bias[row] : 0.f;
+    }
   }
   float c[MU], wp0[MU], wp1[MU], hv0[MU];
   const int nsrc = (sg.Bsrc + kMwPeds - 1) / kMwPeds;
@@ -270,6 +284,79 @@
     }
   }
 
+  if constexpr (FOLD) {
+    int frow[MU];
+#pragma unroll
+    for (int mu = 0; mu < MU; ++mu) frow[mu] = (c16 & 3) * H + slot_unit(g * MU + mu, c16 >> 2);
+    const bool fraw = sg.fW != nullptr;
+    const int nuc = sg.U ? sg.NU : 0;
+    const bool craw = nuc > 0 && sg.uW != nullptr;
+    constexpr int NC = kClMax / kMwThreads;
+    int crow[NC];
+#pragma unroll
+    for (int j = 0; j < NC; ++j) crow[j] = max(min((int)threadIdx.x + j * kMwThreads, nuc - 1), 0);
+    const float* fWp = fraw ? sg.fW : Whh;
+    const int fld = fraw ? sg.fldw : H, fE = fraw ? sg.fE : kFoldChunk;
+    const float *fWe = fraw ? sg.fWe : Whh, *fbe = fraw ? sg.fbe : Whh, *fb1 = fraw ? sg.fb1 : bias;
+    const float* fb2 = fraw && sg.fb2 ? sg.fb2 : fb1;
+    const float* cWp = craw ? sg.uW : nuc > 0 ? sg.Wu : Whh;
+    const int cld = craw ? sg.uldw : nuc > 0 ? sg.ldwu : H, cE = craw ? sg.uE : kFoldChunk;
+    const float *cWe = craw ? sg.uWe : Whh, *cbe = craw ? sg.ube : Whh, *cb1 = craw ? sg.ub1 : nuc > 0 ? sg.cu : Whh;
+    FoldChunk<MU> wl;
+    FoldChunk<NC> wc;
+    float fb1v[MU], fb2v[MU], cb1v[NC], pa0[MU], pa1[MU], pbi[MU];
+    fold_load<MU>(fWp, fld, fE, frow, 0, fWe, fbe, lane, wl);
+    fold_load<NC>(cWp, cld, cE, crow, 0, cWe, cbe, lane, wc);
+#pragma unroll
+    for (int mu = 0; mu < MU; ++mu) {
+      fb1v[mu] = fb1[frow[mu]];
+      fb2v[mu] = fb2[frow[mu]];
+      pa0[mu] = A[2 * frow[mu]];
+      pa1[mu] = A[2 * frow[mu] + 1];
+      pbi[mu] = bias[frow[mu]];
+    }
+#pragma unroll
+    for (int j = 0; j < NC; ++j) cb1v[j] = cb1[crow[j]];
+    float fa0[MU], fa1[MU], fbi[MU], fbb[MU];
+#pragma unroll
+    for (int mu = 0; mu < MU; ++mu) fa0[mu] = fa1[mu] = fbb[mu] = 0.f;
+    float ca0[NC], ca1[NC], cbb[NC];
+#pragma unroll
+    for (int j = 0; j < NC; ++j) ca0[j] = ca1[j] = cbb[j] = 0.f;
+    fold_acc<MU>(wl, fE, 0, fa0, fa1, fbb);
+    fold_acc<NC>(wc, cE, 0, ca0, ca1, cbb);
+    fold_rest<MU>(fWp, fld, fE, frow, fWe, fbe, lane, fa0, fa1, fbb);
+    fold_rest<NC>(cWp, cld, cE, crow, cWe, cbe, lane, ca0, ca1, cbb);
+#pragma unroll
+    for (int mu = 0; mu < MU; ++mu) {
+      const float fb = fold_bias(fbb[mu], fb1v[mu], sg.fb2 ? fb2v[mu] : 0.f);
+      fa0[mu] = fraw ? fa0[mu] : pa0[mu];
+      fa1[mu] = fraw ? fa1[mu] : pa1[mu];
+      fbi[mu] = fraw ? fb : pbi[mu];
+    }
+#pragma unroll
+    for (int j = 0; j < NC; ++j) {
+      const float cv = craw ? fold_bias(cbb[j], cb1v[j], 0.f) : cb1v[j];
+      if ((int)threadIdx.x + j * kMwThreads < nuc) cl[threadIdx.x + j * kMwThreads] = cv;
+    }
+#pragma unroll
+    for (int mu = 0; mu < MU; ++mu) {
+      if constexpr (X3) {
+#pragma unroll
+        for (int c = 0; c < 2; ++c) {
+          float v[8];
+#pragma unroll
+          for (int i = 0; i < 8; ++i) v[i] = x3_val(c, i, whv[mu][c][i], fa0[mu], fa1[mu], fbi[mu]);
+          split8(v, wx[mu][c]);
+        }
+      } else {
+        ak0[mu] = fa0[mu];
+        ak1[mu] = fa1[mu];
+        w[mu][KS] = q == 0 ? ak0[mu] : q == 1 ? ak1[mu] : q == 2 ? fbi[mu] : 0.f;
+      }
+    }
+  }
+
   constexpr bool kUPre = SGG_MW_UPRE && !DEC && H <= 48;
   constexpr int kUT = 8;
   const float* __restrict__ Wu = sg.Wu;
@@ -280,7 +367,8 @@
   float cuv[kUPre ? kUT : 1][4];
   auto load_wu = [&](int i) {
     const int ntile = NU >> 4;
-    const float4 v = *reinterpret_cast<const float4*>(sg.cu + 16 * min(g + 4 * i, ntile - 1) + 4 * q);
+    const int co = 16 * min(g + 4 * i, ntile - 1) + 4 * q;
+    const float4 v = FOLD ? *reinterpret_cast<const float4*>(&cl[co]) : *reinterpret_cast<const float4*>(sg.cu + co);
     cuv[i][0] = v.x;
     cuv[i][1] = v.y;
     cuv[i][2] = v.z;
@@ -565,11 +653,14 @@
         acc0 = __builtin_amdgcn_mfma_f32_16x16x4f32(wa[0][ks], hk[ks], acc0, 0, 0, 0);
         acc1 = __builtin_amdgcn_mfma_f32_16x16x4f32(wa[1][ks], hk[ks], acc1, 0, 0, 0);
       }
-      const float4 cb0 = *reinterpret_cast<const float4*>(cu + 16 * nt + 4 * q);
+      auto cu_at = [&](int co) -> float4 {
+        return FOLD ? *reinterpret_cast<const float4*>(&cl[co]) : *reinterpret_cast<const float4*>(cu + co);
+      };
+      const float4 cb0 = cu_at(16 * nt + 4 * q);
       *reinterpret_cast<float4*>(U + (size_t)pc * NU + 16 * nt + 4 * q) =
           make_float4(acc0[0] + cb0.x, acc0[1] + cb0.y, acc0[2] + cb0.z, acc0[3] + cb0.w);
       if (nt + 4 < ntile) {
-        const float4 cb1 = *reinterpret_cast<const float4*>(cu + 16 * (nt + 4) + 4 * q);
+        const float4 cb1 = cu_at(16 * (nt + 4) + 4 * q);
         *reinterpret_cast<float4*>(U + (size_t)pc * NU + 16 * (nt + 4) + 4 * q) =
             make_float4(acc1[0] + cb1.x, acc1[1] + cb1.y, acc1[2] + cb1.z, acc1[3] + cb1.w);
       }
@@ -585,15 +676,15 @@
   LMARK(63);
 }
 
-template <int H, bool DEC, bool SAVE>
+template <int H, bool DEC, bool SAVE, bool FOLD = false>
 __global__ void __launch_bounds__(kMwThreads) lstm_mw_fwd_kernel(MwSeg sg, SggGlueSeg gl, int nblk) {
   if constexpr (!DEC) {
     if ((int)blockIdx.x >= nblk) {
-      mw_fwd_body<H, DEC, SAVE>(sg, blockIdx.x - nblk, &gl);
+      mw_fwd_body<H, DEC, SAVE, FOLD>(sg, blockIdx.x - nblk, &gl);
       return;
     }
   }
-  mw_fwd_body<H, DEC, SAVE>(sg, blockIdx.x);
+  mw_fwd_body<H, DEC, SAVE, FOLD>(sg, blockIdx.x);
 }
 
 template <int HA, bool SA, int HB, bool SB>
@@ -621,6 +712,36 @@
     mw_fwd_body<HB, false, SB>(b, blk - nblk_a);
   else
     mw_fwd_body<HC, false, SC>(c, blk - nblk_a - nblk_b);
+}
+
+template <int HA, bool SA, int HB, bool SB, int HC, bool SC>
+__global__ void __launch_bounds__(kMwThreads) lstm_mw_fwd3f_kernel(MwSeg a, MwSeg b, MwSeg c, int nblk_a, int nblk_b,
+                                                                  int nblk_c, MwFolds fl) {
+  const int blk = blockIdx.x;
+  if (blk < nblk_a) {
+    mw_fwd_body<HA, false, SA, true>(a, blk);
+  } else if (blk < nblk_a + nblk_b) {
+    mw_fwd_body<HB, false, SB, true>(b, blk - nblk_a);
+  } else if (blk < nblk_a + nblk_b + nblk_c) {
+    mw_fwd_body<HC, false, SC, true>(c, blk - nblk_a - nblk_b);
+  } else {
+    const SggFold& d = fl.f[blk - nblk_a - nblk_b - nblk_c];
+    fold_fwd_body(d.W, d.ldw, d.R, d.E, d.We, d.be, d.b1, d.b2, d.A, d.bias);
+  }
+}
+
+template <int HA, bool SA, int HB, bool SB>
+__global__ void __launch_bounds__(kMwThreads) lstm_mw_fwd2df_kernel(MwSeg a, MwSeg b, int nblk_a, int nblk_b,
+                                                                   MwFolds fl) {
+  const int blk = blockIdx.x;
+  if (blk < nblk_a) {
+    mw_fwd_body<HA, true, SA>(a, blk);
+  } else if (blk < nblk_a + nblk_b) {
+    mw_fwd_body<HB, false, SB, true>(b, blk - nblk_a);
+  } else {
+    const SggFold& d = fl.f[blk - nblk_a - nblk_b];
+    fold_fwd_body(d.W, d.ldw, d.R, d.E, d.We, d.be, d.b1, d.b2, d.A, d.bias);
+  }
 }
 
 #ifndef SGG_MW_BWD_DB
@@ -1155,6 +1276,10 @@
   const int nblk = (sg.B + kMwPeds - 1) / kMwPeds;
   auto k = decoder ? (sg.act_tile ? lstm_mw_fwd_kernel<H, true, true> : lstm_mw_fwd_kernel<H, true, false>)
                    : (sg.act_tile ? lstm_mw_fwd_kernel<H, false, true> : lstm_mw_fwd_kernel<H, false, false>);
+  if constexpr (H != 64) {
+    if (!decoder && (sg.fW || sg.uW))
+      k = sg.act_tile ? lstm_mw_fwd_kernel<H, false, true, true> : lstm_mw_fwd_kernel<H, false, false, true>;
+  }
   const bool ride = glue && !decoder && glue->kind != SGG_GLUE_NONE && glue->S > 0;
   SggGlueSeg gl{};
   if (ride) gl = *glue;
@@ -1235,7 +1360,54 @@
                 "(B=%d Bsrc=%d)", fn, s.t0, s.B, s.Bsrc);
   SGG_CHECK_ARG(s.t0 == 0 || (!s.h0 && !s.c0), "%s: t0 > 0 takes its state from h_all / c_all, not h0 / c0", fn);
   SGG_CHECK_ARG(!s.U || (s.Wu && s.cu && s.NU >= 16 && s.NU % 16 == 0 && s.ldwu >= H), "%s: bad projection", fn);
+  auto raw_ok = [](const float* W, int ldw, int E) {
+    return E >= 4 && E % 4 == 0 && E <= kFoldMaxE && ldw >= E &&
+           ((reinterpret_cast<uintptr_t>(W) | ((uintptr_t)ldw * 4)) & 15) == 0;
+  };
+  SGG_CHECK_ARG(!(s.fW || s.uW) || ((H == 16 || H == 32 || H == 48) && (!s.U || s.NU <= 512)),
+                "%s: in-kernel folds need H = 16 / 32 / 48 and NU <= 512 (H=%d NU=%d)", fn, H, s.NU);
+  SGG_CHECK_ARG(!s.fW || (s.fWe && s.fbe && s.fb1 && raw_ok(s.fW, s.fldw, s.fE)),
+                "%s: raw LSTM fold weights: null pointer, or not E %% 4 == 0, E <= %d, 16-byte aligned rows (E=%d ldw=%d)",
+                fn, kFoldMaxE, s.fE, s.fldw);
+  SGG_CHECK_ARG(!s.uW || (s.U && s.uWe && s.ube && s.ub1 && raw_ok(s.uW, s.uldw, s.uE)),
+                "%s: raw projection-bias fold weights: no projection, null pointer, or not E %% 4 == 0, E <= %d, "
+                "16-byte aligned rows (E=%d ldw=%d)", fn, kFoldMaxE, s.uE, s.uldw);
   return 0;
+}
+
+bool lstm_mw_fold3_ok(const MwSeg& a, int Ha, const MwSeg& b, int Hb, const MwSeg& c, int Hc) {
+  auto nu_ok = [](const MwSeg& s) { return !s.U || s.NU <= 512; };
+  return Ha == 32 && Hb == 48 && Hc == 32 && !a.act_tile && b.act_tile && c.act_tile && nu_ok(a) && nu_ok(b) &&
+         nu_ok(c);
+}
+
+int lstm_mw_fwd_seg3_fold(const MwSeg& a, const MwSeg& b, const MwSeg& c, const MwFolds& folds, hipStream_t st) {
+  if (int rc = seg_check(a, 32, "sgg_lstm_fwd_seg3_fold (a)")) return rc;
+  if (int rc = seg_check(b, 48, "sgg_lstm_fwd_seg3_fold (b)")) return rc;
+  if (int rc = seg_check(c, 32, "sgg_lstm_fwd_seg3_fold (c)")) return rc;
+  const int na = (a.B + kMwPeds - 1) / kMwPeds, nb = (b.B + kMwPeds - 1) / kMwPeds, nc = (c.B + kMwPeds - 1) / kMwPeds;
+  hipLaunchKernelGGL((lstm_mw_fwd3f_kernel<32, false, 48, true, 32, true>), dim3(na + nb + nc + folds.n),
+                     dim3(kMwThreads), 0, st, a, b, c, na, nb, nc, folds);
+  SGG_RETURN_LAUNCH("sgg_lstm_fwd_seg3_fold");
+}
+
+bool lstm_mw_fold_dec_ok(int H, int Hb, const float* act_all, const MwSeg& b) {
+  return H == 32 && Hb == 48 && act_all && b.act_tile && (!b.U || b.NU <= 512);
+}
+
+int lstm_mw_fwd_dec_seg_fold(const float* A, const float* Whh, const float* bias, const float* Wp, const float* bp,
+                             int T, int B, float* h_all, float* c_all, float* act_all, float* rel_out,
+                             const SggDecInit* di, float* rel0_out, const SggTrajOut* to, const MwSeg& b,
+                             const MwFolds& folds, hipStream_t st) {
+  if (int rc = seg_check(b, 48, "sgg_lstm_fwd_dec_seg_fold (prefix)")) return rc;
+  MwSeg a{nullptr, A, Whh, bias, nullptr, nullptr, Wp, bp, T, B, B, 0, T, B, h_all, c_all, act_all, rel_out};
+  a.di = *di;
+  a.rel0_out = rel0_out;
+  if (to) a.to = *to;
+  const int na = (B + kMwPeds - 1) / kMwPeds, nb = (b.B + kMwPeds - 1) / kMwPeds;
+  hipLaunchKernelGGL((lstm_mw_fwd2df_kernel<32, true, 48, true>), dim3(na + nb + folds.n), dim3(kMwThreads), 0, st, a,
+                     b, na, nb, folds);
+  SGG_RETURN_LAUNCH("sgg_lstm_fwd_dec_seg_fold");
 }
 
 int lstm_mw_fwd_seg(const MwSeg& s, int H, hipStream_t st, const SggGlueSeg* glue) {
diff --git a/group-gan-gcn-gat_amd/csrc/sgg_common.h b/group-gan-gcn-gat_amd/csrc/sgg_common.h
--- a/group-gan-gcn-gat_amd/csrc/sgg_common.h
+++ b/group-gan-gcn-gat_amd/csrc/sgg_common.h
@@ -105,6 +105,16 @@
   SggDecInit di;
   float* rel0_out;
   SggTrajOut to;
+  const float *fW;
+  int fldw, fE;
+  const float *fWe, *fbe, *fb1, *fb2;
+  const float* uW;
+  int uldw, uE;
+  const float *uWe, *ube, *ub1;
+};
+struct MwFolds {
+  int n;
+  SggFold f[SGG_FOLD_MAX];
 };
 __device__ __forceinline__ float dec_h0(const SggDecInit& d, int p, int u) {
   const int r = p / d.Bper, i = p - r * d.Bper;
@@ -128,6 +138,18 @@
                                                               hipStream_t st);
 __attribute__((visibility("hidden"))) int lstm_mw_fwd_seg3(const MwSeg& a, int Ha, const MwSeg& b, int Hb,
                                                            const MwSeg& c, int Hc, hipStream_t st);
+__attribute__((visibility("hidden"))) bool lstm_mw_fold3_ok(const MwSeg& a, int Ha, const MwSeg& b, int Hb,
+                                                            const MwSeg& c, int Hc);
+__attribute__((visibility("hidden"))) int lstm_mw_fwd_seg3_fold(const MwSeg& a, const MwSeg& b, const MwSeg& c,
+                                                                const MwFolds& folds, hipStream_t st);
+__attribute__((visibility("hidden"))) bool lstm_mw_fold_dec_ok(int H, int Hb, const float* act_all, const MwSeg& b);
+__attribute__((visibility("hidden"))) int lstm_mw_fwd_dec_seg_fold(const float* A, const float* Whh,
+                                                                   const float* bias, const float* Wp,
+                                                                   const float* bp, int T, int B, float* h_all,
+                                                                   float* c_all, float* act_all, float* rel_out,
+                                                                   const SggDecInit* di, float* rel0_out,
+                                                                   const SggTrajOut* to, const MwSeg& b,
+                                                                   const MwFolds& folds, hipStream_t st);
 
 __attribute__((visibility("hidden"))) void fold_bwd_multi(const SggFoldBwd* folds, int n, hipStream_t st);
 
diff --git a/group-gan-gcn-gat_amd/sgan/_native.py b/group-gan-gcn-gat_amd/sgan/_native.py
--- a/group-gan-gcn-gat_amd/sgan/_native.py
+++ b/group-gan-gcn-gat_amd/sgan/_native.py
@@ -45,7 +45,9 @@
 class LstmSeg(ctypes.Structure):
     _fields_ = [("rel", _p), ("A", _p), ("Whh", _p), ("bias", _p), ("h0", _p), ("c0", _p), ("T", _i), ("B", _i),
                 ("Bl", _i), ("t0", _i), ("Tl", _i), ("Bsrc", _i), ("h_all", _p), ("c_all", _p), ("act_all", _p),
-                ("Wu", _p), ("ldwu", _i), ("cu", _p), ("NU", _i), ("U", _p)]
+                ("Wu", _p), ("ldwu", _i), ("cu", _p), ("NU", _i), ("U", _p),
+                ("fW", _p), ("fldw", _i), ("fE", _i), ("fWe", _p), ("fbe", _p), ("fb1", _p), ("fb2", _p),
+                ("uW", _p), ("uldw", _i), ("uE", _i), ("uWe", _p), ("ube", _p), ("ub1", _p)]
 
 
 _sargs = ctypes.POINTER(LstmSeg)
@@ -65,6 +67,11 @@
 class Fold(ctypes.Structure):
     _fields_ = [("W", _p), ("ldw", _i), ("R", _i), ("E", _i), ("We", _p), ("be", _p), ("b1", _p), ("b2", _p),
                 ("A", _p), ("bias", _p)]
+
+
+class FoldRiders(ctypes.Structure):
+    _fields_ = [("n", _i), ("f", Fold * FOLD_MAX)]
+
 
 RED_MAX = 24
 FOLDB_MAX = 6
@@ -153,6 +160,8 @@
     "sgg_lstm_fwd_seg_glue": (_i, [_sargs, _i, ctypes.POINTER(GlueSeg), _p]),
     "sgg_lstm_fwd_seg2": (_i, [_sargs, _i, _sargs, _i, _p]),
     "sgg_lstm_fwd_seg3": (_i, [_sargs, _i, _sargs, _i, _sargs, _i, _p]),
+    "sgg_lstm_riders_fit": (_i, [_i, _i]),
+    "sgg_lstm_fwd_seg3_fold": (_i, [_sargs, _i, _sargs, _i, _sargs, _i, ctypes.POINTER(FoldRiders), _p]),
     "sgg_lstm_bwd_shared": (_i, [_p, _p, _p, _p, _p, _p, _p, _i, _i, _i, _i, _i, _p, _p, _p]),
     "sgg_lstm_u_ok": (_i, [_i, _i, _i, _i, _i, _i]),
     "sgg_lstm_fwd_u": (_i, [_p, _p, _p, _p, _p, _p, _i, _i, _i, _p, _p, _p, _p, _i, _p, _i, _p, _p]),
@@ -169,6 +178,8 @@
                                _p, _p, ctypes.POINTER(TrajOut), _p]),
     "sgg_lstm_fwd_dec_seg": (_i, [ctypes.POINTER(DecInit), _p, _p, _p, _p, _p, _i, _i, _i, _p, _p, _p, _p, _p,
                                   ctypes.POINTER(TrajOut), _sargs, _i, _p]),
+    "sgg_lstm_fwd_dec_seg_fold": (_i, [ctypes.POINTER(DecInit), _p, _p, _p, _p, _p, _i, _i, _i, _p, _p, _p, _p, _p,
+                                       ctypes.POINTER(TrajOut), _sargs, _i, ctypes.POINTER(FoldRiders), _p]),
     "sgg_grad_finish_losses": (_i, [ctypes.POINTER(Red), _i, ctypes.POINTER(FoldBwd), _i, _p, _sz,
                                     ctypes.POINTER(L2Job), _i, ctypes.POINTER(BceJob), _i, _p]),
     "sgg_adam_parts": (_i, [ctypes.c_longlong]),
diff --git a/group-gan-gcn-gat_amd/sgan/kernels.py b/group-gan-gcn-gat_amd/sgan/kernels.py
--- a/group-gan-gcn-gat_amd/sgan/kernels.py
+++ b/group-gan-gcn-gat_amd/sgan/kernels.py
@@ -179,13 +179,15 @@
     return (C, cs) if colsum else C
 
 
-def fold_fwd(W, We, be, b1, b2=None):
+def fold_fwd(W, We, be, b1, b2=None, carrier=False):
     key, ver = _fold_key(W, We, be, b1, b2)
     ent = _FOLD_CACHE.get(key)
-    if _fold_hit(ent, ver, (W, We, be, b1, b2)):
-        return ent[1], ent[2]
-    prefold([(W, We, be, b1, b2)])
-    ent = _FOLD_CACHE[key]
+    if not _fold_hit(ent, ver, (W, We, be, b1, b2)):
+        prefold([(W, We, be, b1, b2)])
+        ent = _FOLD_CACHE[key]
+    r = _FRIDE[0]
+    if not carrier and r is not None and r.holds(key):
+        r.flush()
     return ent[1], ent[2]
 
 
@@ -228,24 +230,146 @@
     if not todo:
         return
     _fold_purge()
-    arr = (N.Fold * len(todo))()
-    outs = []
-    for k, (key, ver, (W, We, be, b1, b2)) in enumerate(todo):
+    outs, jobs = [], []
+    for key, ver, (W, We, be, b1, b2) in todo:
         W = _rows(W, "W")
         R, E = W.shape
         A = torch.empty(R, 2, device=W.device, dtype=torch.float32)
         bias = torch.empty(R, device=W.device, dtype=torch.float32)
         parts = (W, We.contiguous(), be.contiguous(), b1.contiguous(), b2.contiguous() if b2 is not None else None)
-        arr[k] = N.Fold(N.ptr(parts[0]), W.stride(0), R, E, N.ptr(parts[1]), N.ptr(parts[2]), N.ptr(parts[3]),
-                        N.ptr(parts[4]), N.ptr(A), N.ptr(bias))
+        jobs.append(_FoldJob(key, parts, A, bias))
         outs.append((key, ver, A, bias, parts))
-    for i in range(0, len(todo), N.FOLD_MAX):
-        chunk = (N.Fold * min(N.FOLD_MAX, len(todo) - i))(*arr[i:i + N.FOLD_MAX])
-        N.check(_lib().sgg_fold_fwd_multi(chunk, len(chunk), N.stream_ptr()), "sgg_fold_fwd_multi")
+    r = _FRIDE[0]
+    if r is not None and r.accepts(jobs):
+        r.hold(jobs)
+    else:
+        if r is not None:
+            r.drop([j.key for j in jobs])
+        _fold_launch(jobs)
     for (key, ver, A, bias, parts), (_, _, ts) in zip(outs, todo):
         refs = tuple(weakref.ref(_owner(t)) if t is not None else None for t in ts)
         copies = tuple(p for p, t in zip(parts, ts) if p is not None and p.data_ptr() != t.data_ptr())
         _FOLD_CACHE[key] = (ver, A, bias, copies, refs)
+
+
+class _FoldJob:
+
+    def __init__(self, key, parts, A, bias):
+        W = parts[0]
+        self.key, self.parts, self.A, self.bias = key, parts, A, bias
+        self.R, self.E, self.ldw = int(W.shape[0]), int(W.shape[1]), int(W.stride(0))
+        self.desc = N.Fold(N.ptr(W), self.ldw, self.R, self.E, N.ptr(parts[1]), N.ptr(parts[2]), N.ptr(parts[3]),
+                           N.ptr(parts[4]), N.ptr(A), N.ptr(bias))
+        self.inkernel = (self.E % 4 == 0 and 4 <= self.E <= 64 and self.ldw % 4 == 0 and W.data_ptr() % 16 == 0)
+
+    def tensors(self):
+        return tuple(t for t in self.parts if t is not None) + (self.A, self.bias)
+
+    def nbytes(self):
+        return 4.0 * (self.R * self.E + 3 * self.E + self.R * (2 if self.parts[4] is not None else 1) + 3 * self.R)
+
+
+def _fold_launch(jobs):
+    for i in range(0, len(jobs), N.FOLD_MAX):
+        part = jobs[i:i + N.FOLD_MAX]
+        chunk = (N.Fold * len(part))(*[j.desc for j in part])
+        chunk._keep = tuple(t for j in part for t in j.tensors())
+
+        def launch(chunk=chunk):
+            N.check(_lib().sgg_fold_fwd_multi(chunk, len(chunk), N.stream_ptr()), "sgg_fold_fwd_multi")
+        launch()
+        if timer.active:
+            timer.add("sgg::fold_fwd_multi_kernel", (len(part), sum(j.R for j in part)),
+                      sum(6.0 * j.R * j.E for j in part), sum(j.nbytes() for j in part), launch)
+
+
+FOLD_RIDE = os.environ.get("SGG_FOLD_RIDE", "0") not in ("", "0")
+
+
+class FoldRider:
+
+    def __init__(self):
+        self.jobs = []
+
+    def accepts(self, jobs):
+        keys = {j.key for j in jobs}
+        kept = [j for j in self.jobs if j.key not in keys]
+        return len(kept) + len(jobs) <= N.FOLD_MAX and all(j.inkernel for j in jobs)
+
+    def drop(self, keys):
+        self.jobs = [j for j in self.jobs if j.key not in keys]
+
+    def hold(self, jobs):
+        self.drop({j.key for j in jobs})
+        self.jobs.extend(jobs)
+
+    def holds(self, key):
+        return any(j.key == key for j in self.jobs)
+
+    def describe(self, seg, H):
+        for j in self.jobs:
+            a, b = j.A.data_ptr(), j.bias.data_ptr()
+            if seg.A == a or seg.bias == b:
+                if not (seg.A == a and seg.bias == b and H in (16, 32, 48) and (not seg.U or seg.NU <= 512)):
+                    return False
+                W, We, be, b1, b2 = j.parts
+                seg.fW, seg.fldw, seg.fE = W.data_ptr(), j.ldw, j.E
+                seg.fWe, seg.fbe, seg.fb1 = We.data_ptr(), be.data_ptr(), b1.data_ptr()
+                seg.fb2 = b2.data_ptr() if b2 is not None else None
+                seg._keep = tuple(seg._keep) + j.tensors()
+            if seg.U and seg.cu == b:
+                if not (j.parts[4] is None and H in (16, 32, 48) and seg.NU <= 512 and seg.NU == j.R):
+                    return False
+                W, We, be, b1, _ = j.parts
+                seg.uW, seg.uldw, seg.uE = W.data_ptr(), j.ldw, j.E
+                seg.uWe, seg.ube, seg.ub1 = We.data_ptr(), be.data_ptr(), b1.data_ptr()
+                seg._keep = tuple(seg._keep) + j.tensors()
+            if seg.cu in (a, b) and not (seg.U and seg.cu == b):
+                return False
+        return True
+
+    def reads(self, *ptrs):
+        outs = {p for j in self.jobs for p in (j.A.data_ptr(), j.bias.data_ptr())}
+        return any(p in outs for p in ptrs if p)
+
+    def take(self):
+        jobs, self.jobs = self.jobs, []
+        fr = N.FoldRiders()
+        fr.n = len(jobs)
+        for k, j in enumerate(jobs):
+            fr.f[k] = j.desc
+        fr._keep = tuple(t for j in jobs for t in j.tensors())
+        return fr, sum(j.nbytes() for j in jobs)
+
+    def flush(self):
+        if self.jobs:
+            jobs, self.jobs = self.jobs, []
+            _fold_launch(jobs)
+
+
+_FRIDE = [None]
+
+
+@contextlib.contextmanager
+def fold_ride():
+    if not FOLD_RIDE:
+        yield None
+        return
+    prev = _FRIDE[0]
+    if prev is not None:
+        prev.flush()
+    r = _FRIDE[0] = FoldRider()
+    try:
+        yield r
+    finally:
+        _FRIDE[0] = prev
+        r.flush()
+
+
+def fold_flush():
+    r = _FRIDE[0]
+    if r is not None:
+        r.flush()
 
 
 def lstm_fold_spec(lstm, emb):
@@ -1177,7 +1301,8 @@
 
 def pool_u_spec(pool):
     l1, E = pool.mlp_pre_pool[0], pool.embedding_dim
-    _, c = fold_fwd(l1.weight[:, :E], pool.spatial_embedding.weight, pool.spatial_embedding.bias, l1.bias)
+    _, c = fold_fwd(l1.weight[:, :E], pool.spatial_embedding.weight, pool.spatial_embedding.bias, l1.bias,
+                    carrier=True)
     return l1.weight[:, E:], c
 
 
@@ -1937,7 +2062,8 @@
         l = self.lstm
         if self.fold_specs is not None:
             prefold(self.fold_specs())
-        self.A, self.bias = fold_fwd(l.weight_ih_l0, self.emb.weight, self.emb.bias, l.bias_ih_l0, l.bias_hh_l0)
+        self.A, self.bias = fold_fwd(l.weight_ih_l0, self.emb.weight, self.emb.bias, l.bias_ih_l0, l.bias_hh_l0,
+                                     carrier=True)
         self.Whh = l.weight_hh_l0.contiguous()
         self.fold_ver = _fold_key(*lstm_fold_spec(l, self.emb))[1]
         self.whh_ver = (l.weight_hh_l0._version, _EPOCH.get(l.weight_hh_l0.data_ptr(), 0))
@@ -1988,6 +2114,11 @@
         self.held = None
         self.done = True
         lib = _lib()
+        folds, self.folds = _fold_riders([(a, Ha), (b, Hb), (own, H)])
+        if folds is not None:
+            return lambda: N.check(lib.sgg_lstm_fwd_seg3_fold(N.ctypes.byref(a), Ha, N.ctypes.byref(b), Hb,
+                                                              N.ctypes.byref(own), H, N.ctypes.byref(folds),
+                                                              N.stream_ptr()), "sgg_lstm_fwd_seg3_fold")
         return lambda: N.check(lib.sgg_lstm_fwd_seg3(N.ctypes.byref(a), Ha, N.ctypes.byref(b), Hb,
                                                      N.ctypes.byref(own), H, N.stream_ptr()), "sgg_lstm_fwd_seg3")
 
@@ -1995,6 +2126,7 @@
         if self.held is not None:
             segs, launch = self.held
             self.held = None
+            fold_flush()
             launch()
             if timer.active:
                 name, key, fl, nb = self.timing
@@ -2003,6 +2135,20 @@
 
 
 _RIDER = [None]
+
+
+def _fold_riders(segs, extra_blocks=0):
+    fr = _FRIDE[0]
+    if fr is None or not fr.jobs:
+        return None, (False, 0.0)
+    nblk = extra_blocks + sum((s.B + 15) // 16 for s, _ in segs)
+    if _lib().sgg_lstm_riders_fit(nblk, len(fr.jobs)) and all(fr.describe(s, H) for s, H in segs):
+        folds, nb = fr.take()
+        return folds, (True, nb)
+    for s, _ in segs:
+        s.fW = s.uW = None
+    fr.flush()
+    return None, (False, 0.0)
 
 
 class DecoderRider:
@@ -2124,7 +2270,7 @@
         H = W_hh.shape[1]
         B = rel.shape[-2]
         dev = rel.device
-        A, bias = fold_fwd(W_ih, We, be, b_ih, b_hh)
+        A, bias = fold_fwd(W_ih, We, be, b_ih, b_hh, carrier=True)
         carry = pfx is not None and not decoder and h0 is None and c0 is None and pfx.arm(rel_in, H)
         cont = (pfx is not None and not decoder and h0 is None and c0 is None and not carry
                 and pfx.matches(rel_in, W_hh, T, save))
@@ -2173,6 +2319,7 @@
         if carry:
             pfx.ran = True
         kname = None
+        fold_rode, fold_nb = False, 0.0
         launch_done = False
         dheld = dcarried = False
         if carry:
@@ -2226,11 +2373,24 @@
                     pseg = pfx.segment(pfx.obs_rel)
                     pfx.ran = True
                     kname = "sgg::lstm_mw_fwd2d_kernel<32, true, 48, true>"
-                    fused = lambda k=fkeep, to=to, pseg=pseg, Hp=pfx.H: lib.sgg_lstm_fwd_dec_seg(
-                        N.ctypes.byref(di), N.ptr(A), N.ptr(Whh), N.ptr(bias), N.ptr(Wpc), N.ptr(bp), T, B, H,
-                        N.ptr(h_all), N.ptr(c_all), N.ptr(act), N.ptr(rel_out), N.ptr(rel),
-                        N.ctypes.byref(to) if to is not None else None, N.ctypes.byref(pseg), Hp, N.stream_ptr())
+                    fr = _FRIDE[0]
+                    if fr is not None and fr.reads(A.data_ptr(), bias.data_ptr()):
+                        fr.flush()
+                    folds, (_, fold_nb) = _fold_riders([(pseg, pfx.H)], extra_blocks=(B + 15) // 16)
+                    if folds is not None:
+                        kname = "sgg::lstm_mw_fwd2df_kernel<32, true, 48, true>"
+                        fused = lambda k=fkeep, to=to, pseg=pseg, Hp=pfx.H, folds=folds: lib.sgg_lstm_fwd_dec_seg_fold(
+                            N.ctypes.byref(di), N.ptr(A), N.ptr(Whh), N.ptr(bias), N.ptr(Wpc), N.ptr(bp), T, B, H,
+                            N.ptr(h_all), N.ptr(c_all), N.ptr(act), N.ptr(rel_out), N.ptr(rel),
+                            N.ctypes.byref(to) if to is not None else None, N.ctypes.byref(pseg), Hp,
+                            N.ctypes.byref(folds), N.stream_ptr())
+                    else:
+                        fused = lambda k=fkeep, to=to, pseg=pseg, Hp=pfx.H: lib.sgg_lstm_fwd_dec_seg(
+                            N.ctypes.byref(di), N.ptr(A), N.ptr(Whh), N.ptr(bias), N.ptr(Wpc), N.ptr(bp), T, B, H,
+                            N.ptr(h_all), N.ptr(c_all), N.ptr(act), N.ptr(rel_out), N.ptr(rel),
+                            N.ctypes.byref(to) if to is not None else None, N.ctypes.byref(pseg), Hp, N.stream_ptr())
                 else:
+                    fold_flush()
                     fused = lambda k=fkeep, to=to: lib.sgg_lstm_fwd_dec(
                         N.ctypes.byref(di), N.ptr(A), N.ptr(Whh), N.ptr(bias), N.ptr(Wpc), N.ptr(bp), T, B, H,
                         N.ptr(h_all), N.ptr(c_all), N.ptr(act), N.ptr(rel_out), N.ptr(rel) if save else None,
@@ -2282,7 +2442,10 @@
                 own = seg(0, T, B)
                 launch = rider.carry(own, H)
                 carried = True
+                fold_rode, fold_nb = rider.folds
         if not launch_done and not held:
+            if not carried:
+                fold_flush()
             launch()
         if timer.active or held or dheld:
             Ts = T - pfx.T_pre if cont else T
@@ -2291,6 +2454,7 @@
                                       (0 if no_final else 2 * B * H))
                         + 4 * H * (H + 3) + (T * B * 2 if decoder else 0) + (U.numel() if U is not None else 0))
             nb += glue_nb
+            nb += fold_nb
             if carry or (decoder and kname is not None):
                 Hp, Tp, Bp = pfx.H, pfx.T_pre, pfx.Bsrc
                 fl += Tp * Bp * (8.0 * Hp * (Hp + 3) + 12.0 * Hp)
@@ -2306,8 +2470,8 @@
                 rider.hold([(ga, H), (gb, pfx.H)], launch, (name, key, fl, nb))
             elif carried:
                 hname, hkey, hfl, hnb = rider.timing
-                timer.add("sgg::lstm_mw_fwd3_kernel<32, false, 48, true, 32, true>", hkey + key, hfl + fl, hnb + nb,
-                          launch)
+                timer.add("sgg::lstm_mw_fwd3%s_kernel<32, false, 48, true, 32, true>" % ("f" if fold_rode else ""),
+                          hkey + key, hfl + fl, hnb + nb, launch)
             else:
                 timer.add(name, key, fl, nb, launch)
         ctx.meta = (decoder, T, B, H, h0 is not None)
diff --git a/group-gan-gcn-gat_amd/sgan/train_step.py b/group-gan-gcn-gat_amd/sgan/train_step.py
--- a/group-gan-gcn-gat_amd/sgan/train_step.py
+++ b/group-gan-gcn-gat_amd/sgan/train_step.py
@@ -126,6 +126,7 @@
     traj_ahead = staticmethod(K.traj_ahead)
     decoder_pair = staticmethod(K.decoder_pair)
     glue_ride = staticmethod(K.glue_ride)
+    fold_ride = staticmethod(K.fold_ride)
     eager_losses = staticmethod(K.eager_losses)
 
 
@@ -186,6 +187,7 @@
         if not self._grad_observed():
             st.enter_context(getattr(self.ops, "defer_finish", contextlib.nullcontext)())
         st.enter_context(getattr(self.ops, "glue_ride", contextlib.nullcontext)())
+        st.enter_context(getattr(self.ops, "fold_ride", contextlib.nullcontext)())
         return st
 
     def _grad_observed(self):
diff --git a/include/sgg.h b/include/sgg.h
--- a/include/sgg.h
+++ b/include/sgg.h
@@ -293,6 +293,17 @@
   const float* cu;
   int NU;
   float* U;
+  const float* fW;
+  int fldw, fE;
+  const float* fWe;
+  const float* fbe;
+  const float* fb1;
+  const float* fb2;
+  const float* uW;
+  int uldw, uE;
+  const float* uWe;
+  const float* ube;
+  const float* ub1;
 } SggLstmSeg;
 int sgg_lstm_fwd_seg(const SggLstmSeg* seg, int H, void* stream);
 int sgg_lstm_fwd_seg2(const SggLstmSeg* a, int Ha, const SggLstmSeg* b, int Hb, void* stream);
@@ -302,6 +313,17 @@
                          const float* bp, int T, int B, int H, float* h_all, float* c_all, float* act_all,
                          float* rel_out, float* rel0_out, const SggTrajOut* to, const SggLstmSeg* pre, int Hp,
                          void* stream);
+typedef struct {
+  int n;
+  SggFold f[SGG_FOLD_MAX];
+} SggFoldRiders;
+int sgg_lstm_riders_fit(int nblk, int n);
+int sgg_lstm_fwd_seg3_fold(const SggLstmSeg* a, int Ha, const SggLstmSeg* b, int Hb, const SggLstmSeg* c, int Hc,
+                           const SggFoldRiders* folds, void* stream);
+int sgg_lstm_fwd_dec_seg_fold(const SggDecInit* di, const float* A, const float* Whh, const float* bias,
+                              const float* Wp, const float* bp, int T, int B, int H, float* h_all, float* c_all,
+                              float* act_all, float* rel_out, float* rel0_out, const SggTrajOut* to,
+                              const SggLstmSeg* pre, int Hp, const SggFoldRiders* folds, void* stream);
 int sgg_lstm_bwd_shared(const float* A, const float* Whh, const float* h_all, const float* c_all,
                         const float* act_all, const float* rel, const float* dh_last, int T, int B, int H,
                         int t_sh, int Bsrc, float* drel_in, float* wpart, void* stream);
```

Measured after the change: 142,300 scenes/s. Within noise of the previous version (-0.5%).
